# YuePanEdward/GH-ICP

Hardware: AMD Instinct MI355X
Metric: registered_pairs_per_sec (higher is better)
Workload: dtype f64

## Files before the change

### gh-icp_amd/csrc/ctx.h

```cpp
#pragma once
#include <hip/hip_runtime.h>

#include <atomic>
#include <cstdarg>
#include <cstdio>
#include <cstring>
#include <string>
#include <vector>

#include "../../include/ghicp_c.h"

#define GH_HIP(call)                                                                                          \
  do {                                                                                                        \
    hipError_t e_ = (call);                                                                                   \
    if (e_ != hipSuccess) return ctx->fail(GHICP_ERR_HIP, "%s:%d %s -> %s", __FILE__, __LINE__, #call, hipGetErrorString(e_)); \
  } while (0)
#define GH_TRY(call)               \
  do {                             \
    int r_ = (call);               \
    if (r_ != GHICP_OK) return r_; \
  } while (0)
#define GH_ARG(cond)                                                                \
  do {                                                                              \
    if (!(cond)) return ctx->fail(GHICP_ERR_ARG, "%s: bad argument (%s)", __func__, #cond); \
  } while (0)

#define GH_ENTER(ctx)                                                                                             \
  do {                                                                                                            \
    if (!(ctx)) return GHICP_ERR_ARG;                                                                             \
    if (hipSetDevice((ctx)->device) != hipSuccess) return (ctx)->fail(GHICP_ERR_HIP, "hipSetDevice(%d) failed", (ctx)->device); \
  } while (0)

struct DevBuf {
  void* p = nullptr;
  size_t cap = 0;
  hipError_t reserve(size_t bytes) {
    if (bytes <= cap) return hipSuccess;
    if (p) {
      hipError_t e = hipFree(p);
      if (e != hipSuccess) return e;
      p = nullptr; cap = 0;
    }
    size_t want = bytes + bytes / 4 + 256;
    hipError_t e = hipMalloc(&p, want);
    if (e != hipSuccess) return e;
    cap = want;
    return hipSuccess;
  }
  template <typename T> T* as() const { return reinterpret_cast<T*>(p); }
  void release() { if (p) (void)hipFree(p); p = nullptr; cap = 0; }
};

enum BufSlot {
  B_STAGE0 = 0, B_STAGE1, B_STAGE2, B_STAGE3, B_STAGE4, B_STAGE5, B_STAGE6, B_STAGE7,
  B_LOOP_STATE, B_LOOP_KPS, B_LOOP_PARTMIN, B_LOOP_PARTIDX, B_LOOP_PARTSUM, B_LOOP_PARTMIN2, B_LOOP_PARTIDX2, B_LOOP_FDT,
  B_LOOP_SP, B_LOOP_TP, B_LOOP_TRACE, B_LOOP_WFD, B_LOOP_KMW, B_LOOP_KMMATCH, B_LOOP_KMSCR, B_LOOP_ACC,
  B_GRID_KEYS, B_GRID_KEYS2, B_GRID_VALS, B_GRID_VALS2, B_GRID_TMP, B_GRID_START, B_GRID_PTS, B_GRID_MISC,
  B_GRID2_KEYS, B_GRID2_KEYS2, B_GRID2_VALS, B_GRID2_VALS2, B_GRID2_START, B_GRID2_PTS,
  B_FE_LAMBDA, B_FE_CURV, B_FE_COUNT, B_FE_CAND, B_FE_STATE, B_FE_KP, B_FE_SORTK, B_FE_SORTK2, B_FE_SORTV, B_FE_SORTV2, B_FE_CPTS,
  B_FE_FLAGS, B_FE_SCAN, B_FE_SCATTER,
  B_P_KEEP_S, B_P_KEEP_T, B_P_DS_S, B_P_DS_T, B_P_KP_S, B_P_KP_T, B_P_KPXYZ_S, B_P_KPXYZ_T, B_P_FEAT_S, B_P_FEAT_T, B_P_LCS,
  B_P_FD, B_P_MISC, B_P_PATTERN, B_FD_JOBS, B_TRANSFORM_JOBS,
  B_KM_LX, B_KM_MISC, B_KM_SLACK, B_KM_LSTAT, B_KM_ORDER,
  B_FB_DESC, B_FB_HEADPOS, B_FB_DS, B_FB_ORD,
  B_PRIM_TMP, B_NMSR_KEY, B_NMSR_CELL, B_NMSR_TABLE, B_NMSR_HEAD, B_NMSR_PTS, B_NMSR_SKEY, B_NMSR_STATE, B_NMSR_NEXT, B_NMSR_SEL, B_NMSR_MISC, B_NMSR_LIST, B_NMSR_PTS0, B_NMSR_SKEY0,
  B_ICP_TC_KEYS, B_ICP_TC_KEYS2, B_ICP_TC_VALS, B_ICP_TC_VALS2, B_ICP_TC_START, B_ICP_TC_PTS,
  B_ICP_SC_KEYS, B_ICP_SC_KEYS2, B_ICP_SC_VALS, B_ICP_SC_VALS2, B_ICP_SC_START, B_ICP_SC_PTS,
  B_ICP_CUR, B_ICP_Q, B_ICP_NN, B_ICP_ND, B_ICP_NN2, B_ICP_ND2, B_ICP_KEYS, B_ICP_KEYS2, B_ICP_SORTTMP, B_ICP_PART, B_ICP_STATE,
  B_ICP_PEND, B_ICP_TNRM, B_ICP_OUT,
  B_GICP_COVS, B_GICP_COVT, B_GICP_MAHAL, B_GICP_SRC4,
  B_NUM
};

enum KtSlot { KT_PCA = 0, KT_BSC, KT_KM_SOLVE, KT_CD_ROWMIN, KT_KM_WEIGHTS, KT_FD_BSC, KT_NMS_ROUND, KT_VOXEL_SORT,
              KT_FB_VOXEL, KT_FB_GRID, KT_FB_PRUNE, KT_FB_RANK, KT_FB_OUT,
              KT_PAIR_LOOP,
              KT_TRANSFORM,
              KT_PAIR_LOOP_DISPATCH,
              KT_NUM };
static const char* const kKtNames[KT_NUM] = {"pca_cells", "bsc", "km_solve", "cd_rowmin", "km_weights", "fd_bsc", "nms_round", "voxel_sort",
                                             "fb_voxel", "fb_grid", "fb_prune", "fb_rank", "fb_out", "pair_loop", "transform", "pair_loop_dispatch"};

struct ghicp_ctx {
  bool kt_on = false;
  double kt_ms[KT_NUM] = {0};
  long long kt_count[KT_NUM] = {0};
  struct KtPending { int slot; hipEvent_t a, b; };
  std::vector<KtPending> kt_pending;
  std::vector<hipEvent_t> kt_pool;
  hipEvent_t kt_event() {
    if (!kt_pool.empty()) { hipEvent_t e = kt_pool.back(); kt_pool.pop_back(); return e; }
    hipEvent_t e = nullptr;
    (void)hipEventCreate(&e);
    return e;
  }
  hipEvent_t kt_begin(int slot) { return kt_begin_on(slot, stream); }
  void kt_end(int slot, hipEvent_t a) { kt_end_on(slot, a, stream); }
  hipEvent_t kt_begin_on(int slot, hipStream_t st) {
    if (!kt_on) return nullptr;
    hipEvent_t a = kt_event();
    (void)hipEventRecord(a, st);
    (void)slot;
    return a;
  }
  void kt_end_on(int slot, hipEvent_t a, hipStream_t st) {
    if (!kt_on || !a) return;
    hipEvent_t b = kt_event();
    (void)hipEventRecord(b, st);
    kt_pending.push_back({slot, a, b});
  }
  void kt_collect() {
    for (auto& p : kt_pending) {
      float ms = 0;
      if (hipEventElapsedTime(&ms, p.a, p.b) == hipSuccess) { kt_ms[p.slot] += ms; kt_count[p.slot]++; }
      kt_pool.push_back(p.a);
      kt_pool.push_back(p.b);
    }
    kt_pending.clear();
  }
  static constexpr int KM_LSTAT_MAX = 8192;
  static constexpr int KM_LSTAT_W = 8;
  long long km_launches = 0;
  std::vector<int> km_slots;
  long long loop_hazards = 0;
  std::vector<float> loop_cost_hints;
  std::vector<long long> loop_timeline;
  std::atomic<long long> loop_active{0}, loop_total{0};
  bool bbox_valid = false;
  const float* bbox_ptr = nullptr;
  long long bbox_n = 0;
  int bbox_stride = 0;
  float bbox_mm[6] = {0, 0, 0, 0, 0, 0};
  int device = 0;
  hipStream_t stream = nullptr;
  hipStream_t own_stream = nullptr;
  bool km_stats = false, km_force_hazard = false;
  int loop_slots_cap = 0;
  bool loop_confine = true;
  double loop_confine_margin = 1.15;
  hipStream_t confine_stream = nullptr, rest_stream = nullptr;
  int confine_cus = 0;
  struct ConfinePair { int cus; hipStream_t confined, rest; };
  std::vector<ConfinePair> confine_cache;
  int loop_min_lds = 0;
  std::vector<uint32_t> cu_mask;
  std::vector<hipStream_t> aux_streams;
  std::vector<hipEvent_t> aux_events;
  int* progress_host = nullptr;
  std::atomic<bool> progress_live{false};
  bool host_ptrs = false;
  struct Staged { const void* host; size_t bytes; uint64_t fp; void* dev; uint64_t tick; };
  std::vector<Staged> staged;
  size_t staged_bytes = 0;
  uint64_t stage_tick = 0;
  long long staged_hits = 0, staged_misses = 0;
  void stage_clear() {
    if (staged.empty()) return;
    (void)hipStreamSynchronize(stream);
    for (auto& e : staged) (void)hipFree(e.dev);
    staged.clear();
    staged_bytes = 0;
  }
  static constexpr size_t STAGED_MIN = 256 * 1024, STAGED_CAP = (size_t)1 << 30;
  std::string err;
  DevBuf buf[B_NUM];
  std::vector<DevBuf> pairbuf;
  void* pinned = nullptr;
  void* job_pinned = nullptr;
  size_t job_pinned_cap = 0;
  hipEvent_t job_event = nullptr;
  bool job_pending = false;
  int upload_table(const void* src, size_t bytes, void* dst) {
    if (job_pending) {
      if (hipEventSynchronize(job_event) != hipSuccess) return fail(GHICP_ERR_HIP, "job table: event wait failed");
      job_pending = false;
    }
    if (bytes > job_pinned_cap) {
      if (job_pinned) (void)hipHostFree(job_pinned);
      job_pinned = nullptr;
      job_pinned_cap = 0;
      const size_t cap = ((bytes * 3 / 2) + 4095) & ~(size_t)4095;
      if (hipHostMalloc(&job_pinned, cap, hipHostMallocDefault) != hipSuccess) return fail(GHICP_ERR_HIP, "job table: pinned allocation of %zu bytes failed", cap);
      job_pinned_cap = cap;
    }
    if (!job_event && hipEventCreateWithFlags(&job_event, hipEventDisableTiming) != hipSuccess) return fail(GHICP_ERR_HIP, "job table: event creation failed");
    memcpy(job_pinned, src, bytes);
    if (hipMemcpyAsync(dst, job_pinned, bytes, hipMemcpyHostToDevice, stream) != hipSuccess) return fail(GHICP_ERR_HIP, "job table: upload failed");
    if (hipEventRecord(job_event, stream) != hipSuccess) return fail(GHICP_ERR_HIP, "job table: event record failed");
    job_pending = true;
    return GHICP_OK;
  }
  void* fb_pinned = nullptr;
  std::vector<struct ghicp_cloud*> pair_clouds;
  size_t pinned_cap = 0;
  int num_cu = 256;

  int fail(int code, const char* fmt, ...) {
    char tmp[1024];
    va_list ap;
    va_start(ap, fmt);
    vsnprintf(tmp, sizeof(tmp), fmt, ap);
    va_end(ap);
    err = tmp;
    return code;
  }
  template <typename T> int reserve(BufSlot s, size_t count, T** out) {
    hipError_t e = buf[s].reserve(count * sizeof(T) + 16);
    if (e != hipSuccess) return fail(GHICP_ERR_HIP, "hipMalloc(%zu bytes, slot %d): %s", count * sizeof(T), (int)s, hipGetErrorString(e));
    *out = buf[s].as<T>();
    return GHICP_OK;
  }
};

struct Stager {
  ghicp_ctx* ctx;
  struct Out { void* host; void* dev; size_t bytes; };
  std::vector<Out> outs;
  std::vector<void*> temps;
  bool uploaded = false;
  explicit Stager(ghicp_ctx* c) : ctx(c) { ctx->stage_tick++; }
  ~Stager() {
    if (uploaded && temps.empty()) (void)hipStreamSynchronize(ctx->stream);
    for (void* p : temps) (void)hipFree(p);
  }
  static uint64_t fingerprint(const void* p, size_t bytes) {
    const unsigned char* b = reinterpret_cast<const unsigned char*>(p);
    const size_t nw = bytes / 8;
    uint64_t h0 = 0x9E3779B97F4A7C15ull, h1 = 0xC2B2AE3D27D4EB4Full, h2 = 0x165667B19E3779F9ull, h3 = 0x27D4EB2F165667C5ull;
    size_t i = 0;
    for (; i + 4 <= nw; i += 4) {
      uint64_t w[4];
      memcpy(w, b + i * 8, 32);
      h0 = (h0 ^ w[0]) * 0x100000001B3ull; h1 = (h1 ^ w[1]) * 0x100000001B3ull;
      h2 = (h2 ^ w[2]) * 0x100000001B3ull; h3 = (h3 ^ w[3]) * 0x100000001B3ull;
      h0 ^= h0 >> 29; h1 ^= h1 >> 31; h2 ^= h2 >> 27; h3 ^= h3 >> 33;
    }
    for (; i < nw; i++) { uint64_t w; memcpy(&w, b + i * 8, 8); h0 = (h0 ^ w) * 0x100000001B3ull; }
    for (size_t k = nw * 8; k < bytes; k++) h1 = (h1 ^ b[k]) * 0x100000001B3ull;
    return (h0 ^ (h1 << 1) ^ (h2 << 2) ^ (h3 << 3)) + bytes;
  }
  template <typename T> int in_cloud(const T* p, size_t count, const T** out) { return stage_in(p, count, out, true); }
  template <typename T> int in(const T* p, size_t count, const T** out) { return stage_in(p, count, out, false); }
  template <typename T> int stage_in(const T* p, size_t count, const T** out, bool cacheable) {
    if (!ctx->host_ptrs || p == nullptr) { *out = p; return GHICP_OK; }
    const size_t bytes = count * sizeof(T);
    if (cacheable && bytes >= ghicp_ctx::STAGED_MIN && bytes <= ghicp_ctx::STAGED_CAP / 4) {
      const uint64_t fp = fingerprint(p, bytes);
      for (auto& e : ctx->staged)
        if (e.host == p && e.bytes == bytes && e.fp == fp) {
          e.tick = ctx->stage_tick;
          ctx->staged_hits++;
          *out = reinterpret_cast<const T*>(e.dev);
          return GHICP_OK;
        }
      while (!ctx->staged.empty() && (ctx->staged_bytes + bytes > ghicp_ctx::STAGED_CAP || ctx->staged.size() >= 16)) {
        size_t lru = ctx->staged.size();
        for (size_t i = 0; i < ctx->staged.size(); i++)
          if (ctx->staged[i].tick != ctx->stage_tick && (lru == ctx->staged.size() || ctx->staged[i].tick < ctx->staged[lru].tick)) lru = i;
        if (lru == ctx->staged.size()) break;
        (void)hipStreamSynchronize(ctx->stream);
        (void)hipFree(ctx->staged[lru].dev);
        ctx->staged_bytes -= ctx->staged[lru].bytes;
        ctx->staged.erase(ctx->staged.begin() + (long)lru);
      }
      void* d = nullptr;
      if (hipMalloc(&d, bytes + 16) != hipSuccess) return ctx->fail(GHICP_ERR_HIP, "stage-in hipMalloc failed");
      if (hipMemcpyAsync(d, p, bytes, hipMemcpyHostToDevice, ctx->stream) != hipSuccess) { (void)hipFree(d); return ctx->fail(GHICP_ERR_HIP, "stage-in copy failed"); }
      ctx->staged.push_back({p, bytes, fp, d, ctx->stage_tick});
      ctx->staged_bytes += bytes;
      ctx->staged_misses++;
      uploaded = true;
      *out = reinterpret_cast<const T*>(d);
      return GHICP_OK;
    }
    void* d = nullptr;
    if (hipMalloc(&d, count * sizeof(T) + 16) != hipSuccess) return ctx->fail(GHICP_ERR_HIP, "stage-in hipMalloc failed");
    temps.push_back(d);
    if (hipMemcpyAsync(d, p, count * sizeof(T), hipMemcpyHostToDevice, ctx->stream) != hipSuccess)
      return ctx->fail(GHICP_ERR_HIP, "stage-in copy failed");
    *out = reinterpret_cast<const T*>(d);
    return GHICP_OK;
  }
  template <typename T> int out(T* p, size_t count, T** outp) {
    if (!ctx->host_ptrs || p == nullptr) { *outp = p; return GHICP_OK; }
    void* d = nullptr;
    if (hipMalloc(&d, count * sizeof(T) + 16) != hipSuccess) return ctx->fail(GHICP_ERR_HIP, "stage-out hipMalloc failed");
    temps.push_back(d);
    outs.push_back({p, d, count * sizeof(T)});
    *outp = reinterpret_cast<T*>(d);
    return GHICP_OK;
  }
  int finish() {
    for (auto& o : outs)
      if (hipMemcpyAsync(o.host, o.dev, o.bytes, hipMemcpyDeviceToHost, ctx->stream) != hipSuccess)
        return ctx->fail(GHICP_ERR_HIP, "stage-out copy failed");
    if (!outs.empty() && hipStreamSynchronize(ctx->stream) != hipSuccess) return ctx->fail(GHICP_ERR_HIP, "stage-out sync failed");
    outs.clear();
    return GHICP_OK;
  }
};

static inline int cdiv(long long a, long long b) { return (int)((a + b - 1) / b); }
__host__ __device__ inline int cdiv_dev(int a, int b) { return (a + b - 1) / b; }

struct gh_loop_job {
  const ghicp_params* p;
  const double* kpS;
  int ks;
  const double* kpT;
  int kt;
  const void* FD;
  const void* FDt;
  double* Rt16;
  ghicp_iter* trace;
  int32_t* n_iter;
  int32_t* converged;
  int32_t* matchlist;
  double* rmse_after;
  const void* resume_in;
  void* resume_out;
  double* kpS_out;
  ghicp_iter* trace_last;
  int ml_row0;
};
int gh_register_batch_dev(ghicp_ctx* ctx, int nb, const gh_loop_job* jobs);
static inline int gh_registered_ok(int converged, double rmse_after, float radius_nonmax) {
  return (converged && rmse_after < 1.5 * (double)radius_nonmax) ? 1 : 0;
}

int gh_fd_bsc_dev(ghicp_ctx* ctx, const uint8_t* featS, int ks, int V, const uint8_t* featT, int kt, uint16_t* FD);
struct gh_fd_bsc_job { const uint8_t* featS; const uint8_t* featT; uint16_t* FD; uint16_t* FDt; int ks, kt, V; };
int gh_fd_bsc_batch_dev(ghicp_ctx* ctx, int nb, const gh_fd_bsc_job* jobs);
int gh_register_dev(ghicp_ctx* ctx, const ghicp_params* p, const double* kpS, int ks, const double* kpT, int kt, const void* FD,
                    double* Rt16, ghicp_iter* trace, int32_t* n_iter, int32_t* matchlist);
int gh_knn_normals_dev(ghicp_ctx* ctx, const float* xyz, long long m, int stride, int k, float* normals);
int gh_gicp_cov_dev(ghicp_ctx* ctx, const float* xyz, long long m, int stride, int k, double eps, double* cov6);
int gh_km_solve_dev(ghicp_ctx* ctx, const double* w, int n, double eps, int32_t* match, const int* done_flag);
```

### gh-icp_amd/csrc/ctx.hip

```cpp
#include "ctx.h"
#include "devmath.h"

extern "C" const char* ghicp_version(void) { return "ghicp-hip 0.1 (gfx950)"; }

extern "C" void ghicp_params_default(ghicp_params* p) {
  if (!p) return;
  memset(p, 0, sizeof(*p));
  p->feature = GHICP_FEATURE_BSC;
  p->corr = GHICP_CORR_KM;
  p->dof = 6;
  p->max_iter = 200;
  p->radius_nonmax = 1.5f;
  p->adjust_ratio = 1.1f;
  p->adjust_step = 0.1f;
  p->est_iou = 0.6f;
  p->converge_t = 0.02f;
  p->converge_r = 0.02f;
  p->bbx_magnitude = 0.f;
  p->penalty_initial = 2.0;
  p->para1 = 1.0;
  p->para2 = 1.0;
  p->km_eps = 0.01;
  p->min_cor = 10;
  p->weight_changing_rate = 6;
}

extern "C" int ghicp_ctx_create(int device, ghicp_ctx** out) {
  if (!out) return GHICP_ERR_ARG;
  *out = nullptr;
  int count = 0;
  if (hipGetDeviceCount(&count) != hipSuccess || count <= 0 || device < 0 || device >= count) return GHICP_ERR_NO_GPU;
  if (hipSetDevice(device) != hipSuccess) return GHICP_ERR_NO_GPU;
  hipDeviceProp_t prop;
  if (hipGetDeviceProperties(&prop, device) != hipSuccess) return GHICP_ERR_NO_GPU;
  ghicp_ctx* c = new ghicp_ctx();
  c->device = device;
  c->num_cu = prop.multiProcessorCount > 0 ? prop.multiProcessorCount : 256;
  c->km_stats = getenv("GHICP_KM_STATS") != nullptr;
  c->km_force_hazard = getenv("GHICP_KM_FORCE_HAZARD") != nullptr;
  if (const char* e = getenv("GHICP_LOOP_SLOTS")) c->loop_slots_cap = atoi(e) > 0 ? atoi(e) : 0;
  if (const char* e = getenv("GHICP_LOOP_CONFINE")) c->loop_confine = atoi(e) != 0;
  if (const char* e = getenv("GHICP_LOOP_MIN_LDS")) c->loop_min_lds = atoi(e) > 0 ? atoi(e) : 0;
  if (const char* e = getenv("GHICP_LOOP_CONFINE_MARGIN")) { const double m = atof(e); if (m >= 0.25 && m <= 4.0) c->loop_confine_margin = m; }
  if (hipHostMalloc(&c->pinned, 4096, hipHostMallocDefault) != hipSuccess) { delete c; return GHICP_ERR_HIP; }
  c->pinned_cap = 4096;
  *out = c;
  return GHICP_OK;
}

extern "C" int ghicp_ctx_destroy(ghicp_ctx* ctx) {
  if (!ctx) return GHICP_OK;
  (void)hipSetDevice(ctx->device);
  (void)hipDeviceSynchronize();
  ctx->kt_collect();
  for (hipEvent_t e : ctx->kt_pool) (void)hipEventDestroy(e);
  for (ghicp_cloud* c : ctx->pair_clouds) (void)ghicp_cloud_destroy(c);
  ctx->pair_clouds.clear();
  for (int i = 0; i < B_NUM; i++) ctx->buf[i].release();
  for (auto& b : ctx->pairbuf) b.release();
  ctx->stage_clear();
  if (ctx->pinned) (void)hipHostFree(ctx->pinned);
  if (ctx->job_pinned) (void)hipHostFree(ctx->job_pinned);
  if (ctx->job_event) (void)hipEventDestroy(ctx->job_event);
  if (ctx->fb_pinned) (void)hipHostFree(ctx->fb_pinned);
  if (ctx->own_stream) (void)hipStreamDestroy(ctx->own_stream);
  for (auto& e : ctx->confine_cache) { (void)hipStreamDestroy(e.confined); (void)hipStreamDestroy(e.rest); }
  for (hipStream_t a : ctx->aux_streams) (void)hipStreamDestroy(a);
  for (hipEvent_t e : ctx->aux_events) (void)hipEventDestroy(e);
  if (ctx->progress_host) (void)hipHostFree(ctx->progress_host);
  delete ctx;
  return GHICP_OK;
}

extern "C" int ghicp_ctx_stage_stats(const ghicp_ctx* ctx, int64_t* hits, int64_t* misses, int64_t* bytes_kept) {
  if (!ctx) return GHICP_ERR_ARG;
  if (hits) *hits = ctx->staged_hits;
  if (misses) *misses = ctx->staged_misses;
  if (bytes_kept) *bytes_kept = (int64_t)ctx->staged_bytes;
  return GHICP_OK;
}

extern "C" int ghicp_ctx_set_stream(ghicp_ctx* ctx, void* s) {
  GH_ENTER(ctx);
  ctx->stream = reinterpret_cast<hipStream_t>(s);
  return GHICP_OK;
}
extern "C" int ghicp_ctx_set_cu_mask(ghicp_ctx* ctx, const uint32_t* mask, int32_t n_words) {
  GH_ENTER(ctx);
  GH_ARG(mask != nullptr && n_words >= 1 && n_words <= 64);
  bool any = false;
  for (int i = 0; i < n_words; i++) any = any || mask[i] != 0u;
  GH_ARG(any);
  hipStream_t s = nullptr;
  GH_HIP(hipExtStreamCreateWithCUMask(&s, (uint32_t)n_words, mask));
  if (ctx->own_stream) { (void)hipStreamSynchronize(ctx->own_stream); (void)hipStreamDestroy(ctx->own_stream); }
  ctx->own_stream = s;
  ctx->stream = s;
  ctx->cu_mask.assign(mask, mask + n_words);
  for (hipStream_t a : ctx->aux_streams) { (void)hipStreamSynchronize(a); (void)hipStreamDestroy(a); }
  ctx->aux_streams.clear();
  return GHICP_OK;
}

extern "C" int ghicp_ctx_set_host_pointers(ghicp_ctx* ctx, int on) {
  GH_ENTER(ctx);
  ctx->host_ptrs = on != 0;
  if (!ctx->host_ptrs) ctx->stage_clear();
  return GHICP_OK;
}
extern "C" int ghicp_ctx_stage_clear(ghicp_ctx* ctx) {
  GH_ENTER(ctx);
  ctx->stage_clear();
  return GHICP_OK;
}
extern "C" int ghicp_ctx_synchronize(ghicp_ctx* ctx) {
  GH_ENTER(ctx);
  GH_HIP(hipStreamSynchronize(ctx->stream));
  return GHICP_OK;
}
extern "C" int ghicp_ctx_kernel_timing(ghicp_ctx* ctx, int on) {
  GH_ENTER(ctx);
  GH_HIP(hipStreamSynchronize(ctx->stream));
  ctx->kt_collect();
  ctx->kt_on = on != 0;
  for (int i = 0; i < KT_NUM; i++) { ctx->kt_ms[i] = 0; ctx->kt_count[i] = 0; }
  if (on) {
    unsigned long long* lstat;
    GH_TRY(ctx->reserve(B_KM_LSTAT, (size_t)ghicp_ctx::KM_LSTAT_MAX * ghicp_ctx::KM_LSTAT_W, &lstat));
    GH_HIP(hipMemsetAsync(lstat, 0, (size_t)ghicp_ctx::KM_LSTAT_MAX * ghicp_ctx::KM_LSTAT_W * sizeof(unsigned long long), ctx->stream));
    ctx->km_launches = 0;
    ctx->km_slots.clear();
  }
  return GHICP_OK;
}
extern "C" int ghicp_ctx_loop_progress(const ghicp_ctx* ctx, int64_t* active, int64_t* total) {
  if (!ctx || !active || !total) return GHICP_ERR_ARG;
  *total = ctx->loop_total.load(std::memory_order_relaxed);
  if (ctx->progress_live.load(std::memory_order_acquire) && ctx->progress_host) {
    const long long done = *(volatile int*)ctx->progress_host;
    *active = *total > done ? *total - done : 0;
  } else {
    *active = ctx->loop_active.load(std::memory_order_relaxed);
  }
  return GHICP_OK;
}
extern "C" int ghicp_ctx_loop_progress_reset(ghicp_ctx* ctx, int64_t total) {
  if (!ctx || total < 0) return GHICP_ERR_ARG;
  ctx->progress_live.store(false, std::memory_order_release);
  ctx->loop_total.store(total, std::memory_order_relaxed);
  ctx->loop_active.store(total, std::memory_order_relaxed);
  return GHICP_OK;
}
extern "C" int ghicp_ctx_kernel_time(ghicp_ctx* ctx, const char* name, double* total_ms, int64_t* launches) {
  GH_ENTER(ctx);
  GH_ARG(name != nullptr);
  GH_HIP(hipStreamSynchronize(ctx->stream));
  ctx->kt_collect();
  for (int i = 0; i < KT_NUM; i++)
    if (strcmp(name, kKtNames[i]) == 0) {
      if (total_ms) *total_ms = ctx->kt_ms[i];
      if (launches) *launches = ctx->kt_count[i];
      return GHICP_OK;
    }
  return ctx->fail(GHICP_ERR_ARG, "unknown kernel name '%s'", name);
}
extern "C" int ghicp_ctx_set_loop_cost_hints(ghicp_ctx* ctx, int32_t n_pairs, const float* cost) {
  GH_ENTER(ctx);
  GH_ARG(n_pairs >= 0 && (n_pairs == 0 || cost != nullptr));
  ctx->loop_cost_hints.assign(cost, cost + n_pairs);
  for (float& c : ctx->loop_cost_hints)
    if (!(c == c)) c = 0.f;
  return GHICP_OK;
}
extern "C" int ghicp_ctx_loop_timeline(ghicp_ctx* ctx, int64_t* out3, int64_t cap_pairs, int64_t* n_pairs) {
  GH_ENTER(ctx);
  GH_ARG(n_pairs != nullptr && cap_pairs >= 0);
  const int64_t n = (int64_t)(ctx->loop_timeline.size() / 3);
  *n_pairs = n;
  if (out3)
    for (int64_t i = 0; i < std::min(n, cap_pairs) * 3; i++) out3[i] = ctx->loop_timeline[(size_t)i];
  return GHICP_OK;
}
extern "C" const char* ghicp_last_error(const ghicp_ctx* ctx) { return ctx ? ctx->err.c_str() : "null context"; }

namespace {

__global__ __launch_bounds__(1024) void k_rigid_svd(const double* __restrict__ src, const double* __restrict__ tgt, int c,
                                                    double* __restrict__ out16) {
  __shared__ double red[16];
  const int tid = threadIdx.x, nt = blockDim.x;
  double m[6] = {0, 0, 0, 0, 0, 0};
  for (int i = tid; i < c; i += nt)
    for (int d = 0; d < 3; d++) { m[d] += (double)(float)src[(size_t)i * 3 + d]; m[3 + d] += (double)(float)tgt[(size_t)i * 3 + d]; }
  for (int d = 0; d < 6; d++) m[d] = gh_block_sum(m[d], red);
  float msf[3], mtf[3];
  for (int d = 0; d < 3; d++) { msf[d] = (float)(m[d] / (double)c); mtf[d] = (float)(m[3 + d] / (double)c); }
  double H[9] = {0, 0, 0, 0, 0, 0, 0, 0, 0};
  for (int i = tid; i < c; i += nt) {
    double a[3], b[3];
    for (int d = 0; d < 3; d++) {
      a[d] = (double)(float)tgt[(size_t)i * 3 + d] - (double)mtf[d];
      b[d] = (double)(float)src[(size_t)i * 3 + d] - (double)msf[d];
    }
    for (int r = 0; r < 3; r++)
      for (int q = 0; q < 3; q++) H[r * 3 + q] += a[r] * b[q];
  }
  for (int d = 0; d < 9; d++) H[d] = gh_block_sum(H[d], red);
  if (tid == 0) {
    double A[9], R[9];
    for (int d = 0; d < 9; d++) A[d] = H[d] / (double)c;
    gh_quant_grid(A, 9);
    gh_kabsch(A, R);
    float Rf[9];
    for (int d = 0; d < 9; d++) Rf[d] = (float)R[d];
    for (int d = 0; d < 16; d++) out16[d] = 0;
    for (int r = 0; r < 3; r++) {
      const float t = (float)((double)mtf[r] - (((double)Rf[r * 3] * (double)msf[0] + (double)Rf[r * 3 + 1] * (double)msf[1]) +
                                                 (double)Rf[r * 3 + 2] * (double)msf[2]));
      for (int q = 0; q < 3; q++) out16[r * 4 + q] = (double)Rf[r * 3 + q];
      out16[r * 4 + 3] = (double)t;
    }
    out16[15] = 1;
  }
}

struct M34 { float m[12]; };
__global__ __launch_bounds__(256) void k_transform(const float* __restrict__ xyz, long long n, int stride, M34 M, float* __restrict__ out) {
  for (long long i = blockIdx.x * 256ll + threadIdx.x; i < n; i += (long long)gridDim.x * 256) {
    const float x = xyz[i * stride], y = xyz[i * stride + 1], z = xyz[i * stride + 2];
    out[i * 3 + 0] = ((M.m[0] * x + M.m[1] * y) + M.m[2] * z) + M.m[3];
    out[i * 3 + 1] = ((M.m[4] * x + M.m[5] * y) + M.m[6] * z) + M.m[7];
    out[i * 3 + 2] = ((M.m[8] * x + M.m[9] * y) + M.m[10] * z) + M.m[11];
  }
}

struct TransformJob { const float* xyz; float* out; long long n; M34 M; };
__device__ __forceinline__ void transform_point(const M34& M, float x, float y, float z, float& ox, float& oy, float& oz) {
  ox = ((M.m[0] * x + M.m[1] * y) + M.m[2] * z) + M.m[3];
  oy = ((M.m[4] * x + M.m[5] * y) + M.m[6] * z) + M.m[7];
  oz = ((M.m[8] * x + M.m[9] * y) + M.m[10] * z) + M.m[11];
}
__global__ __launch_bounds__(256) void k_transform_batch(const TransformJob* __restrict__ jobs, int job0, int stride) {
  const TransformJob J = jobs[job0 + blockIdx.y];
  const long long n = J.n;
  if (stride == 3 && ((reinterpret_cast<uintptr_t>(J.xyz) | reinterpret_cast<uintptr_t>(J.out)) & 15) == 0) {
    const long long n4 = n >> 2;
    const float4* __restrict__ in4 = reinterpret_cast<const float4*>(J.xyz);
    float4* __restrict__ out4 = reinterpret_cast<float4*>(J.out);
    for (long long g = blockIdx.x * 256ll + threadIdx.x; g < n4; g += (long long)gridDim.x * 256) {
      const float4 a = in4[g * 3], b = in4[g * 3 + 1], c = in4[g * 3 + 2];
      float4 oa, ob, oc;
      transform_point(J.M, a.x, a.y, a.z, oa.x, oa.y, oa.z);
      transform_point(J.M, a.w, b.x, b.y, oa.w, ob.x, ob.y);
      transform_point(J.M, b.z, b.w, c.x, ob.z, ob.w, oc.x);
      transform_point(J.M, c.y, c.z, c.w, oc.y, oc.z, oc.w);
      out4[g * 3] = oa; out4[g * 3 + 1] = ob; out4[g * 3 + 2] = oc;
    }
    if (blockIdx.x == 0 && threadIdx.x < (n & 3)) {
      const long long i = (n4 << 2) + threadIdx.x;
      transform_point(J.M, J.xyz[i * 3], J.xyz[i * 3 + 1], J.xyz[i * 3 + 2], J.out[i * 3], J.out[i * 3 + 1], J.out[i * 3 + 2]);
    }
    return;
  }
  for (long long i = blockIdx.x * 256ll + threadIdx.x; i < n; i += (long long)gridDim.x * 256)
    transform_point(J.M, J.xyz[i * stride], J.xyz[i * stride + 1], J.xyz[i * stride + 2], J.out[i * 3], J.out[i * 3 + 1], J.out[i * 3 + 2]);
}

__global__ __launch_bounds__(256) void k_gather4(const float* __restrict__ xyz, int stride, const int* __restrict__ idx, long long m,
                                                 float4* __restrict__ out) {
  const long long i = blockIdx.x * 256ll + threadIdx.x;
  if (i >= m) return;
  const long long s = idx[i];
  out[i] = make_float4(xyz[s * stride], xyz[s * stride + 1], xyz[s * stride + 2], 0.f);
}

__global__ __launch_bounds__(256) void k_bbox(const float* __restrict__ xyz, long long n, int stride, float* __restrict__ mm ) {
  __shared__ float smin[3][4], smax[3][4];
  float mn[3] = {3.0e38f, 3.0e38f, 3.0e38f}, mx[3] = {-3.0e38f, -3.0e38f, -3.0e38f};
  for (long long i = blockIdx.x * 256ll + threadIdx.x; i < n; i += (long long)gridDim.x * 256)
    for (int d = 0; d < 3; d++) { const float v = xyz[i * stride + d]; mn[d] = fminf(mn[d], v); mx[d] = fmaxf(mx[d], v); }
  for (int d = 0; d < 3; d++) {
    for (int o = 32; o > 0; o >>= 1) { mn[d] = fminf(mn[d], __shfl_xor(mn[d], o, 64)); mx[d] = fmaxf(mx[d], __shfl_xor(mx[d], o, 64)); }
    if ((threadIdx.x & 63) == 0) { smin[d][threadIdx.x >> 6] = mn[d]; smax[d][threadIdx.x >> 6] = mx[d]; }
  }
  __syncthreads();
  if (threadIdx.x < 3) {
    const int d = threadIdx.x;
    float a = smin[d][0], b = smax[d][0];
    for (int w = 1; w < 4; w++) { a = fminf(a, smin[d][w]); b = fmaxf(b, smax[d][w]); }
    auto enc = [](float f) { int i = __float_as_int(f); return i >= 0 ? i : i ^ 0x7fffffff; };
    atomicMin(reinterpret_cast<int*>(mm) + d, enc(a));
    atomicMax(reinterpret_cast<int*>(mm) + 3 + d, enc(b));
  }
}

}

__global__ void k_bbox_init(int* mm) {
  if (threadIdx.x < 6) mm[threadIdx.x] = threadIdx.x < 3 ? 0x7f7fffff : (int)0x80800000;
}

int gh_bbox_dev(ghicp_ctx* ctx, const float* xyz, long long n, int stride, float* mm_host6) {
  if (ctx->bbox_valid && ctx->bbox_ptr == xyz && ctx->bbox_n == n && ctx->bbox_stride == stride) {
    memcpy(mm_host6, ctx->bbox_mm, 6 * sizeof(float));
    return GHICP_OK;
  }
  int* d;
  GH_TRY(ctx->reserve(B_GRID_MISC, 64, &d));
  hipLaunchKernelGGL(k_bbox_init, dim3(1), dim3(64), 0, ctx->stream, d);
  if (n > 0) hipLaunchKernelGGL(k_bbox, dim3(min(cdiv(n, 256), 2048)), dim3(256), 0, ctx->stream, xyz, n, stride, reinterpret_cast<float*>(d));
  int* h = reinterpret_cast<int*>(reinterpret_cast<char*>(ctx->pinned) + 256);
  GH_HIP(hipMemcpyAsync(h, d, 6 * sizeof(int), hipMemcpyDeviceToHost, ctx->stream));
  GH_HIP(hipStreamSynchronize(ctx->stream));
  for (int k = 0; k < 6; k++) {
    int i = h[k] >= 0 ? h[k] : h[k] ^ 0x7fffffff;
    memcpy(&mm_host6[k], &i, 4);
  }
  return GHICP_OK;
}

extern "C" int ghicp_cloud_bounds(ghicp_ctx* ctx, const float* xyz, int64_t n, int stride, double* out6) {
  GH_ENTER(ctx);
  GH_ARG(out6 != nullptr && n > 0 && stride >= 3);
  Stager sg(ctx);
  const float* d;
  GH_TRY(sg.in_cloud(xyz, (size_t)n * stride, &d));
  float mm[6];
  GH_TRY(gh_bbox_dev(ctx, d, n, stride, mm));
  for (int k = 0; k < 6; k++) out6[k] = (double)mm[k];
  return GHICP_OK;
}

extern "C" int ghicp_bbx_magnitude(ghicp_ctx* ctx, const float* xyz, int64_t n, int stride, float* bbx) {
  GH_ENTER(ctx);
  GH_ARG(bbx != nullptr && n >= 0 && stride >= 3);
  Stager sg(ctx);
  const float* d;
  GH_TRY(sg.in_cloud(xyz, (size_t)n * stride, &d));
  if (n == 0) { *bbx = 0.f; return GHICP_OK; }
  float mm[6];
  GH_TRY(gh_bbox_dev(ctx, d, n, stride, mm));
  *bbx = (float)((double)mm[3] - (double)mm[0] + (double)mm[4] - (double)mm[1] + (double)mm[5] - (double)mm[2]);
  return GHICP_OK;
}

extern "C" int ghicp_rigid_svd(ghicp_ctx* ctx, const double* src, const double* tgt, int64_t c, double* Rt16) {
  GH_ENTER(ctx);
  GH_ARG(c > 0 && src && tgt && Rt16);
  Stager sg(ctx);
  const double *ds, *dt;
  GH_TRY(sg.in(src, (size_t)c * 3, &ds));
  GH_TRY(sg.in(tgt, (size_t)c * 3, &dt));
  double* out;
  GH_TRY(ctx->reserve(B_P_MISC, 16, &out));
  hipLaunchKernelGGL(k_rigid_svd, dim3(1), dim3(1024), 0, ctx->stream, ds, dt, (int)c, out);
  GH_HIP(hipGetLastError());
  GH_HIP(hipMemcpyAsync(Rt16, out, 16 * sizeof(double), hipMemcpyDeviceToHost, ctx->stream));
  GH_HIP(hipStreamSynchronize(ctx->stream));
  return GHICP_OK;
}

extern "C" int ghicp_rigid_svd_host(const double* src, const double* tgt, int64_t c, double* out16) {
  if (!src || !tgt || !out16 || c < 1) return GHICP_ERR_ARG;
  double m[6] = {0, 0, 0, 0, 0, 0};
  for (int64_t i = 0; i < c; i++)
    for (int d = 0; d < 3; d++) { m[d] += (double)(float)src[(size_t)i * 3 + d]; m[3 + d] += (double)(float)tgt[(size_t)i * 3 + d]; }
  float msf[3], mtf[3];
  for (int d = 0; d < 3; d++) { msf[d] = (float)(m[d] / (double)c); mtf[d] = (float)(m[3 + d] / (double)c); }
  double H[9] = {0, 0, 0, 0, 0, 0, 0, 0, 0};
  for (int64_t i = 0; i < c; i++) {
    double a[3], b[3];
    for (int d = 0; d < 3; d++) {
      a[d] = (double)(float)tgt[(size_t)i * 3 + d] - (double)mtf[d];
      b[d] = (double)(float)src[(size_t)i * 3 + d] - (double)msf[d];
    }
    for (int r = 0; r < 3; r++)
      for (int q = 0; q < 3; q++) H[r * 3 + q] += a[r] * b[q];
  }
  double A[9], R[9];
  for (int d = 0; d < 9; d++) A[d] = H[d] / (double)c;
  gh_quant_grid(A, 9);
  gh_kabsch(A, R);
  float Rf[9];
  for (int d = 0; d < 9; d++) Rf[d] = (float)R[d];
  for (int d = 0; d < 16; d++) out16[d] = 0;
  for (int r = 0; r < 3; r++) {
    const float t = (float)((double)mtf[r] - (((double)Rf[r * 3] * (double)msf[0] + (double)Rf[r * 3 + 1] * (double)msf[1]) +
                                               (double)Rf[r * 3 + 2] * (double)msf[2]));
    for (int q = 0; q < 3; q++) out16[r * 4 + q] = (double)Rf[r * 3 + q];
    out16[r * 4 + 3] = (double)t;
  }
  out16[15] = 1;
  return GHICP_OK;
}

extern "C" int ghicp_transform_cloud(ghicp_ctx* ctx, const float* xyz, int64_t n, int stride, const double* Rt, float* out) {
  GH_ENTER(ctx);
  GH_ARG(n >= 0 && stride >= 3 && Rt != nullptr);
  Stager sg(ctx);
  const float* d;
  float* o;
  GH_TRY(sg.in_cloud(xyz, (size_t)n * stride, &d));
  GH_TRY(sg.out(out, (size_t)n * 3, &o));
  M34 M;
  for (int r = 0; r < 3; r++)
    for (int c = 0; c < 4; c++) M.m[r * 4 + c] = (float)Rt[r * 4 + c];
  if (n > 0) {
    hipLaunchKernelGGL(k_transform, dim3(min(cdiv(n, 256), 4096)), dim3(256), 0, ctx->stream, d, (long long)n, stride, M, o);
    GH_HIP(hipGetLastError());
  }
  return sg.finish();
}

extern "C" int ghicp_transform_clouds(ghicp_ctx* ctx, int32_t n_clouds, const float* const* xyz, const int64_t* n, int stride, const double* Rt16,
                                      float* const* out) {
  GH_ENTER(ctx);
  GH_ARG(n_clouds >= 0 && stride >= 3 && (n_clouds == 0 || (xyz && n && Rt16 && out)));
  if (ctx->host_ptrs) return ctx->fail(GHICP_ERR_ARG, "ghicp_transform_clouds: device-pointer mode only (use ghicp_transform_cloud per cloud)");
  if (n_clouds == 0) return GHICP_OK;
  std::vector<TransformJob> h((size_t)n_clouds);
  int64_t nmax = 0;
  for (int i = 0; i < n_clouds; i++) {
    GH_ARG(n[i] >= 0 && (n[i] == 0 || (xyz[i] && out[i])));
    h[i].xyz = xyz[i]; h[i].out = out[i]; h[i].n = n[i];
    for (int r = 0; r < 3; r++)
      for (int c = 0; c < 4; c++) h[i].M.m[r * 4 + c] = (float)Rt16[(size_t)i * 16 + r * 4 + c];
    nmax = std::max<int64_t>(nmax, n[i]);
  }
  TransformJob* d;
  GH_TRY(ctx->reserve(B_TRANSFORM_JOBS, h.size(), &d));
  GH_TRY(ctx->upload_table(h.data(), h.size() * sizeof(TransformJob), d));
  if (nmax > 0) {
    const int bx = (int)std::max<int64_t>(1, std::min<int64_t>(cdiv(nmax, 256 * 8), 2048));
    hipEvent_t kev = ctx->kt_begin(KT_TRANSFORM);
    for (int j0 = 0; j0 < n_clouds; j0 += 65535)
      hipLaunchKernelGGL(k_transform_batch, dim3(bx, std::min(65535, n_clouds - j0)), dim3(256), 0, ctx->stream, (const TransformJob*)d, j0, stride);
    ctx->kt_end(KT_TRANSFORM, kev);
    GH_HIP(hipGetLastError());
  }
  return GHICP_OK;
}

extern "C" int ghicp_gather_points(ghicp_ctx* ctx, const float* xyz, int stride, const int32_t* idx, int64_t m, float* out) {
  GH_ENTER(ctx);
  GH_ARG(m >= 0 && stride >= 3);
  if (ctx->host_ptrs) return ctx->fail(GHICP_ERR_ARG, "ghicp_gather_points: device-pointer mode only");
  if (m > 0) {
    hipLaunchKernelGGL(k_gather4, dim3(cdiv(m, 256)), dim3(256), 0, ctx->stream, xyz, stride, idx, (long long)m, reinterpret_cast<float4*>(out));
    GH_HIP(hipGetLastError());
  }
  return GHICP_OK;
}
```

### gh-icp_amd/csrc/km4.hip

```cpp
#include "km4_dev.h"

#include <algorithm>
#include <vector>
#include <cstdlib>

namespace {

template <bool PROF>
__global__ __launch_bounds__(K4_T) void k_km4(const Km2Problem* __restrict__ probs, int flags, int lds_bytes, unsigned long long* __restrict__ lstat,
                                            const int* __restrict__ order) {
  const Km2Problem P = probs[order ? order[blockIdx.x] : (int)blockIdx.x];
  if (P.n <= 0 || (P.done && *P.done)) return;
  extern __shared__ __attribute__((aligned(16))) char smem[];
  k4_solve_block<PROF>(P, flags, smem, lds_bytes, lstat);
}

}

size_t gh_km4_lds_bytes(int n) {
  const size_t nw = (size_t)(n + 31) / 32;
  return (size_t)n * 3 * 8 + 16 * 8 + 8 * nw * 4 + SH_NUM * 4 + ((size_t)n * (1 + 2 * K4_CAP) + 2 * ((size_t)n + 2)) * 2 + (size_t)n + 64;
}

bool gh_km4_fits(int n) { return n <= 65534 && gh_km4_lds_bytes(n) <= 160 * 1024 - 256; }

static int k4_launch(ghicp_ctx* ctx, const Km2Problem* d_probs, int nprob, size_t lds, const int* d_order) {
  const size_t want = 160 * 1024;
  GH_HIP(hipFuncSetAttribute(reinterpret_cast<const void*>(&k_km4<false>), hipFuncAttributeMaxDynamicSharedMemorySize, (int)want));
  GH_HIP(hipFuncSetAttribute(reinterpret_cast<const void*>(&k_km4<true>), hipFuncAttributeMaxDynamicSharedMemorySize, (int)want));
  const int kflags = ctx->km_force_hazard ? 4 : 0;
  unsigned long long* lstat = nullptr;
  if (ctx->kt_on && ctx->km_launches < ghicp_ctx::KM_LSTAT_MAX) {
    GH_TRY(ctx->reserve(B_KM_LSTAT, (size_t)ghicp_ctx::KM_LSTAT_MAX * ghicp_ctx::KM_LSTAT_W, &lstat));
    lstat += ctx->km_launches * ghicp_ctx::KM_LSTAT_W;
    int per_cu = 0;
    GH_HIP(hipOccupancyMaxActiveBlocksPerMultiprocessor(&per_cu, reinterpret_cast<const void*>(&k_km4<false>), K4_T, lds));
    ctx->km_slots.push_back(per_cu * ctx->num_cu);
    ctx->km_launches++;
  }
  hipEvent_t kt = ctx->kt_begin(KT_KM_SOLVE);
  if (ctx->km_stats) hipLaunchKernelGGL((k_km4<true>), dim3(nprob), dim3(K4_T), lds, ctx->stream, d_probs, kflags, (int)lds, lstat, d_order);
  else hipLaunchKernelGGL((k_km4<false>), dim3(nprob), dim3(K4_T), lds, ctx->stream, d_probs, kflags, (int)lds, lstat, d_order);
  ctx->kt_end(KT_KM_SOLVE, kt);
  GH_HIP(hipGetLastError());
  return GHICP_OK;
}

int gh_km4_launch(ghicp_ctx* ctx, const Km2Problem* d_probs, int nprob, int n_max) {
  return k4_launch(ctx, d_probs, nprob, gh_km4_lds_bytes(n_max), nullptr);
}

int gh_km4_plan(ghicp_ctx* ctx, const int* h_n, int nprob, Km4Plan* plan, const float* cost) {
  *plan = Km4Plan();
  std::vector<std::pair<int, int>> key((size_t)nprob);
  for (int i = 0; i < nprob; i++) {
    const int n = std::max(1, h_n[i]);
    if (!gh_km4_fits(n)) return ctx->fail(GHICP_ERR_INTERNAL, "gh_km4_plan: n = %d does not fit", n);
    key[i] = {(int)std::min<size_t>(4, (160 * 1024) / gh_km4_lds_bytes(n)), n};
  }
  std::vector<int> order((size_t)nprob);
  for (int i = 0; i < nprob; i++) order[i] = i;
  std::stable_sort(order.begin(), order.end(), [&](int a, int b) {
    if (key[a].first != key[b].first) return key[a].first < key[b].first;
    if (cost && cost[a] != cost[b]) return cost[a] > cost[b];
    return key[a].second > key[b].second;
  });
  int nc = 0;
  for (int i = 0; i < nprob;) {
    int j = i;
    while (j < nprob && key[order[j]].first == key[order[i]].first) j++;
    if (nc == 8) { plan->count[7] += nprob - i; break; }
    plan->begin[nc] = i; plan->count[nc] = j - i;
    int nmax = 1;
    for (int t = i; t < j; t++) nmax = std::max(nmax, key[order[t]].second);
    plan->lds[nc] = gh_km4_lds_bytes(nmax);
    plan->per_cu[nc] = key[order[i]].first;
    for (int t = i; t < j; t++) plan->weight[nc] += (cost && cost[order[t]] > 0.f) ? (double)cost[order[t]] : (double)key[order[t]].second * (double)key[order[t]].second;
    nc++;
    i = j;
  }
  plan->nclass = nc;
  GH_TRY(ctx->reserve(B_KM_ORDER, (size_t)nprob + 1, &plan->d_order));
  GH_HIP(hipMemcpyAsync(plan->d_order, order.data(), (size_t)nprob * sizeof(int), hipMemcpyHostToDevice, ctx->stream));
  GH_HIP(hipStreamSynchronize(ctx->stream));
  return GHICP_OK;
}

int gh_km4_launch_plan(ghicp_ctx* ctx, const Km2Problem* d_probs, const Km4Plan& plan) {
  for (int c = 0; c < plan.nclass; c++)
    if (plan.count[c] > 0) GH_TRY(k4_launch(ctx, d_probs, plan.count[c], plan.lds[c], plan.d_order + plan.begin[c]));
  return GHICP_OK;
}

extern "C" int ghicp_ctx_km_launch_stats(ghicp_ctx* ctx, double* out8) {
  GH_ENTER(ctx);
  GH_ARG(out8 != nullptr);
  for (int i = 0; i < 8; i++) out8[i] = 0.0;
  const long long nl = ctx->km_launches;
  if (nl <= 0 || !ctx->buf[B_KM_LSTAT].p) return GHICP_OK;
  GH_HIP(hipStreamSynchronize(ctx->stream));
  constexpr int W = ghicp_ctx::KM_LSTAT_W;
  std::vector<unsigned long long> h((size_t)nl * W);
  GH_HIP(hipMemcpy(h.data(), ctx->buf[B_KM_LSTAT].p, h.size() * sizeof(unsigned long long), hipMemcpyDeviceToHost));
  const double tick_ms = 1e3 / 100e6;
  double solves = 0, sum_dt = 0, sum_max = 0, sum_span = 0, cap = 0, worst = 0, slots = 0;
  long long used = 0;
  for (long long l = 0; l < nl; l++) {
    const unsigned long long* r = &h[(size_t)l * W];
    if (r[4] == 0 || r[6] != 0) continue;
    const double start = (double)((1ull << 62) - r[0]), span = (double)r[1] - start;
    used++;
    solves += (double)r[4]; sum_dt += (double)r[2]; sum_max += (double)r[3]; sum_span += span;
    slots = (double)ctx->km_slots[(size_t)l];
    cap += std::min(slots, (double)r[4]) * span;
    worst = std::max(worst, (double)r[3] / ((double)r[2] / (double)r[4]));
  }
  if (used == 0) return GHICP_OK;
  out8[0] = (double)used; out8[1] = solves; out8[2] = sum_dt / solves * tick_ms; out8[3] = sum_max / (double)used * tick_ms;
  out8[4] = sum_span / (double)used * tick_ms; out8[5] = slots; out8[6] = cap > 0 ? 1.0 - sum_dt / cap : 0.0; out8[7] = worst;
  return GHICP_OK;
}

extern "C" int ghicp_ctx_loop_hazards(ghicp_ctx* ctx, int64_t* solves) {
  GH_ENTER(ctx);
  GH_ARG(solves != nullptr);
  *solves = (int64_t)ctx->loop_hazards;
  return GHICP_OK;
}

extern "C" int ghicp_ctx_pair_loop_stats(ghicp_ctx* ctx, double* out8) {
  GH_ENTER(ctx);
  GH_ARG(out8 != nullptr);
  for (int i = 0; i < 8; i++) out8[i] = 0.0;
  const long long nl = ctx->km_launches;
  if (nl <= 0 || !ctx->buf[B_KM_LSTAT].p) return GHICP_OK;
  for (hipStream_t a : ctx->aux_streams) GH_HIP(hipStreamSynchronize(a));
  GH_HIP(hipStreamSynchronize(ctx->stream));
  constexpr int W = ghicp_ctx::KM_LSTAT_W;
  std::vector<unsigned long long> h((size_t)nl * W);
  GH_HIP(hipMemcpy(h.data(), ctx->buf[B_KM_LSTAT].p, h.size() * sizeof(unsigned long long), hipMemcpyDeviceToHost));
  const double tick_ms = 1e3 / 100e6;
  double launches = 0, slots = 0, solves = 0, sum_dt = 0, mx = 0, sum_span = 0, life = 0, cap = 0;
  for (long long l = 0; l < nl; l++) {
    const unsigned long long* r = &h[(size_t)l * W];
    if (r[6] == 0) continue;
    const double start = (double)((1ull << 62) - r[0]), span = (double)r[1] - start;
    launches++; slots += (double)r[6]; solves += (double)r[4]; sum_dt += (double)r[2]; mx = std::max(mx, (double)r[3]);
    sum_span += span; life += (double)r[5]; cap += std::min((double)ctx->km_slots[(size_t)l], (double)r[6]) * span;
  }
  if (launches == 0) return GHICP_OK;
  out8[0] = launches; out8[1] = slots; out8[2] = solves; out8[3] = solves > 0 ? sum_dt / solves * tick_ms : 0.0; out8[4] = mx * tick_ms;
  out8[5] = sum_span / launches * tick_ms; out8[6] = cap > 0 ? 1.0 - life / cap : 0.0; out8[7] = life > 0 ? sum_dt / life : 0.0;
  return GHICP_OK;
}
```

### gh-icp_amd/csrc/km4_dev.h

```cpp
#pragma once
#include "ctx.h"
#include "devmath.h"
#include "km_prob.h"

#include <climits>

namespace {


constexpr int K4_CAP = 3;
constexpr int K4_OVER = 255;
constexpr int K4_HINT = 2 * K4_CAP;
constexpr int K4_T = 256;
constexpr int K4_NONE = 0xFFFF;
constexpr double K4_INF = 1000.0;

typedef __attribute__((address_space(1))) const int* k4_gint;
typedef __attribute__((address_space(1))) const double* k4_gf64;
typedef __attribute__((address_space(1))) const unsigned* k4_gu32;

enum { SH_QT = 0, SH_FREE, SH_RES, SH_QTF, SH_HAZ, SH_CH0, SH_CH1, SH_BAD, SH_NF, SH_UNCERT, SH_LROW, SH_CH2, SH_DFS, SH_NUM = 16 };

struct K4 {
  double *lx, *ly, *slack, *red;
  unsigned *visx, *visy, *prevy, *pushed, *good, *goody, *freey, *ovf;
  int* sh;
  unsigned short *match, *stx, *sty, *tlc, *tlo;
  unsigned char* tln;
  int n, nw;
  double bg, eps;
  k4_gu32 rptr;
  k4_gint cols;
  k4_gf64 vals;
};

__device__ inline bool k4_bit(const unsigned* b, int i) { return (b[i >> 5] >> (i & 31)) & 1u; }
__device__ inline bool k4_flagged(int tn) { return tn > K4_CAP; }
__device__ inline int k4_cnt(int tn) { return tn > K4_CAP ? 0 : tn; }

template <bool REBUILD, bool PUSH, bool ONLY_UNPUSHED, bool SEED = false>
__device__ inline void k4_bulk(const K4& s, const unsigned short* list, int count, int wave, int lane) {
  const int grp = lane >> 4, lig = lane & 15;
  unsigned long long* sl = reinterpret_cast<unsigned long long*>(s.slack);
  for (int base = 0; base < count; base += 16) {
    const int i = base + wave * 4 + grp;
    int x = -1;
    if (i < count) {
      x = list[i];
      if (ONLY_UNPUSHED && k4_bit(s.pushed, x)) x = -1;
    }
    unsigned cb = 0, ce = 0;
    double lxr = 0.0;
    if (x >= 0) { cb = s.rptr[x]; ce = s.rptr[x + 1]; lxr = s.lx[x]; }
    int cnt = 0;
    for (unsigned off = 0; __ballot(cb + off < ce); off += 64) {
      int col[4];
      double val[4];
      unsigned c[4];
#pragma unroll
      for (int j = 0; j < 4; j++) {
        c[j] = cb + off + 16u * j + lig;
        col[j] = 0; val[j] = 0.0;
        if (ce > cb) { const unsigned cc = min(c[j], ce - 1u); col[j] = s.cols[cc]; val[j] = s.vals[cc]; }
      }
      double lyv[4];
#pragma unroll
      for (int j = 0; j < 4; j++) lyv[j] = s.ly[col[j]];
#pragma unroll
      for (int j = 0; j < 4; j++) {
        const bool in = c[j] < ce;
        const double d = (lxr + lyv[j]) - val[j];
        const bool td = d < s.eps;
        if (PUSH && in && !td) atomicMin(&sl[col[j]], (unsigned long long)__double_as_longlong(d));
        if (SEED && in && td) {
          const unsigned bit = 1u << (col[j] & 31);
          if (s.prevy[col[j] >> 5] & bit) {
            if (s.sty[col[j]] == x) atomicOr(&s.goody[col[j] >> 5], bit);
          } else if (!(atomicOr(&s.visy[col[j] >> 5], bit) & bit)) {
            s.sty[col[j]] = (unsigned short)x;
            const int m = s.match[col[j]];
            if (m == K4_NONE) s.sh[SH_FREE] = 1;
            else { s.stx[atomicAdd(&s.sh[SH_QT], 1)] = (unsigned short)m; atomicOr(&s.visx[m >> 5], 1u << (m & 31)); }
          }
        }
        if (REBUILD) {
          const unsigned gb = (unsigned)(__ballot(in && td) >> (grp * 16)) & 0xffffu;
          if (in && td) {
            const int rk = cnt + __popc(gb & ((1u << lig) - 1u));
            if (rk < K4_CAP) { s.tlc[x * K4_CAP + rk] = (unsigned short)col[j]; s.tlo[x * K4_CAP + rk] = (unsigned short)(c[j] - cb); }
          }
          __builtin_amdgcn_wave_barrier();
          if (in && td) {
            const int rk = cnt + __popc(gb & ((1u << lig) - 1u));
            if (rk >= K4_CAP && rk < K4_HINT) s.tlo[x * K4_CAP + rk - K4_CAP] = (unsigned short)col[j];
          }
          cnt += __popc(gb);
        }
      }
    }
    if (REBUILD && lig == 0 && x >= 0) {
      const int tn = cnt > K4_HINT ? K4_OVER : cnt;
      const bool over = tn == K4_OVER, was = s.tln[x] == K4_OVER;
      s.tln[x] = (unsigned char)tn;
      if (over != was) {
        if (over) atomicOr(&s.ovf[x >> 5], 1u << (x & 31));
        else atomicAnd(&s.ovf[x >> 5], ~(1u << (x & 31)));
      }
    }
  }
}

__device__ inline void k4_revalidate(const K4& s, int tid) {
  for (int base = tid; base < s.n; base += 4 * K4_T) {
    int tn[4], lc[4][K4_CAP];
    unsigned px[4], pv[4][K4_CAP];
#pragma unroll
    for (int k = 0; k < 4; k++) {
      const int ic = min(base + k * K4_T, s.n - 1);
      tn[k] = s.tln[ic];
      px[k] = s.pushed[ic >> 5];
#pragma unroll
      for (int e = 0; e < K4_CAP; e++) lc[k][e] = s.tlc[ic * K4_CAP + e];
    }
#pragma unroll
    for (int k = 0; k < 4; k++)
#pragma unroll
      for (int e = 0; e < K4_CAP; e++) pv[k][e] = s.prevy[lc[k][e] >> 5];
#pragma unroll
    for (int k = 0; k < 4; k++) {
      const int i = base + k * K4_T;
      if (i >= s.n || tn[k] == 0 || k4_flagged(tn[k]) || ((px[k] >> (i & 31)) & 1u)) continue;
      bool hit = false;
#pragma unroll
      for (int e = 0; e < K4_CAP; e++) hit |= (int)(e < tn[k]) & (int)((pv[k][e] >> (lc[k][e] & 31)) & 1u);
      if (!hit) continue;
      const double lxv = s.lx[i];
      const unsigned rb = s.rptr[i];
      int keep = 0;
      for (int e = 0; e < tn[k]; e++) {
        const int col = s.tlc[i * K4_CAP + e];
        const unsigned short o = s.tlo[i * K4_CAP + e];
        const double w = s.vals[rb + o];
        if (((lxv + s.ly[col]) - w) < s.eps) { s.tlc[i * K4_CAP + keep] = (unsigned short)col; s.tlo[i * K4_CAP + keep] = o; keep++; }
      }
      s.tln[i] = (unsigned char)keep;
    }
  }
}

__device__ inline void k4_pool_build(const K4& s, const unsigned short* __restrict__ flist, unsigned short* __restrict__ pool, int nf, int region, int wave, int lane) {
  const int grp = lane >> 4, lig = lane & 15, capf = region - 1;
  for (int base = 0; base < nf; base += 16) {
    const int i = base + wave * 4 + grp;
    int x = -1;
    if (i < nf) x = flist[i];
    unsigned cb = 0, ce = 0;
    double lxr = 0.0;
    if (x >= 0) { cb = s.rptr[x]; ce = s.rptr[x + 1]; lxr = s.lx[x]; }
    int cnt = 0;
    for (unsigned off = 0; __ballot(cb + off < ce); off += 64) {
      int col[4];
      double val[4];
      unsigned c[4];
#pragma unroll
      for (int j = 0; j < 4; j++) {
        c[j] = cb + off + 16u * j + lig;
        col[j] = 0; val[j] = 0.0;
        if (ce > cb) { const unsigned cc = min(c[j], ce - 1u); col[j] = s.cols[cc]; val[j] = s.vals[cc]; }
      }
      double lyv[4];
#pragma unroll
      for (int j = 0; j < 4; j++) lyv[j] = s.ly[col[j]];
#pragma unroll
      for (int j = 0; j < 4; j++) {
        const bool td = (int)(c[j] < ce) & (int)(((lxr + lyv[j]) - val[j]) < s.eps);
        const unsigned gb = (unsigned)(__ballot(td) >> (grp * 16)) & 0xffffu;
        if (td) {
          const int rk = cnt + __popc(gb & ((1u << lig) - 1u));
          if (rk < capf) pool[i * region + 1 + rk] = (unsigned short)col[j];
        }
        cnt += __popc(gb);
      }
    }
    if (lig == 0 && x >= 0) {
      if (cnt > capf) { atomicOr(&s.good[x >> 5], 1u << (x & 31)); cnt = 0; }
      pool[i * region] = (unsigned short)cnt;
    }
  }
}

#define K4_DPP_MIN(V, CTRL)                                                                                   \
  V = fmin(V, __hiloint2double(__builtin_amdgcn_update_dpp(0, __double2hiint(V), CTRL, 0xf, 0xf, false),     \
                               __builtin_amdgcn_update_dpp(0, __double2loint(V), CTRL, 0xf, 0xf, false)))
__device__ inline double k4_wave_min(double v) {
  K4_DPP_MIN(v, 0xb1);
  K4_DPP_MIN(v, 0x4e);
  K4_DPP_MIN(v, 0x124);
  K4_DPP_MIN(v, 0x128);
  const int hi = __double2hiint(v), lo = __double2loint(v);
  const double r0 = __hiloint2double(__builtin_amdgcn_readlane(hi, 0), __builtin_amdgcn_readlane(lo, 0));
  const double r1 = __hiloint2double(__builtin_amdgcn_readlane(hi, 16), __builtin_amdgcn_readlane(lo, 16));
  const double r2 = __hiloint2double(__builtin_amdgcn_readlane(hi, 32), __builtin_amdgcn_readlane(lo, 32));
  const double r3 = __hiloint2double(__builtin_amdgcn_readlane(hi, 48), __builtin_amdgcn_readlane(lo, 48));
  return fmin(fmin(r0, r1), fmin(r2, r3));
}
#undef K4_DPP_MIN

#define K4_CLAIM(WANT, COL, OWNER, PARENT)                                                  \
  do {                                                                                      \
    unsigned old_ = 0u;                                                                     \
    const unsigned bit_ = 1u << ((COL) & 31);                                               \
    if (WANT) old_ = atomicOr(&s.visy[(COL) >> 5], bit_);                                   \
    const bool fresh_ = (WANT) && !(old_ & bit_);                                           \
    if (fresh_) s.sty[COL] = (unsigned short)(PARENT);                                      \
    free_l |= fresh_ && (OWNER) == K4_NONE;                                                 \
    const bool enq_ = fresh_ && (OWNER) != K4_NONE;                                         \
    const unsigned long long eb_ = __ballot(enq_);                                          \
    if (enq_) {                                                                             \
      s.stx[qt + __popcll(eb_ & ((1ull << lane) - 1ull))] = (unsigned short)(OWNER);        \
      atomicOr(&s.visx[(OWNER) >> 5], 1u << ((OWNER) & 31));                                \
    }                                                                                       \
    qt += __popcll(eb_);                                                                    \
  } while (0)

template <bool PROF>
__device__ inline bool k4_flood(const K4& s, int qh0, int qt0, double lflood0, int lane, int* qt_out, long long* pc) {
  const int n = s.n;
  int qh = qh0, qt = qt0;
  bool free_l = false;
  double lflood = lflood0;
  while (qh < qt) {
    const int qe = qt;
    double lcand = INFINITY;
    int xcand = 0;
    const long long tl0 = PROF ? (long long)__builtin_readcyclecounter() : 0;
    if (PROF) pc[0]++;
    for (int base = qh; base < qe; base += 64) {
      const int i = base + lane;
      const bool act = i < qe;
      const int xr = s.stx[min(i, qe - 1)];
      const double lxr = s.lx[xr];
      const int tn = s.tln[xr];
      int lc[K4_CAP], mc[K4_CAP];
      unsigned vw[K4_CAP];
#pragma unroll
      for (int k = 0; k < K4_CAP; k++) lc[k] = s.tlc[xr * K4_CAP + k];
#pragma unroll
      for (int k = 0; k < K4_CAP; k++) { vw[k] = s.visy[lc[k] >> 5]; mc[k] = s.match[lc[k]]; }
      const int t = act ? k4_cnt(tn) : 0;
#pragma unroll
      for (int k = 0; k < K4_CAP; k++) {
        const bool want = (int)(k < t) & (int)(((vw[k] >> (lc[k] & 31)) & 1u) == 0u);
        K4_CLAIM(want, lc[k], mc[k], xr);
      }
      if (act && (lxr - s.bg) < s.eps && lxr < lflood && lxr < lcand) { lcand = lxr; xcand = xr; }
      unsigned long long ob = __ballot(act && k4_flagged(tn));
      if (PROF) pc[1] += __popcll(ob);
      while (ob) {
        const int l = (int)__ffsll((long long)ob) - 1;
        ob &= ob - 1ull;
        const int xo = __builtin_amdgcn_readlane(xr, l);
        const double lxo = s.lx[xo];
        const unsigned cb = s.rptr[xo], ce = s.rptr[xo + 1];
        for (unsigned c0 = cb; c0 < ce; c0 += 64) {
          const unsigned c = c0 + lane, cc = min(c, ce - 1u);
          const int col = s.cols[cc];
          const double val = s.vals[cc];
          const int m = s.match[col];
          const bool want = (int)(c < ce) & (int)(((lxo + s.ly[col]) - val) < s.eps) & (int)!k4_bit(s.visy, col);
          K4_CLAIM(want, col, m, xo);
        }
      }
    }
    const long long tl1 = PROF ? (long long)__builtin_readcyclecounter() : 0;
    if (PROF) pc[2] += tl1 - tl0;
    if (__ballot(lcand < lflood)) {
      const double lmin = k4_wave_min(lcand);
      const int xpar = __builtin_amdgcn_readlane(xcand, (int)__ffsll((long long)__ballot(lcand == lmin)) - 1);
      lcand = lmin;
      lflood = lcand;
      if (PROF) pc[3]++;
      for (int y0 = 0; y0 < n; y0 += 256) {
        bool c[4];
        int m[4];
#pragma unroll
        for (int k = 0; k < 4; k++) {
          const int y = y0 + k * 64 + lane, yc = min(y, n - 1);
          const unsigned vw = s.visy[yc >> 5];
          const double lv = s.ly[yc];
          m[k] = s.match[yc];
          c[k] = (int)(y < n) & (int)(((vw >> (yc & 31)) & 1u) == 0u) & (int)(((lcand + lv) - s.bg) < s.eps);
        }
#pragma unroll
        for (int k = 0; k < 4; k++) {
          if (y0 + k * 64 >= n) break;
          const int y = min(y0 + k * 64 + lane, n - 1);
          K4_CLAIM(c[k], y, m[k], xpar);
        }
      }
    }
    __builtin_amdgcn_wave_barrier();
    if (PROF) pc[4] += (long long)__builtin_readcyclecounter() - tl1;
    qh = qe;
    if (__ballot(free_l)) { *qt_out = qt; return true; }
  }
  *qt_out = qt;
  return false;
}
#undef K4_CLAIM

struct K4Dfs {
  int sp, x, ystart, cp, cnext;
  double ck;
};
template <bool PROF>
__device__ inline int k4_dfs(const K4& s, K4Dfs& D, const bool lazy, int lane, long long* q_iter, long long* q_act, long long* pd) {
  const int n = s.n;
  const double bg = s.bg, eps = s.eps;
  int sp = D.sp, x = D.x, ystart = D.ystart;
  double ck = D.ck;
  int cp = D.cp, cnext = D.cnext;
  const int lk = min(lane, K4_CAP - 1);
  for (;;) {
    if (PROF) { ++*q_iter; ++*q_act; }
    const long long t_it0 = PROF ? (long long)__builtin_readcyclecounter() : 0;
    int it_type = 0;
    const double lxv = s.lx[x];
    const int tn = s.tln[x];
    const int lc = s.tlc[x * K4_CAP + lk];
    const int ncnt = k4_cnt(tn);
    const bool bgt = (lxv - bg) < eps;
    if (PROF) it_type = k4_flagged(tn) ? 0 : (!bgt ? 1 : (tn != 0 ? 2 : 3));
    int slot = 0, p = n;
    if (bgt) {
      const unsigned long long hit = __ballot(ck == lxv);
      p = ystart;
      if (hit) {
        slot = (int)__ffsll((long long)hit) - 1;
        p = max(p, __builtin_amdgcn_readlane(cp, slot));
      } else {
        slot = cnext;
        cnext = (cnext + 1) & 63;
        if (lane == slot) ck = lxv;
      }
    }
    const unsigned vwL = s.visy[lc >> 5], gwL = s.goody[lc >> 5];
    const int mL = s.match[lc];
    int yw = p + lane, ywc = min(yw, n - 1);
    unsigned vwW = s.visy[ywc >> 5], gwW = s.goody[ywc >> 5];
    double lyW = s.ly[ywc];
    int mW = s.match[ywc];
    int best = INT_MAX, mbest = K4_NONE;
    if (k4_flagged(tn)) {
      const unsigned cb = s.rptr[x], ce = s.rptr[x + 1];
      for (unsigned c0 = cb; c0 < ce; c0 += 64) {
        const unsigned c = c0 + lane, cc = min(c, ce - 1u);
        const int col = s.cols[cc];
        const double val = s.vals[cc];
        const bool t = (int)(c < ce) & (int)(((lxv + s.ly[col]) - val) < eps) & (int)(col >= ystart) & (int)!k4_bit(s.visy, col) & (int)k4_bit(s.goody, col);
        const unsigned long long b = __ballot(t);
        if (b) { best = __builtin_amdgcn_readlane(col, (int)__ffsll((long long)b) - 1); mbest = s.match[best]; break; }
      }
    } else {
      const bool t = (int)(lane < ncnt) & (int)(lc >= ystart) & (int)((((~vwL & gwL) >> (lc & 31)) & 1u) != 0u);
      const unsigned long long b = __ballot(t);
      if (b) {
        const int l = (int)__ffsll((long long)b) - 1;
        best = __builtin_amdgcn_readlane(lc, l);
        mbest = __builtin_amdgcn_readlane(mL, l);
      }
    }
    bool augment = false;
    if (bgt) {
      const int lim = min(n, best);
      bool cand = (int)(yw < lim) & (int)((((~vwW & gwW) >> (ywc & 31)) & 1u) != 0u) & (int)(((lxv + lyW) - bg) < eps);
      unsigned long long bw = __ballot(cand);
      while (!bw && p + 64 < lim) {
        p += 64;
        yw = p + lane; ywc = min(yw, n - 1);
        vwW = s.visy[ywc >> 5]; gwW = s.goody[ywc >> 5]; lyW = s.ly[ywc]; mW = s.match[ywc];
        cand = (int)(yw < lim) & (int)((((~vwW & gwW) >> (ywc & 31)) & 1u) != 0u) & (int)(((lxv + lyW) - bg) < eps);
        bw = __ballot(cand);
      }
      if (tn != 0) {
        if (bw) {
          const int l = (int)__ffsll((long long)bw) - 1;
          best = p + l;
          mbest = __builtin_amdgcn_readlane(mW, l);
          if (lane == slot) cp = best;
        } else if (lane == slot) cp = max(p, lim);
      } else {
        int outcome = bw ? 3 : 0;
        if (!bw) p = n;
        while (outcome == 3) {
          bool cont = false;
          if (cand && mW != K4_NONE) cont = (int)(s.tln[mW] == 0) & (int)(s.lx[mW] == lxv);
          const unsigned long long stop = __ballot(cand && !cont);
          const int jstar = stop ? (int)__ffsll((long long)stop) - 1 : 63;
          const unsigned long long R = bw & (~0ull >> (63 - jstar));
          const unsigned long long below = R & ((1ull << lane) - 1ull);
          const int rank = __popcll(below);
          const int pm = __shfl(mW, below ? 63 - __clzll((long long)below) : 0, 64);
          if ((R >> lane) & 1ull) {
            atomicOr(&s.visy[yw >> 5], 1u << (yw & 31));
            s.sty[sp + rank] = (unsigned short)yw;
            if (rank > 0) s.stx[sp + rank] = (unsigned short)pm;
          }
          const int k = __popcll(R), lastlane = 63 - __clzll((long long)R);
          const int mlast = __builtin_amdgcn_readlane(mW, lastlane);
          if (PROF) *q_act += k - 1;
          sp += k - 1;
          p += lastlane + 1;
          if (mlast == K4_NONE) { outcome = 1; break; }
          sp++;
          if (lane == 0) { s.stx[sp] = (unsigned short)mlast; s.sty[sp] = (unsigned short)K4_NONE; }
          x = mlast; ystart = 0;
          if (stop) { outcome = 2; break; }
          if (PROF) ++*q_act;
          bw = 0;
          while (!bw && p < n) {
            yw = p + lane; ywc = min(yw, n - 1);
            vwW = s.visy[ywc >> 5]; gwW = s.goody[ywc >> 5]; lyW = s.ly[ywc]; mW = s.match[ywc];
            cand = (int)(yw < n) & (int)((((~vwW & gwW) >> (ywc & 31)) & 1u) != 0u) & (int)(((lxv + lyW) - bg) < eps);
            bw = __ballot(cand);
            if (!bw) p += 64;
          }
          if (!bw) outcome = 0;
        }
        if (lane == slot) cp = min(p, n);
        __builtin_amdgcn_wave_barrier();
        if (outcome == 1) { augment = true; }
        else if (outcome == 2) { if (PROF) { pd[it_type]++; pd[5 + it_type] += (long long)__builtin_readcyclecounter() - t_it0; } continue; }
      }
    }
    if (PROF && (augment || best != INT_MAX)) { pd[it_type]++; pd[5 + it_type] += (long long)__builtin_readcyclecounter() - t_it0; }
    if (augment) break;
    if (best != INT_MAX) {
      if (lane == 0) { atomicOr(&s.visy[best >> 5], 1u << (best & 31)); s.sty[sp] = (unsigned short)best; }
      if (mbest == K4_NONE) break;
      sp++;
      if (lane == 0) { s.stx[sp] = (unsigned short)mbest; s.sty[sp] = (unsigned short)K4_NONE; }
      x = mbest; ystart = 0;
    } else {
      if (lazy) {
        D.sp = sp; D.x = x; D.ystart = ystart; D.ck = ck; D.cp = cp; D.cnext = cnext;
        __builtin_amdgcn_wave_barrier();
        return 2;
      }
      sp--;
      if (sp < 0) return 0;
      x = s.stx[sp]; ystart = (int)s.sty[sp] + 1;
      if (PROF) { pd[4]++; pd[9] += (long long)__builtin_readcyclecounter() - t_it0; }
    }
    __builtin_amdgcn_wave_barrier();
  }
  __builtin_amdgcn_wave_barrier();
  const int ylast = s.sty[sp];
  for (int f = lane; f <= sp; f += 64) s.match[s.sty[f]] = s.stx[f];
  if (lane == 0) atomicAnd(&s.freey[ylast >> 5], ~(1u << (ylast & 31)));
  return 1;
}

__device__ inline bool k4_dfs_unwind(const K4& s, K4Dfs& D, int lane) {
  int keep = D.sp + 1;
  for (int base = 0; base <= D.sp; base += 64) {
    const int f = base + lane;
    const bool out = f <= D.sp && !k4_bit(s.good, s.stx[min(f, D.sp)]);
    const unsigned long long b = __ballot(out);
    if (b) { keep = base + (int)__ffsll((long long)b) - 1; break; }
  }
  if (keep == 0) return false;
  if (keep <= D.sp) {
    D.sp = keep - 1;
    D.x = s.stx[D.sp];
    D.ystart = (int)s.sty[D.sp] + 1;
  }
  return true;
}

__device__ inline int k4_literal(const K4& s, const Km2Problem& P) {
  const int n = s.n;
  const double bg = s.bg, eps = s.eps;
  unsigned short* curs = s.tlc;
  for (int i = 0; i < n; i++) { s.lx[i] = P.lx_init[i]; s.ly[i] = 0.0; s.match[i] = (unsigned short)K4_NONE; }
  long long budget = 2ll * n * n * n + 4096;
  for (int root = 0; root < n; root++) {
    for (int j = 0; j < n; j++) s.slack[j] = K4_INF;
    for (;;) {
      for (int w = 0; w < s.nw; w++) { s.visx[w] = 0u; s.visy[w] = 0u; }
      int sp = 0;
      s.stx[0] = (unsigned short)root; s.sty[0] = 0; curs[0] = 0;
      s.visx[root >> 5] |= 1u << (root & 31);
      bool ok = false;
      while (sp >= 0) {
        const int x = s.stx[sp];
        const double lxv = s.lx[x];
        const unsigned rb = s.rptr[x], re = s.rptr[x + 1];
        unsigned c = rb + curs[sp];
        int y = s.sty[sp];
        bool descended = false;
        for (; y < n; ++y) {
          double wv = bg;
          if (c < re && s.cols[c] == y) { wv = s.vals[c]; ++c; }
          if (k4_bit(s.visy, y)) continue;
          const double t = lxv + s.ly[y] - wv;
          if (t < eps) {
            s.visy[y >> 5] |= 1u << (y & 31);
            const int m = s.match[y];
            s.sty[sp] = (unsigned short)y;
            curs[sp] = (unsigned short)(c - rb);
            if (m == K4_NONE) { ok = true; break; }
            if (--budget < 0) return 5;
            sp++;
            s.stx[sp] = (unsigned short)m; s.sty[sp] = 0; curs[sp] = 0;
            s.visx[m >> 5] |= 1u << (m & 31);
            descended = true;
            break;
          } else
            s.slack[y] = fmin(t, s.slack[y]);
        }
        if (ok) break;
        if (descended) continue;
        sp--;
        if (sp >= 0) s.sty[sp] = (unsigned short)(s.sty[sp] + 1);
      }
      if (ok) {
        for (int f = 0; f <= sp; f++) s.match[s.sty[f]] = s.stx[f];
        break;
      }
      double delta = K4_INF;
      for (int j = 0; j < n; j++)
        if (!k4_bit(s.visy, j)) delta = fmin(delta, s.slack[j]);
      for (int i = 0; i < n; i++)
        if (k4_bit(s.visx, i)) s.lx[i] -= delta;
      for (int i = 0; i < n; i++) {
        if (k4_bit(s.visy, i)) s.ly[i] += delta;
        else s.slack[i] -= delta;
      }
      if (--budget < 0) return 5;
    }
  }
  return 0;
}

template <bool PROF>
__device__ inline void k4_solve_block(const Km2Problem& P, int flags, char* smem, int lds_bytes, unsigned long long* __restrict__ lstat) {
  const unsigned long long t_wall0 = lstat ? __builtin_amdgcn_s_memrealtime() : 0ull;
  const int n = P.n, nw = (n + 31) / 32, tid = threadIdx.x, lane = tid & 63, wave = tid >> 6;
  K4 s;
  s.n = n; s.nw = nw; s.bg = P.bg; s.eps = P.eps;
  s.rptr = (k4_gu32)P.row_ptr; s.cols = (k4_gint)P.cols; s.vals = (k4_gf64)P.vals;
  s.lx = (double*)smem;
  s.ly = s.lx + n;
  s.slack = s.ly + n;
  s.red = s.slack + n;
  s.visx = (unsigned*)(s.red + 16);
  s.visy = s.visx + nw; s.prevy = s.visy + nw; s.pushed = s.prevy + nw; s.good = s.pushed + nw; s.goody = s.good + nw;
  s.freey = s.goody + nw; s.ovf = s.freey + nw;
  s.sh = (int*)(s.ovf + nw);
  s.match = (unsigned short*)(s.sh + SH_NUM);
  s.stx = s.match + n;
  s.sty = s.stx + n + 2;
  s.tlc = s.sty + n + 2;
  s.tlo = s.tlc + (size_t)n * K4_CAP;
  s.tln = (unsigned char*)(s.tlo + (size_t)n * K4_CAP);
  if ((long long)(reinterpret_cast<char*>(s.tln + n) - smem) > (long long)lds_bytes) {
    if (tid == 0 && P.status) *P.status = 6;
    for (int i = tid; i < n; i += K4_T) P.match_out[i] = -1;
    return;
  }
  const double bg = s.bg, eps = s.eps;
  constexpr int sw = 0;

  long long c_flood = 0, c_fail = 0, c_pull = 0, c_dfs = 0, q_phase = 0, q_fail = 0, q_rounds = 0, q_iter = 0, q_act = 0, q_frows = 0, q_prows = 0;
  long long pcf[5] = {0, 0, 0, 0, 0};
  long long pd[10] = {0, 0, 0, 0, 0, 0, 0, 0, 0, 0};
  const long long t_begin = PROF ? (long long)__builtin_readcyclecounter() : 0;

  for (int i = tid; i < n; i += K4_T) { s.lx[i] = P.lx_init[i]; s.ly[i] = 0.0; s.match[i] = (unsigned short)K4_NONE; s.tln[i] = 0; }
  for (int i = tid; i < n * K4_CAP; i += K4_T) { s.tlc[i] = 0; s.tlo[i] = 0; }
  for (int w = tid; w < nw; w += K4_T) {
    unsigned all = ~0u;
    if (w == nw - 1 && (n & 31)) all = (1u << (n & 31)) - 1u;
    s.freey[w] = all; s.ovf[w] = 0u;
  }
  if (tid < SH_NUM) s.sh[tid] = 0;
  __syncthreads();
  for (int i = tid; i < n; i += K4_T) s.stx[i] = (unsigned short)i;
  __syncthreads();
  k4_bulk<true, false, false>(s, s.stx, n, wave, lane);
  __syncthreads();

  int bad = 0;
  bool hazard = false;
  for (int root = 0; root < n && !bad && !hazard; ++root) {
    for (int i = tid; i < n; i += K4_T) s.slack[i] = K4_INF;
    for (int w = tid; w < nw; w += K4_T) s.pushed[w] = 0u;
    bool have_prev = false;
    for (int w = tid; w < nw; w += K4_T) { s.visx[w] = 0u; s.visy[w] = 0u; }
    __syncthreads();
    if (wave == sw) {
      if (lane == 0) { s.stx[0] = (unsigned short)root; s.visx[root >> 5] = 1u << (root & 31); }
      __builtin_amdgcn_wave_barrier();
      int fq = 0;
      const long long tf0 = PROF ? (long long)__builtin_readcyclecounter() : 0;
      const bool fr = k4_flood<PROF>(s, 0, 1, INFINITY, lane, &fq, pcf);
      if (PROF) c_flood += (long long)__builtin_readcyclecounter() - tf0;
      if (lane == 0) { s.sh[SH_RES] = fr ? 1 : 0; s.sh[SH_QTF] = fq; }
    }
    for (int phase = 0;; ++phase) {
      if (PROF) q_phase++;
      __syncthreads();
      const bool free_found = s.sh[SH_RES] != 0;
      const int qt = s.sh[SH_QTF];
      const long long t1 = PROF ? (long long)__builtin_readcyclecounter() : 0;
      if (!free_found) {
        if (PROF) { q_fail++; q_frows += qt; }
        k4_bulk<false, true, true>(s, s.stx, qt, wave, lane);
        double lm = INFINITY;
        for (int i = tid; i < qt; i += K4_T) lm = fmin(lm, s.lx[s.stx[i]]);
        lm = k4_wave_min(lm);
        if (lane == 0) s.red[wave] = lm;
        __syncthreads();
        const double lxmin = fmin(fmin(s.red[0], s.red[1]), fmin(s.red[2], s.red[3]));
        double dl = K4_INF;
        for (int y = tid; y < n; y += K4_T)
          if (!k4_bit(s.visy, y)) {
            const double s2 = fmin(s.slack[y], (lxmin + s.ly[y]) - bg);
            s.slack[y] = s2;
            dl = fmin(dl, s2);
          }
        dl = k4_wave_min(dl);
        if (lane == 0) s.red[4 + wave] = dl;
        for (int w = tid; w < nw; w += K4_T) {
          if (have_prev && (s.prevy[w] & ~s.visy[w])) s.sh[SH_HAZ] = 1;
          s.prevy[w] = s.visy[w];
        }
        __syncthreads();
        dl = fmin(fmin(s.red[4], s.red[5]), fmin(s.red[6], s.red[7]));
        if (s.sh[SH_HAZ] || ((flags & 4) && phase == 0 && root == n / 2)) { hazard = true; break; }
        for (int i = tid; i < n; i += K4_T) {
          if (k4_bit(s.visx, i)) s.lx[i] -= dl;
          if (k4_bit(s.visy, i)) s.ly[i] += dl;
          else s.slack[i] -= dl;
        }
        for (int w = tid; w < nw; w += K4_T) { s.pushed[w] = s.visx[w]; s.goody[w] = 0u; }
        if (tid == 0) { s.sh[SH_QT] = qt; s.sh[SH_FREE] = 0; s.sh[SH_UNCERT] = 0; s.sh[SH_LROW] = 0; }
        __syncthreads();
        k4_revalidate(s, tid);
        k4_bulk<true, true, false, true>(s, s.stx, qt, wave, lane);
        double lb = INFINITY;
        for (int i = tid; i < qt; i += K4_T) {
          const double l = s.lx[s.stx[i]];
          if ((l - bg) < eps) lb = fmin(lb, l);
        }
        lb = k4_wave_min(lb);
        if (lane == 0) s.red[8 + wave] = lb;
        __syncthreads();
        const double lnew = fmin(fmin(s.red[8], s.red[9]), fmin(s.red[10], s.red[11]));
        for (int i = tid; i < qt; i += K4_T)
          if (s.lx[s.stx[i]] == lnew) s.sh[SH_LROW] = s.stx[i];
        __syncthreads();
        const int lrow = s.sh[SH_LROW];
        for (int y = tid; y < n; y += K4_T) {
          const unsigned bit = 1u << (y & 31);
          if (s.prevy[y >> 5] & bit) {
            if (!(s.goody[y >> 5] & bit) && !(((s.lx[s.sty[y]] + s.ly[y]) - bg) < eps)) s.sh[SH_UNCERT] = 1;
          } else if (!(s.visy[y >> 5] & bit) && ((lnew + s.ly[y]) - bg) < eps) {
            if (!(atomicOr(&s.visy[y >> 5], bit) & bit)) {
              s.sty[y] = (unsigned short)lrow;
              const int m = s.match[y];
              if (m == K4_NONE) s.sh[SH_FREE] = 1;
              else { s.stx[atomicAdd(&s.sh[SH_QT], 1)] = (unsigned short)m; atomicOr(&s.visx[m >> 5], 1u << (m & 31)); }
            }
          }
        }
        __syncthreads();
        const bool certified = s.sh[SH_UNCERT] == 0;
        if (!certified) {
          __syncthreads();
          for (int w = tid; w < nw; w += K4_T) { s.visx[w] = 0u; s.visy[w] = 0u; }
          __syncthreads();
        }
        long long c_fl_in = 0;
        if (wave == sw) {
          int fq = s.sh[SH_QT];
          bool fr = s.sh[SH_FREE] != 0;
          const long long tf0 = PROF ? (long long)__builtin_readcyclecounter() : 0;
          if (!certified) {
            if (lane == 0) { s.stx[0] = (unsigned short)root; s.visx[root >> 5] = 1u << (root & 31); }
            __builtin_amdgcn_wave_barrier();
            fr = k4_flood<PROF>(s, 0, 1, INFINITY, lane, &fq, pcf);
          } else if (!fr) {
            fr = k4_flood<PROF>(s, qt, fq, lnew, lane, &fq, pcf);
          }
          __builtin_amdgcn_wave_barrier();
          if (PROF) { c_fl_in = (long long)__builtin_readcyclecounter() - tf0; c_flood += c_fl_in; }
          if (lane == 0) { s.sh[SH_RES] = fr ? 1 : 0; s.sh[SH_QTF] = fq; }
        }
        have_prev = true;
        if (PROF) { q_prows += qt; c_fail += (long long)__builtin_readcyclecounter() - t1 - c_fl_in; }
        if (phase > 4 * n + 16) { bad = 2; break; }
        continue;
      }
      for (int w = tid; w < nw; w += K4_T) { s.visx[w] = 0u; s.visy[w] = 0u; s.goody[w] = ~0u; }
      __syncthreads();
      K4Dfs dfs;
      dfs.sp = 0; dfs.x = root; dfs.ystart = 0; dfs.cp = 0; dfs.cnext = 0;
      dfs.ck = __longlong_as_double(0x7ff8000000000000ll);
      if (wave == sw) {
        if (lane == 0) { s.stx[0] = (unsigned short)root; s.sty[0] = (unsigned short)K4_NONE; }
        __builtin_amdgcn_wave_barrier();
        const int r = k4_dfs<PROF>(s, dfs, true, lane, &q_iter, &q_act, pd);
        if (lane == 0) s.sh[SH_DFS] = r;
      }
      __syncthreads();
      const long long t1b = PROF ? (long long)__builtin_readcyclecounter() : 0;
      if (PROF) c_dfs += t1b - t1;
      long long t2 = t1b;
      if (s.sh[SH_DFS] == 2) {
      for (int w = tid; w < nw; w += K4_T) { s.good[w] = 0u; s.goody[w] = s.freey[w]; }
      if (tid == 0) { s.sh[SH_CH0] = 0; s.sh[SH_CH1] = 0; s.sh[SH_CH2] = 0; s.sh[SH_NF] = 0; }
      unsigned short* mx = reinterpret_cast<unsigned short*>(s.slack);
      unsigned short* flist = mx + n;
      unsigned short* pool = mx + 2 * (size_t)n;
      if (wave == 0) {
        int cnt = 0;
        for (int base = 0; base < n; base += 64) {
          const int x = base + lane;
          const bool f = x < n && k4_bit(s.ovf, x);
          const unsigned long long b = __ballot(f);
          if (f) flist[cnt + __popcll(b & ((1ull << lane) - 1ull))] = (unsigned short)x;
          cnt += __popcll(b);
        }
        if (lane == 0) s.sh[SH_NF] = cnt;
      }
      for (int i = tid; i < n; i += K4_T) mx[i] = (unsigned short)K4_NONE;
      __syncthreads();
      for (int y = tid; y < n; y += K4_T) {
        const int m = s.match[y];
        if (m != K4_NONE) mx[m] = (unsigned short)y;
      }
      __syncthreads();
      const int nf = s.sh[SH_NF];
      const int region = nf > 0 ? min(64, (n + 2) / nf) : 0;
      if (nf > 0) {
        k4_pool_build(s, flist, pool, nf, region, wave, lane);
        __syncthreads();
      }
      for (int round = 0;; round++) {
        if (PROF) q_rounds++;
        const int chslot[3] = {SH_CH0, SH_CH1, SH_CH2};
        if (tid == 0) s.sh[chslot[(round + 1) % 3]] = 0;
        bool ch = false;
        for (int base = tid; base < n; base += 2 * K4_T) {
          int xx[2], tn[2], lc[2][K4_HINT];
          unsigned gdw[2];
          double lxv[2];
#pragma unroll
          for (int k = 0; k < 2; k++) {
            xx[k] = base + k * K4_T;
            const int xc = min(xx[k], n - 1);
            gdw[k] = s.good[xc >> 5]; lxv[k] = s.lx[xc]; tn[k] = s.tln[xc];
#pragma unroll
            for (int e = 0; e < K4_CAP; e++) { lc[k][e] = s.tlc[xc * K4_CAP + e]; lc[k][K4_CAP + e] = s.tlo[xc * K4_CAP + e]; }
          }
          unsigned gyw[2][K4_HINT];
#pragma unroll
          for (int k = 0; k < 2; k++)
#pragma unroll
            for (int e = 0; e < K4_HINT; e++) gyw[k][e] = s.goody[lc[k][e] >> 5];
#pragma unroll
          for (int k = 0; k < 2; k++) {
            if (xx[k] >= n) continue;
            if ((gdw[k] >> (xx[k] & 31)) & 1u) {
              const int yo = mx[xx[k]];
              if (yo != K4_NONE && !k4_bit(s.goody, yo)) { atomicOr(&s.goody[yo >> 5], 1u << (yo & 31)); ch = true; }
              continue;
            }
            bool g = (lxv[k] - bg) < eps;
            const int t = tn[k] <= K4_HINT ? tn[k] : 0;
#pragma unroll
            for (int e = 0; e < K4_HINT; e++) g |= (int)(e < t) & (int)((gyw[k][e] >> (lc[k][e] & 31)) & 1u);
            if (g) {
              atomicOr(&s.good[xx[k] >> 5], 1u << (xx[k] & 31));
              const int yo = mx[xx[k]];
              if (yo != K4_NONE) atomicOr(&s.goody[yo >> 5], 1u << (yo & 31));
              ch = true;
            }
          }
        }
        for (int fb = 0; fb < nf; fb += 16) {
          const int i = fb + wave * 4 + (lane >> 4), lig = lane & 15;
          int x = -1, cnt = 0;
          if (i < nf) { x = flist[i]; cnt = pool[i * region]; }
          bool hit = false;
          if (x >= 0 && !k4_bit(s.good, x))
            for (int e = lig; e < cnt; e += 16) hit |= k4_bit(s.goody, pool[i * region + 1 + e]);
          const unsigned gb = (unsigned)(__ballot(hit) >> (lane & 48)) & 0xffffu;
          if (gb && lig == 0) {
            atomicOr(&s.good[x >> 5], 1u << (x & 31));
            const int yo = mx[x];
            if (yo != K4_NONE) atomicOr(&s.goody[yo >> 5], 1u << (yo & 31));
            ch = true;
          }
        }
        if (ch) s.sh[chslot[round % 3]] = 1;
        __syncthreads();
        if (!s.sh[chslot[round % 3]]) break;
        if (round >= 40) {
          for (int w = tid; w < nw; w += K4_T) { s.goody[w] = ~0u; s.good[w] = ~0u; }
          break;
        }
      }
      __syncthreads();
      t2 = PROF ? (long long)__builtin_readcyclecounter() : 0;
      if (PROF) c_pull += t2 - t1b;
      if (wave == sw) {
        int r = 0;
        if (k4_dfs_unwind(s, dfs, lane)) r = k4_dfs<PROF>(s, dfs, false, lane, &q_iter, &q_act, pd);
        if (lane == 0) s.sh[SH_DFS] = r;
      }
      __syncthreads();
      if (PROF) c_dfs += (long long)__builtin_readcyclecounter() - t2;
      }
      if (s.sh[SH_DFS] != 1 && tid == 0) s.sh[SH_BAD] = 3;
      __syncthreads();
      if (s.sh[SH_BAD]) bad = s.sh[SH_BAD];
      break;
    }
  }
  __syncthreads();
  if (hazard) {
    if (tid == 0) s.sh[SH_BAD] = k4_literal(s, P);
    __syncthreads();
    bad = s.sh[SH_BAD];
  }
  for (int i = tid; i < n; i += K4_T) P.match_out[i] = s.match[i] == K4_NONE ? -1 : (int)s.match[i];
  if (tid == 0 && lstat) {
    const unsigned long long t1 = __builtin_amdgcn_s_memrealtime(), dt = t1 - t_wall0;
    atomicMax(&lstat[0], (1ull << 62) - t_wall0);
    atomicMax(&lstat[1], t1);
    atomicAdd(&lstat[2], dt);
    atomicMax(&lstat[3], dt);
    atomicAdd(&lstat[4], 1ull);
  }
  if (tid == 0) {
    if (bad && P.status) *P.status = bad;
    if (hazard && P.status) atomicAdd(P.status, 0x10000);
    if (P.steps) {
      P.steps[0] = q_act;
      if (PROF) {
        P.steps[1] = q_phase; P.steps[2] = q_fail; P.steps[3] = q_rounds; P.steps[4] = q_iter; P.steps[5] = q_frows; P.steps[6] = q_prows;
        P.steps[7] = c_flood; P.steps[8] = c_fail; P.steps[9] = c_pull; P.steps[10] = c_dfs;
        P.steps[11] = (long long)__builtin_readcyclecounter() - t_begin; P.steps[12] = hazard ? 1 : 0;
        for (int k = 0; k < 5; k++) P.steps[13 + k] = pcf[k];
        for (int k = 0; k < 10; k++) P.steps[18 + k] = pd[k];
      }
    }
  }
}


}
```

### gh-icp_amd/csrc/km_prob.h

```cpp
#pragma once
struct Km2Problem {
  int n, pad_;
  double bg, eps;
  const unsigned* row_ptr;
  const int* cols;
  const double* vals;
  const double* lx_init;
  int* match_out;
  int* status;
  const int* done;
  long long* steps;
};
struct ghicp_ctx;
int gh_km4_launch(ghicp_ctx* ctx, const Km2Problem* d_probs, int nprob, int n_max);
bool gh_km4_fits(int n);
size_t gh_km4_lds_bytes(int n);

struct Km4Plan {
  int nclass = 0;
  int begin[8] = {0}, count[8] = {0};
  size_t lds[8] = {0};
  int per_cu[8] = {0};
  double weight[8] = {0};
  int* d_order = nullptr;
};
int gh_km4_plan(ghicp_ctx* ctx, const int* h_n, int nprob, Km4Plan* plan, const float* cost = nullptr);
int gh_km4_launch_plan(ghicp_ctx* ctx, const Km2Problem* d_probs, const Km4Plan& plan);
```

### gh-icp_amd/csrc/loop.hip

```cpp
#include "ctx.h"
#include "devmath.h"

#include <cmath>

#include "km_prob.h"
#include "km4_dev.h"
int gh_km_solve_dev(ghicp_ctx* ctx, const double* w, int n, double eps, int32_t* match, const int* done_flag);

namespace {

struct LoopState {
  int it, done, cor, converged_flag;
  double RMS, FDM, FDstd, IoU, para1, para2, penalty, CDmean, CDstd, energy;
  double Rt_till[16];
  double rmse_after;
  unsigned long long t_begin, t_end;
  unsigned long long t_solve_max;
  int it_solve_max;
  unsigned hw_id;
};

struct LoopConst {
  int ks, kt, n, feature, corr, max_iter, min_cor, nchunk_a, nchunk_b, chunk_a, chunk_b, nparts;
  float scale, est_iou, adjust_ratio, adjust_step;
  double converge_t, converge_r, penalty_initial, km_eps;
};

struct LoopProb {
  LoopConst C;
  LoopState* st;
  double* kpS;
  const double* kpS_src;
  const double* kpT;
  const void* FD;
  const void* FDt;
  int fdt_given;
  const double* wfd;
  double *pminA, *pminB, *psum;
  int *pidxA, *pidxB, *SP, *TP, *SVs, *TVs;
  ghicp_iter* trace;
  int* matchlist;
  int ml_row0;
  unsigned *km_cnt, *km_rptr;
  int *km_cols, *kmmatch, *km_status;
  double *km_vals, *km_lx, *kmw;
  Km2Problem* km_desc;
};

constexpr int ROWS = 256;
constexpr int CHUNK_MAX = 512;

template <int FT>
__device__ inline double combined_distance(double ed, const void* fd, size_t idx, double wed, double wfd, double inv_k) {
  if (FT == GHICP_FEATURE_BSC) return wed * ed + wfd * (double)reinterpret_cast<const uint16_t*>(fd)[idx];
  if (FT == GHICP_FEATURE_FPFH) return 1.0 * ed / pow((double)reinterpret_cast<const float*>(fd)[idx], inv_k);
  return ed;
}

template <int FT>
__device__ inline double cd_pivot(const LoopProb& P, double wed, double wfd, double inv_k) {
  const double dx = P.kpS[0] - P.kpT[0], dy = P.kpS[1] - P.kpT[1], dz = P.kpS[2] - P.kpT[2];
  return combined_distance<FT>((double)P.C.scale * sqrt(dx * dx + dy * dy + dz * dz), P.FD, 0, wed, wfd, inv_k);
}

template <int FT, bool COLS>
__device__ inline void dev_cd_rowmin(const LoopProb& P, const int bx, const int by, double* sB, double* red) {
  const int ka = COLS ? P.C.kt : P.C.ks, kb = COLS ? P.C.ks : P.C.kt;
  const int chunk = COLS ? P.C.chunk_a : P.C.chunk_b, nchunk = COLS ? P.C.nchunk_a : P.C.nchunk_b;
  if (by >= nchunk || bx * ROWS >= ka) return;
  const double* A = COLS ? P.kpT : P.kpS;
  const double* B = COLS ? P.kpS : P.kpT;
  const void* F = COLS ? P.FD : P.FDt;
  const int it = P.st->it;
  const int jb = by * chunk;
  const int je = min(kb, jb + chunk);
  for (int t = threadIdx.x; t < (je - jb) * 3; t += ROWS) sB[t] = B[(size_t)jb * 3 + t];
  __syncthreads();
  const int a = bx * ROWS + threadIdx.x;
  const bool live = a < ka;
  double ax = 0, ay = 0, az = 0;
  if (live) { ax = A[(size_t)a * 3]; ay = A[(size_t)a * 3 + 1]; az = A[(size_t)a * 3 + 2]; }
  double wfd = 0, wed = 1;
  if (FT == GHICP_FEATURE_BSC) { wfd = P.wfd[it]; wed = 1.0 - wfd; }
  const double inv_k = 1.0 / (double)(it + 1);
  const double dscale = (double)P.C.scale;
  double best = 9e20, s = 0, s2 = 0;
  int bidx = 0;
  double piv = 0;
  if (!COLS) piv = cd_pivot<FT>(P, wed, wfd, inv_k);
  if (live) {
    for (int j = jb; j < je; j++) {
      const double dx = ax - sB[(j - jb) * 3], dy = ay - sB[(j - jb) * 3 + 1], dz = az - sB[(j - jb) * 3 + 2];
      const double ed = dscale * sqrt(dx * dx + dy * dy + dz * dz);
      const double cd = combined_distance<FT>(ed, F, (size_t)j * ka + a, wed, wfd, inv_k);
      if (cd < best) { best = cd; bidx = j; }
      if (!COLS) { const double c0 = cd - piv; s += c0; s2 += c0 * c0; }
    }
    (COLS ? P.pminB : P.pminA)[(size_t)by * ka + a] = best;
    (COLS ? P.pidxB : P.pidxA)[(size_t)by * ka + a] = bidx;
  }
  if (!COLS) {
    const double bs = gh_block_sum(s, red);
    const double bs2 = gh_block_sum(s2, red);
    if (threadIdx.x == 0) {
      const size_t b = (size_t)by * cdiv_dev(ka, ROWS) + bx;
      P.psum[b * 2] = bs;
      P.psum[b * 2 + 1] = bs2;
    }
  }
}

template <int FT, bool COLS>
__global__ __launch_bounds__(ROWS) void k_cd_rowmin(const LoopProb* __restrict__ probs) {
  const LoopProb& P = probs[blockIdx.z];
  if (P.st->done) return;
  __shared__ double sB[CHUNK_MAX * 3];
  __shared__ double red[16];
  dev_cd_rowmin<FT, COLS>(P, (int)blockIdx.x, (int)blockIdx.y, sB, red);
}

__device__ inline void dev_penalty(const LoopProb& P, double* red) {
  LoopState* st = P.st;
  const LoopConst& C = P.C;
  double s = 0, s2 = 0;
  for (int i = threadIdx.x; i < C.nparts; i += blockDim.x) { s += P.psum[i * 2]; s2 += P.psum[i * 2 + 1]; }
  s = gh_block_sum(s, red);
  s2 = gh_block_sum(s2, red);
  if (threadIdx.x == 0) {
    const int it = st->it;
    const double cnt = (double)C.ks * (double)C.kt;
    double piv, wfd0 = 0, wed0 = 1;
    if (C.feature == GHICP_FEATURE_BSC) { wfd0 = P.wfd[it]; wed0 = 1.0 - wfd0; }
    const double inv_k0 = 1.0 / (double)(it + 1);
    if (C.feature == GHICP_FEATURE_BSC) piv = cd_pivot<GHICP_FEATURE_BSC>(P, wed0, wfd0, inv_k0);
    else if (C.feature == GHICP_FEATURE_FPFH) piv = cd_pivot<GHICP_FEATURE_FPFH>(P, wed0, wfd0, inv_k0);
    else piv = cd_pivot<GHICP_FEATURE_NONE>(P, wed0, wfd0, inv_k0);
    const double dm = s / (double)C.kt / (double)C.ks;
    const double mean = piv + dm;
    double var = s2 / cnt - dm * dm;
    if (var < 0) var = 0;
    const double sd = sqrt(var);
    double pen;
    if (C.feature == GHICP_FEATURE_NONE) {
      pen = fmax(mean, 1.0);
      st->CDstd = 0;
    } else if (C.feature == GHICP_FEATURE_BSC) {
      const double wfd = P.wfd[it], wed = 1.0 - wfd;
      if (it > 1) pen = st->RMS * st->para1 * (double)C.scale * wed + (st->FDM + st->para2 * st->FDstd) * wfd;
      else pen = mean - C.penalty_initial * sd;
      pen = fmax(pen, 5.0);
      st->CDstd = sd;
    } else {
      if (it > 1) pen = st->RMS * st->para1 * (double)C.scale * st->para2;
      else pen = mean / C.penalty_initial;
      st->CDstd = 0;
    }
    st->CDmean = mean;
    st->penalty = pen;
  }
}

__global__ __launch_bounds__(256) void k_penalty(const LoopProb* __restrict__ probs) {
  const LoopProb& P = probs[blockIdx.x];
  if (P.st->done) return;
  __shared__ double red[16];
  dev_penalty(P, red);
}

template <int FT>
__global__ __launch_bounds__(256) void k_km_weights(const LoopProb* __restrict__ probs) {
  const LoopProb& P = probs[blockIdx.z];
  if (P.st->done || P.kmw == nullptr) return;
  const LoopConst& C = P.C;
  const int j = blockIdx.x * 256 + threadIdx.x;
  const int i = blockIdx.y;
  if (j >= C.n || i >= C.n) return;
  const double pen = P.st->penalty;
  double out = -pen;
  if (i < C.ks && j < C.kt) {
    const int it = P.st->it;
    const double dx = P.kpS[(size_t)i * 3] - P.kpT[(size_t)j * 3], dy = P.kpS[(size_t)i * 3 + 1] - P.kpT[(size_t)j * 3 + 1],
                 dz = P.kpS[(size_t)i * 3 + 2] - P.kpT[(size_t)j * 3 + 2];
    const double ed = (double)C.scale * sqrt(dx * dx + dy * dy + dz * dz);
    double wfd = 0, wed = 1;
    if (FT == GHICP_FEATURE_BSC) { wfd = P.wfd[it]; wed = 1.0 - wfd; }
    const double cd = combined_distance<FT>(ed, P.FD, (size_t)i * C.kt + j, wed, wfd, 1.0 / (double)(it + 1));
    if (cd < pen) out = -cd;
  }
  P.kmw[(size_t)i * C.n + j] = out;
}

template <int FT, int FILL>
__device__ inline void dev_km_csr(const LoopProb& P, const int bx) {
  const LoopConst& C = P.C;
  const int wave = threadIdx.x >> 6, lane = threadIdx.x & 63;
  const int i = bx * 4 + wave;
  if (i >= C.n) return;
  const double pen = P.st->penalty;
  if (i >= C.ks) {
    if (!FILL && lane == 0) { P.km_cnt[i] = 0u; P.km_lx[i] = -pen; }
    return;
  }
  const int it = P.st->it;
  double wfd = 0, wed = 1;
  if (FT == GHICP_FEATURE_BSC) { wfd = P.wfd[it]; wed = 1.0 - wfd; }
  const double inv_k = 1.0 / (double)(it + 1);
  const double sx = P.kpS[(size_t)i * 3], sy = P.kpS[(size_t)i * 3 + 1], sz = P.kpS[(size_t)i * 3 + 2];
  const unsigned base = FILL ? P.km_rptr[i] : 0u;
  unsigned c = 0;
  double mx = -pen;
  for (int j0 = 0; j0 < C.kt; j0 += 64) {
    const int j = j0 + lane;
    bool e = false;
    double wv = 0;
    if (j < C.kt) {
      const double dx = sx - P.kpT[(size_t)j * 3], dy = sy - P.kpT[(size_t)j * 3 + 1], dz = sz - P.kpT[(size_t)j * 3 + 2];
      const double ed = (double)C.scale * sqrt(dx * dx + dy * dy + dz * dz);
      const double cd = combined_distance<FT>(ed, P.FD, (size_t)i * C.kt + j, wed, wfd, inv_k);
      e = cd < pen;
      wv = -cd;
    }
    const unsigned long long b = __ballot(e);
    if (FILL && e) {
      const unsigned off = c + __popcll(b & ((1ull << lane) - 1ull));
      P.km_cols[base + off] = j;
      P.km_vals[base + off] = wv;
    }
    if (!FILL && e) mx = fmax(mx, wv);
    c += __popcll(b);
  }
  if (!FILL) {
    for (int o = 32; o > 0; o >>= 1) mx = fmax(mx, __shfl_xor(mx, o, 64));
    if (lane == 0) { P.km_cnt[i] = c; P.km_lx[i] = mx; }
  }
}

template <int FT, int FILL>
__global__ __launch_bounds__(256) void k_km_csr(const LoopProb* __restrict__ probs) {
  const LoopProb& P = probs[blockIdx.y];
  if (P.st->done || P.km_rptr == nullptr) return;
  dev_km_csr<FT, FILL>(P, (int)blockIdx.x);
}

__device__ inline void dev_km_scan_desc(const LoopProb& P, int* sc) {
  const int n = P.C.n;
  int carry = 0;
  for (int base = 0; base < n; base += (int)blockDim.x) {
    const int i = base + threadIdx.x;
    const int v = i < n ? (int)P.km_cnt[i] : 0;
    int tot;
    const int ex = gh_block_excl_scan(v, sc, &tot);
    if (i < n) P.km_rptr[i] = (unsigned)(carry + ex);
    carry += tot;
    __syncthreads();
  }
  if (threadIdx.x == 0) {
    P.km_rptr[n] = (unsigned)carry;
    Km2Problem p;
    p.n = n; p.pad_ = 0; p.bg = -P.st->penalty; p.eps = P.C.km_eps; p.row_ptr = P.km_rptr; p.cols = P.km_cols; p.vals = P.km_vals;
    p.lx_init = P.km_lx; p.match_out = P.kmmatch; p.status = P.km_status; p.done = &P.st->done; p.steps = nullptr;
    *P.km_desc = p;
  }
}

__global__ __launch_bounds__(1024) void k_km_scan_desc(const LoopProb* __restrict__ probs) {
  const LoopProb& P = probs[blockIdx.x];
  if (P.st->done || P.km_rptr == nullptr) return;
  __shared__ int sc[17];
  dev_km_scan_desc(P, sc);
}

template <int FT>
__device__ inline void dev_solve(const LoopProb& P, double* red, int* ired, double* sh) {
  LoopState* st = P.st;
  const LoopConst& C = P.C;
  double* kpS = P.kpS;
  const double* kpT = P.kpT;
  const void* FD = P.FD;
  int* SP = P.SP;
  int* TP = P.TP;
  const int tid = threadIdx.x, nt = blockDim.x;
  const int it = st->it;
  const double penalty = st->penalty;
  int* matchlist = P.matchlist;
  if (matchlist)
    for (int i = tid; i < C.ks; i += nt) matchlist[(size_t)(it - P.ml_row0) * C.ks + i] = -1;

  int cor = 0;
  if (C.corr == GHICP_CORR_KM) {
    double e = 0;
    for (int base = 0; base < C.n; base += nt) {
      const int y = base + tid;
      int flag = 0, x = -1;
      if (y < C.n) x = P.kmmatch[y];
      if (y < C.n && x >= 0) {
        double g = -penalty;
        if (P.km_rptr) {
          unsigned lo = P.km_rptr[x], hi = P.km_rptr[x + 1];
          const unsigned end = hi;
          while (lo < hi) { const unsigned mid = (lo + hi) >> 1; if (P.km_cols[mid] < y) lo = mid + 1; else hi = mid; }
          if (lo < end && P.km_cols[lo] == y) g = P.km_vals[lo];
        } else {
          g = P.kmw[(size_t)x * C.n + y];
        }
        flag = (g != -penalty) ? 1 : 0;
        if (g != -10000.0) e -= g;
      }
      int tot;
      const int pos = gh_block_excl_scan(flag, ired, &tot);
      if (flag) { SP[cor + pos] = x; TP[cor + pos] = y; }
      cor += tot;
      __syncthreads();
    }
    e = gh_block_sum(e, red);
    if (tid == 0) st->energy = e;
  } else {
    for (int i = tid; i < C.ks; i += nt) {
      double best = 9e20; int bi = 0;
      for (int c = 0; c < C.nchunk_b; c++) {
        const double v = P.pminA[(size_t)c * C.ks + i];
        if (v < best) { best = v; bi = P.pidxA[(size_t)c * C.ks + i]; }
      }
      P.SVs[i] = bi;
      P.TVs[C.kt + i] = (best < penalty) ? 1 : 0;
    }
    if (C.corr == GHICP_CORR_NNR) {
      for (int j = tid; j < C.kt; j += nt) {
        double best = 9e20; int bi = 0;
        for (int c = 0; c < C.nchunk_a; c++) {
          const double v = P.pminB[(size_t)c * C.kt + j];
          if (v < best) { best = v; bi = P.pidxB[(size_t)c * C.kt + j]; }
        }
        P.TVs[j] = bi;
      }
    }
    __syncthreads();
    for (int base = 0; base < C.ks; base += nt) {
      const int i = base + tid;
      int flag = 0, sv = 0;
      if (i < C.ks) {
        sv = P.SVs[i];
        if (C.corr == GHICP_CORR_NN) flag = P.TVs[C.kt + i];
        else flag = (C.kt > 0 && P.TVs[sv] == i) ? 1 : 0;
      }
      int tot;
      const int pos = gh_block_excl_scan(flag, ired, &tot);
      if (flag) { SP[cor + pos] = i; TP[cor + pos] = sv; }
      cor += tot;
      __syncthreads();
    }
  }
  __syncthreads();
  if (matchlist)
    for (int c = tid; c < cor; c += nt) matchlist[(size_t)(it - P.ml_row0) * C.ks + SP[c]] = TP[c];

  double rm = 0, fm = 0;
  for (int c = tid; c < cor; c += nt) {
    const int i = SP[c], j = TP[c];
    const double dx = kpS[(size_t)i * 3] - kpT[(size_t)j * 3], dy = kpS[(size_t)i * 3 + 1] - kpT[(size_t)j * 3 + 1],
                 dz = kpS[(size_t)i * 3 + 2] - kpT[(size_t)j * 3 + 2];
    rm += dx * dx + dy * dy + dz * dz;
    if (FT == GHICP_FEATURE_BSC) fm += (double)reinterpret_cast<const uint16_t*>(FD)[(size_t)i * C.kt + j];
    if (FT == GHICP_FEATURE_FPFH) fm += (double)reinterpret_cast<const float*>(FD)[(size_t)i * C.kt + j];
  }
  rm = gh_block_sum(rm, red);
  fm = gh_block_sum(fm, red);
  const double FDM = fm / (double)cor;
  double fc = 0;
  if (FT != GHICP_FEATURE_NONE)
    for (int c = tid; c < cor; c += nt) {
      const int i = SP[c], j = TP[c];
      double f = (FT == GHICP_FEATURE_BSC) ? (double)reinterpret_cast<const uint16_t*>(FD)[(size_t)i * C.kt + j]
                                           : (double)reinterpret_cast<const float*>(FD)[(size_t)i * C.kt + j];
      f -= FDM;
      fc += f * f;
    }
  fc = gh_block_sum(fc, red);
  const double FDstd = sqrt(fc / (double)cor);
  const double RMSE = sqrt(rm / (double)cor);

  double m[6] = {0, 0, 0, 0, 0, 0};
  for (int c = tid; c < cor; c += nt) {
    const int i = SP[c], j = TP[c];
    for (int d = 0; d < 3; d++) { m[d] += (double)(float)kpS[(size_t)i * 3 + d]; m[3 + d] += (double)(float)kpT[(size_t)j * 3 + d]; }
  }
  for (int d = 0; d < 6; d++) m[d] = gh_block_sum(m[d], red);
  float msf[3], mtf[3];
  for (int d = 0; d < 3; d++) { msf[d] = (float)(m[d] / (double)cor); mtf[d] = (float)(m[3 + d] / (double)cor); }
  double H[9] = {0, 0, 0, 0, 0, 0, 0, 0, 0};
  for (int c = tid; c < cor; c += nt) {
    const int i = SP[c], j = TP[c];
    double a[3], b[3];
    for (int d = 0; d < 3; d++) {
      a[d] = (double)(float)kpT[(size_t)j * 3 + d] - (double)mtf[d];
      b[d] = (double)(float)kpS[(size_t)i * 3 + d] - (double)msf[d];
    }
    for (int r = 0; r < 3; r++)
      for (int q = 0; q < 3; q++) H[r * 3 + q] += a[r] * b[q];
  }
  for (int d = 0; d < 9; d++) H[d] = gh_block_sum(H[d], red);
  if (tid == 0) {
    double A[9], R[9];
    for (int d = 0; d < 9; d++) A[d] = H[d] / (double)cor;
    gh_quant_grid(A, 9);
    gh_kabsch(A, R);
    float Rf[9], tf[3];
    for (int d = 0; d < 9; d++) Rf[d] = (float)R[d];
    for (int r = 0; r < 3; r++)
      tf[r] = (float)((double)mtf[r] -
                      (((double)Rf[r * 3] * (double)msf[0] + (double)Rf[r * 3 + 1] * (double)msf[1]) + (double)Rf[r * 3 + 2] * (double)msf[2]));
    for (int r = 0; r < 3; r++) {
      for (int q = 0; q < 3; q++) sh[r * 4 + q] = (double)Rf[r * 3 + q];
      sh[r * 4 + 3] = (double)tf[r];
    }
  }
  __syncthreads();
  double Rt[12];
  for (int d = 0; d < 12; d++) Rt[d] = sh[d];

  double ra = 0;
  for (int c = tid; c < cor; c += nt) {
    const int i = SP[c], j = TP[c];
    const double x = kpS[(size_t)i * 3], y = kpS[(size_t)i * 3 + 1], z = kpS[(size_t)i * 3 + 2];
    const double nx = ((Rt[0] * x + Rt[1] * y) + Rt[2] * z) + Rt[3];
    const double ny = ((Rt[4] * x + Rt[5] * y) + Rt[6] * z) + Rt[7];
    const double nz = ((Rt[8] * x + Rt[9] * y) + Rt[10] * z) + Rt[11];
    const double dx = nx - kpT[(size_t)j * 3], dy = ny - kpT[(size_t)j * 3 + 1], dz = nz - kpT[(size_t)j * 3 + 2];
    ra += dx * dx + dy * dy + dz * dz;
  }
  ra = gh_block_sum(ra, red);
  __syncthreads();
  for (int i = tid; i < C.ks; i += nt) {
    const double x = kpS[(size_t)i * 3], y = kpS[(size_t)i * 3 + 1], z = kpS[(size_t)i * 3 + 2];
    kpS[(size_t)i * 3] = ((Rt[0] * x + Rt[1] * y) + Rt[2] * z) + Rt[3];
    kpS[(size_t)i * 3 + 1] = ((Rt[4] * x + Rt[5] * y) + Rt[6] * z) + Rt[7];
    kpS[(size_t)i * 3 + 2] = ((Rt[8] * x + Rt[9] * y) + Rt[10] * z) + Rt[11];
  }

  if (tid == 0) {
    const double RMSEafter = sqrt(ra / (double)cor);
    bool conv = false;
    if (cor < C.min_cor) conv = true;
    const double IoU = 1.0 * (double)cor / (double)(C.ks + C.kt - cor);
    const double dx = Rt[3], dy = Rt[7], dz = Rt[11];
    double ax = atan2(Rt[9], Rt[10]);
    double ay = atan2(-Rt[8], sqrt(Rt[9] * Rt[9] + Rt[10] * Rt[10]));
    double az = atan2(Rt[1], Rt[0]);
    const double pi = 3.1415926;
    ax = ax / pi * 180; ay = ay / pi * 180; az = az / pi * 180;
    if (fabs(dx) < C.converge_t && fabs(dy) < C.converge_t && fabs(dz) < C.converge_t && fabs(ax) < C.converge_r &&
        fabs(ay) < C.converge_r && fabs(az) < C.converge_r)
      conv = true;
    double p1 = st->para1, p2 = st->para2;
    if ((double)C.est_iou / IoU > (double)C.adjust_ratio) { p1 += (double)C.adjust_step; p2 += (double)C.adjust_step; }
    else if (IoU / (double)C.est_iou > (double)C.adjust_ratio) { p1 -= (double)C.adjust_step; p2 -= (double)C.adjust_step; }
    double nt16[16];
    const double Rt16[16] = {Rt[0], Rt[1], Rt[2], Rt[3], Rt[4], Rt[5], Rt[6], Rt[7], Rt[8], Rt[9], Rt[10], Rt[11], 0, 0, 0, 1};
    for (int r = 0; r < 4; r++)
      for (int c = 0; c < 4; c++) {
        double s = 0;
        for (int k = 0; k < 4; k++) s += Rt16[r * 4 + k] * st->Rt_till[k * 4 + c];
        nt16[r * 4 + c] = s;
      }
    for (int d = 0; d < 16; d++) st->Rt_till[d] = nt16[d];
    ghicp_iter rec;
    rec.cor = cor; rec.converged = conv ? 1 : 0;
    rec.penalty = penalty; rec.cdmean = st->CDmean; rec.cdstd = st->CDstd; rec.rmse = RMSE; rec.rmse_after = RMSEafter;
    rec.fdm = FDM; rec.fdstd = FDstd; rec.iou = IoU; rec.para1 = p1; rec.para2 = p2;
    rec.energy = (C.corr == GHICP_CORR_KM) ? st->energy : 0.0;
    for (int d = 0; d < 16; d++) rec.Rt[d] = Rt16[d];
    P.trace[it] = rec;
    st->RMS = RMSE; st->FDM = FDM; st->FDstd = FDstd; st->IoU = IoU; st->para1 = p1; st->para2 = p2; st->cor = cor;
    st->rmse_after = RMSEafter;
    st->it = it + 1;
    if (conv || it + 1 >= C.max_iter) { st->done = 1; st->converged_flag = conv ? 1 : 0; }
  }
}

template <int FT>
__global__ __launch_bounds__(1024) void k_solve(const LoopProb* __restrict__ probs) {
  const LoopProb& P = probs[blockIdx.x];
  if (P.st->done) return;
  __shared__ double red[16];
  __shared__ int ired[17];
  __shared__ double sh[32];
  dev_solve<FT>(P, red, ired, sh);
}

__global__ __launch_bounds__(256) void k_pairs_copy_kps(const LoopProb* __restrict__ probs, int pair0) {
  const LoopProb& P = probs[pair0 + blockIdx.y];
  const int n = P.C.ks * 3;
  for (int i = blockIdx.x * 256 + threadIdx.x; i < n; i += gridDim.x * 256) P.kpS[i] = P.kpS_src[i];
}
template <typename T> __global__ void k_pairs_transpose(const LoopProb* __restrict__ probs, int pair0) {
  const LoopProb& P = probs[pair0 + blockIdx.z];
  const int rows = P.C.ks, cols = P.C.kt;
  if (rows <= 0 || cols <= 0 || (int)blockIdx.x * 32 >= cols || (int)blockIdx.y * 32 >= rows || P.fdt_given) return;
  const T* __restrict__ in = reinterpret_cast<const T*>(P.FD);
  T* __restrict__ out = const_cast<T*>(reinterpret_cast<const T*>(P.FDt));
  __shared__ T tile[32][33];
  const int x = blockIdx.x * 32 + threadIdx.x, y0 = blockIdx.y * 32;
  for (int r = threadIdx.y; r < 32; r += blockDim.y)
    if (x < cols && y0 + r < rows) tile[r][threadIdx.x] = in[(size_t)(y0 + r) * cols + x];
  __syncthreads();
  const int ox = blockIdx.y * 32 + threadIdx.x, oy0 = blockIdx.x * 32;
  for (int r = threadIdx.y; r < 32; r += blockDim.y)
    if (ox < rows && oy0 + r < cols) out[(size_t)(oy0 + r) * rows + ox] = tile[threadIdx.x][r];
}


__global__ void k_collect_done(const LoopProb* __restrict__ probs, int n, int* __restrict__ out) {
  const int i = blockIdx.x * blockDim.x + threadIdx.x;
  if (i < n) { out[i * 2] = probs[i].st->it; out[i * 2 + 1] = probs[i].st->done; }
}

constexpr int PL_SCRATCH = (CHUNK_MAX * 3 + 16 + 32) * 8 + 20 * 4;

template <int FT>
__device__ __noinline__ void pl_sweep(const LoopProb& P, double* sB, double* red) {
  const int rbA = cdiv_dev(P.C.ks > 0 ? P.C.ks : 1, ROWS);
  for (int by = 0; by < P.C.nchunk_b; by++)
    for (int bx = 0; bx < rbA; bx++) {
      __syncthreads();
      dev_cd_rowmin<FT, false>(P, bx, by, sB, red);
    }
  __syncthreads();
  dev_penalty(P, red);
  __syncthreads();
}
template <int FT>
__device__ __noinline__ void pl_graph(const LoopProb& P, int* ired) {
  const int rb4 = cdiv_dev(P.C.n, 4);
  for (int bx = 0; bx < rb4; bx++) dev_km_csr<FT, 0>(P, bx);
  __syncthreads();
  dev_km_scan_desc(P, ired);
  __syncthreads();
  for (int bx = 0; bx < rb4; bx++) dev_km_csr<FT, 1>(P, bx);
  __syncthreads();
}
template <bool PROF>
__device__ __noinline__ void pl_km(const Km2Problem* desc, int km_flags, char* smem, int lds_bytes) {
  const Km2Problem KP = *desc;
  k4_solve_block<PROF>(KP, km_flags, smem, lds_bytes, nullptr);
  __syncthreads();
}
template <int FT>
__device__ __noinline__ void pl_solve(const LoopProb& P, double* red, int* ired, double* sh) {
  dev_solve<FT>(P, red, ired, sh);
  __syncthreads();
}

template <int FT, bool PROF>
__global__ __launch_bounds__(K4_T, 4) void k_pair_loop(const LoopProb* __restrict__ probs, const int* __restrict__ order, const int npairs, int* qhead,
                                                  const int km_flags, const int lds_bytes, unsigned long long* lstat, int* progress,
                                                  const int* __restrict__ order2, const int npairs2, int* qhead2) {
  extern __shared__ __attribute__((aligned(16))) char smem[];
  double* sB = reinterpret_cast<double*>(smem);
  double* red = sB + CHUNK_MAX * 3;
  double* sh = red + 16;
  int* ired = reinterpret_cast<int*>(sh + 32);
  volatile int* s_idx = ired + 18;
  const unsigned long long t_slot0 = lstat ? __builtin_amdgcn_s_memrealtime() : 0ull;
  unsigned long long t_solve = 0ull, t_solve_max = 0ull, n_solve = 0ull;
  __builtin_amdgcn_s_setprio(3);
  for (int qsel = 0; qsel < 2; qsel++) {
  const int* const ord = qsel == 0 ? order : order2;
  const int np = qsel == 0 ? npairs : npairs2;
  int* const qh = qsel == 0 ? qhead : qhead2;
  if (ord == nullptr) break;
  for (;;) {
    __syncthreads();
    if (threadIdx.x == 0) *s_idx = atomicAdd(qh, 1);
    __syncthreads();
    const int q = *s_idx;
    if (q >= np) break;
    const LoopProb& P = probs[ord[q]];
    if (threadIdx.x == 0 && lstat) P.st->t_begin = __builtin_amdgcn_s_memrealtime();
    unsigned long long t_pair_max = 0ull;
    int it_pair_max = 0;
    while (*(volatile int*)&P.st->done == 0) {
      pl_sweep<FT>(P, sB, red);
      pl_graph<FT>(P, ired);
      const unsigned long long t0 = lstat ? __builtin_amdgcn_s_memrealtime() : 0ull;
      pl_km<PROF>(P.km_desc, km_flags, smem, lds_bytes);
      if (lstat) {
        const unsigned long long dt = __builtin_amdgcn_s_memrealtime() - t0;
        t_solve += dt; t_solve_max = dt > t_solve_max ? dt : t_solve_max; n_solve++;
        if (dt > t_pair_max) { t_pair_max = dt; it_pair_max = *(volatile int*)&P.st->it; }
      }
      pl_solve<FT>(P, red, ired, sh);
    }
    if (threadIdx.x == 0 && lstat) {
      P.st->t_end = __builtin_amdgcn_s_memrealtime();
      P.st->t_solve_max = t_pair_max;
      P.st->it_solve_max = it_pair_max;
      P.st->hw_id = ((unsigned)__builtin_amdgcn_s_getreg((4) | (0 << 6) | (31 << 11)) & 0xFFFFu) | (((unsigned)__builtin_amdgcn_s_getreg((20) | (0 << 6) | (3 << 11)) & 0xFu) << 16);
    }
    if (threadIdx.x == 0 && progress) __hip_atomic_fetch_add(progress, 1, __ATOMIC_RELAXED, __HIP_MEMORY_SCOPE_SYSTEM);
  }
  }
  if (threadIdx.x == 0 && lstat) {
    const unsigned long long t1 = __builtin_amdgcn_s_memrealtime();
    atomicMax(&lstat[0], (1ull << 62) - t_slot0);
    atomicMax(&lstat[1], t1);
    atomicAdd(&lstat[2], t_solve);
    atomicMax(&lstat[3], t_solve_max);
    atomicAdd(&lstat[4], n_solve);
    atomicAdd(&lstat[5], t1 - t_slot0);
    atomicAdd(&lstat[6], 1ull);
  }
}

static void pick_chunks(int ka, int kb, int batch, int* chunk, int* nchunk) {
  const int rowblocks = cdiv(ka > 0 ? ka : 1, ROWS) * (batch > 0 ? batch : 1);
  int want = cdiv(2048, rowblocks);
  int ch = cdiv(kb > 0 ? kb : 1, want);
  if (ch < 32) ch = 32;
  if (ch > CHUNK_MAX) ch = CHUNK_MAX;
  *chunk = ch;
  *nchunk = kb > 0 ? cdiv(kb, ch) : 1;
}

struct Carver {
  char* base;
  size_t off = 0;
  explicit Carver(char* b) : base(b) {}
  template <typename T> T* take(size_t count) {
    off = (off + 255) & ~(size_t)255;
    T* p = base ? reinterpret_cast<T*>(base + off) : nullptr;
    off += count * sizeof(T);
    return p;
  }
};

static void gh_join_aux(ghicp_ctx* ctx) {
  (void)hipStreamSynchronize(ctx->stream);
  if (ctx->confine_stream) (void)hipStreamSynchronize(ctx->confine_stream);
  if (ctx->rest_stream) (void)hipStreamSynchronize(ctx->rest_stream);
  for (hipStream_t a : ctx->aux_streams) (void)hipStreamSynchronize(a);
}
#define GH_HIP_JOIN(call)                                                                                     \
  do {                                                                                                        \
    const hipError_t e_ = (call);                                                                             \
    if (e_ != hipSuccess) { gh_join_aux(ctx); return ctx->fail(GHICP_ERR_HIP, "%s: %s", #call, hipGetErrorString(e_)); } \
  } while (0)
template <int FT>
int run_pair_loop(ghicp_ctx* ctx, const LoopProb* dprobs, int nb, const Km4Plan& plan, int* dqheads) {
  hipStream_t s = ctx->stream;
  const int nc = plan.nclass;
  if (nc <= 0) return GHICP_OK;
  while ((int)ctx->aux_streams.size() < nc - 1) {
    hipStream_t a = nullptr;
    if (ctx->cu_mask.empty()) GH_HIP(hipStreamCreateWithFlags(&a, hipStreamNonBlocking));
    else GH_HIP(hipExtStreamCreateWithCUMask(&a, (uint32_t)ctx->cu_mask.size(), ctx->cu_mask.data()));
    ctx->aux_streams.push_back(a);
  }
  while ((int)ctx->aux_events.size() < nc + 2) {
    hipEvent_t e = nullptr;
    GH_HIP(hipEventCreateWithFlags(&e, hipEventDisableTiming));
    ctx->aux_events.push_back(e);
  }
  if (!ctx->progress_host) {
    if (hipHostMalloc((void**)&ctx->progress_host, 64, hipHostMallocMapped) != hipSuccess)
      return ctx->fail(GHICP_ERR_HIP, "pair loop: mapped progress counter allocation failed");
  }
  *(volatile int*)ctx->progress_host = 0;
  ctx->progress_live.store(true, std::memory_order_release);
  const bool prof = ctx->km_stats;
  const void* fn = prof ? reinterpret_cast<const void*>(&k_pair_loop<FT, true>) : reinterpret_cast<const void*>(&k_pair_loop<FT, false>);
  GH_HIP(hipFuncSetAttribute(fn, hipFuncAttributeMaxDynamicSharedMemorySize, 160 * 1024));
  const int kflags = ctx->km_force_hazard ? 4 : 0;
  GH_HIP(hipMemsetAsync(dqheads, 0, 16 * sizeof(int), s));
  unsigned long long* lstat = nullptr;
  int batch_slots = 0, batch_grid = 0;
  if (ctx->kt_on && ctx->km_launches < ghicp_ctx::KM_LSTAT_MAX) {
    GH_TRY(ctx->reserve(B_KM_LSTAT, (size_t)ghicp_ctx::KM_LSTAT_MAX * ghicp_ctx::KM_LSTAT_W, &lstat));
    lstat += ctx->km_launches * ghicp_ctx::KM_LSTAT_W;
  }
  int confine_b = 0;
  if (ctx->loop_confine && nc == 2 && plan.per_cu[0] == 3 && plan.per_cu[1] == 4 && plan.count[0] > 0 && plan.count[1] > 0 && ctx->cu_mask.empty() &&
      ctx->num_cu >= 8 && ctx->num_cu <= 2048 && plan.weight[0] > 0 && plan.weight[1] > 0) {
    const double w = std::min(0.9, ctx->loop_confine_margin * plan.weight[0] / (plan.weight[0] + plan.weight[1]));
    int B = (int)std::ceil(w * 4.0 * ctx->num_cu / (3.0 + w));
    B = std::max(B, (plan.count[0] >= 3 ? 1 : 0));
    B = std::min(B, std::min(ctx->num_cu / 2, cdiv(plan.count[0], 3)));
    if (B >= 1) {
      if (ctx->confine_stream == nullptr || ctx->rest_stream == nullptr || ctx->confine_cus != B) {
        ctx->confine_stream = ctx->rest_stream = nullptr;
        ctx->confine_cus = 0;
        for (auto& e : ctx->confine_cache)
          if (e.cus == B) { ctx->confine_stream = e.confined; ctx->rest_stream = e.rest; ctx->confine_cus = B; }
        if (ctx->confine_cus != B) {
          if (ctx->confine_cache.size() >= 16) {
            for (auto& e : ctx->confine_cache) {
              (void)hipStreamSynchronize(e.confined); (void)hipStreamDestroy(e.confined);
              (void)hipStreamSynchronize(e.rest); (void)hipStreamDestroy(e.rest);
            }
            ctx->confine_cache.clear();
          }
          std::vector<uint32_t> mask((size_t)cdiv(ctx->num_cu, 32), 0u), rest((size_t)cdiv(ctx->num_cu, 32), 0u);
          for (int i = 0; i < ctx->num_cu; i++) {
            const bool in = (long long)(i + 1) * B / ctx->num_cu > (long long)i * B / ctx->num_cu;
            (in ? mask : rest)[(size_t)i >> 5] |= 1u << (i & 31);
          }
          hipStream_t sa = nullptr, sb = nullptr;
          if (hipExtStreamCreateWithCUMask(&sa, (uint32_t)mask.size(), mask.data()) == hipSuccess &&
              hipExtStreamCreateWithCUMask(&sb, (uint32_t)rest.size(), rest.data()) == hipSuccess) {
            ctx->confine_cache.push_back({B, sa, sb});
            ctx->confine_stream = sa; ctx->rest_stream = sb; ctx->confine_cus = B;
          } else {
            if (sa) (void)hipStreamDestroy(sa);
            if (sb) (void)hipStreamDestroy(sb);
            (void)hipGetLastError();
          }
        }
      }
      if (ctx->confine_cus == B) confine_b = B;
    }
  }
  hipEvent_t kt = ctx->kt_begin(KT_PAIR_LOOP);
  GH_HIP_JOIN(hipEventRecord(ctx->aux_events[0], s));
  bool stole = false;
  for (int c = 0; c < nc; c++) {
    if (plan.count[c] <= 0) continue;
    const bool confined = confine_b > 0;
    hipStream_t sc = confined ? (c == 0 ? ctx->confine_stream : ctx->rest_stream) : (c == 0 ? s : ctx->aux_streams[(size_t)c - 1]);
    if (c > 0 || confined) GH_HIP_JOIN(hipStreamWaitEvent(sc, ctx->aux_events[0], 0));
    const size_t lds = std::max(std::max(plan.lds[c], (size_t)PL_SCRATCH + 64), (size_t)ctx->loop_min_lds);
    int per_cu = 0;
    GH_HIP_JOIN(hipOccupancyMaxActiveBlocksPerMultiprocessor(&per_cu, fn, K4_T, lds));
    if (per_cu <= 0) gh_join_aux(ctx);
    if (per_cu <= 0) return ctx->fail(GHICP_ERR_INTERNAL, "pair loop: a workgroup with %zu bytes of LDS does not fit a CU", lds);
    const int slots = per_cu * (confined ? (c == 0 ? confine_b : ctx->num_cu - confine_b) : ctx->num_cu);
    int grid = std::min(plan.count[c], slots);
    if (ctx->loop_slots_cap > 0) grid = std::min(grid, ctx->loop_slots_cap);
    batch_slots = std::max(batch_slots, per_cu * ctx->num_cu);
    batch_grid += grid;
    hipEvent_t kd = ctx->kt_begin_on(KT_PAIR_LOOP_DISPATCH, sc);
    const bool steal = confined && c == 0 && plan.lds[1] <= lds;
    stole = stole || steal;
    const int* o2 = steal ? (const int*)(plan.d_order + plan.begin[1]) : (const int*)nullptr;
    const int n2 = steal ? plan.count[1] : 0;
    int* q2 = steal ? dqheads + 1 : (int*)nullptr;
    if (prof)
      hipLaunchKernelGGL((k_pair_loop<FT, true>), dim3(grid), dim3(K4_T), lds, sc, dprobs, (const int*)(plan.d_order + plan.begin[c]), plan.count[c],
                         dqheads + c, kflags, (int)lds, lstat, ctx->progress_host, o2, n2, q2);
    else
      hipLaunchKernelGGL((k_pair_loop<FT, false>), dim3(grid), dim3(K4_T), lds, sc, dprobs, (const int*)(plan.d_order + plan.begin[c]), plan.count[c],
                         dqheads + c, kflags, (int)lds, lstat, ctx->progress_host, o2, n2, q2);
    ctx->kt_end_on(KT_PAIR_LOOP_DISPATCH, kd, sc);
    GH_HIP_JOIN(hipGetLastError());
    if (c > 0 || confined) {
      GH_HIP_JOIN(hipEventRecord(ctx->aux_events[(size_t)c + 1], sc));
      GH_HIP_JOIN(hipStreamWaitEvent(s, ctx->aux_events[(size_t)c + 1], 0));
    }
    if (confined && c == 1 && !stole) {
      const int grid2 = std::min(plan.count[c], per_cu * confine_b);
      hipEvent_t kd2 = ctx->kt_begin_on(KT_PAIR_LOOP_DISPATCH, ctx->confine_stream);
      if (prof)
        hipLaunchKernelGGL((k_pair_loop<FT, true>), dim3(grid2), dim3(K4_T), lds, ctx->confine_stream, dprobs, (const int*)(plan.d_order + plan.begin[c]),
                           plan.count[c], dqheads + c, kflags, (int)lds, lstat, ctx->progress_host, (const int*)nullptr, 0, (int*)nullptr);
      else
        hipLaunchKernelGGL((k_pair_loop<FT, false>), dim3(grid2), dim3(K4_T), lds, ctx->confine_stream, dprobs, (const int*)(plan.d_order + plan.begin[c]),
                           plan.count[c], dqheads + c, kflags, (int)lds, lstat, ctx->progress_host, (const int*)nullptr, 0, (int*)nullptr);
      ctx->kt_end_on(KT_PAIR_LOOP_DISPATCH, kd2, ctx->confine_stream);
      GH_HIP_JOIN(hipGetLastError());
      batch_grid += grid2;
      GH_HIP_JOIN(hipEventRecord(ctx->aux_events[(size_t)nc + 1], ctx->confine_stream));
      GH_HIP_JOIN(hipStreamWaitEvent(s, ctx->aux_events[(size_t)nc + 1], 0));
    }
  }
  ctx->kt_end(KT_PAIR_LOOP, kt);
  if (lstat) {
    ctx->km_slots.push_back(std::min(batch_slots, batch_grid));
    ctx->km_launches++;
  }
  GH_HIP_JOIN(hipStreamSynchronize(s));
  return GHICP_OK;
}
#undef GH_HIP_JOIN

template <int FT>
int run_loops(ghicp_ctx* ctx, int nb, const gh_loop_job* jobs) {
  hipStream_t s = ctx->stream;
  std::vector<float> cost_hints;
  cost_hints.swap(ctx->loop_cost_hints);
  const ghicp_params* p0 = jobs[0].p;
  const int corr = p0->corr;
  int max_iter = 1;
  for (int b = 0; b < nb; b++) max_iter = jobs[b].p->max_iter > max_iter ? jobs[b].p->max_iter : max_iter;
  std::vector<double> wtab(max_iter + 1);
  for (int i = 0; i <= max_iter; i++) wtab[i] = std::exp(-1.0 * i / p0->weight_changing_rate);

  std::vector<LoopProb> hp(nb);
  std::vector<LoopState> hst(nb);
  size_t total = 0;
  int max_rowsA = 1, max_chunkB = 1, max_rowsB = 1, max_chunkA = 1, max_n = 1;
  bool persistent = corr == GHICP_CORR_KM;
  for (int b = 0; b < nb && persistent; b++) {
    const int n = std::max(jobs[b].ks, jobs[b].kt);
    persistent = (jobs[b].ks <= 0 || jobs[b].kt <= 0) || gh_km4_fits(n);
  }
  const int chunk_batch = persistent ? (1 << 20) : nb;
  for (int pass = 0; pass < 2; pass++) {
    char* arena = nullptr;
    if (pass == 1) GH_TRY(ctx->reserve(B_LOOP_STATE, total + 4096, &arena));
    Carver cv(arena);
    const double* wfd = cv.take<double>(wtab.size());
    LoopProb* dprobs = cv.take<LoopProb>(nb);
    int* dflags = cv.take<int>((size_t)nb * 2);
    int* dqheads = cv.take<int>(16);
    Km2Problem* d_descs = cv.take<Km2Problem>(nb);
    LoopState* dstates = cv.take<LoopState>(nb);
    int* dkmst = cv.take<int>((size_t)nb + 1);
    int max_ks = 1, max_kt = 1;
    bool need_transpose = false;
    for (int b = 0; b < nb; b++) {
      const gh_loop_job& J = jobs[b];
      const ghicp_params* p = J.p;
      LoopProb& L = hp[b];
      memset(&L, 0, sizeof(L));
      LoopConst& C = L.C;
      const int ks = J.ks, kt = J.kt;
      C.ks = ks; C.kt = kt; C.n = ks > kt ? ks : kt; C.feature = p->feature; C.corr = p->corr; C.max_iter = p->max_iter; C.min_cor = p->min_cor;
      C.scale = (float)(0.005 * p->bbx_magnitude);
      C.est_iou = p->est_iou; C.adjust_ratio = p->adjust_ratio; C.adjust_step = p->adjust_step;
      C.converge_t = (double)p->converge_t; C.converge_r = (double)p->converge_r; C.penalty_initial = p->penalty_initial; C.km_eps = p->km_eps;
      pick_chunks(ks, kt, chunk_batch, &C.chunk_b, &C.nchunk_b);
      pick_chunks(kt, ks, chunk_batch, &C.chunk_a, &C.nchunk_a);
      C.nparts = cdiv(ks > 0 ? ks : 1, ROWS) * C.nchunk_b;
      max_rowsA = std::max(max_rowsA, cdiv(ks > 0 ? ks : 1, ROWS)); max_chunkB = std::max(max_chunkB, C.nchunk_b);
      max_rowsB = std::max(max_rowsB, cdiv(kt > 0 ? kt : 1, ROWS)); max_chunkA = std::max(max_chunkA, C.nchunk_a);
      max_n = std::max(max_n, C.n);
      L.wfd = wfd;
      L.st = dstates + b;
      L.kpS_src = J.kpS;
      max_ks = std::max(max_ks, ks); max_kt = std::max(max_kt, kt);
      L.kpS = cv.take<double>((size_t)ks * 3 + 3);
      L.kpT = J.kpT; L.FD = J.FD;
      L.pminA = cv.take<double>((size_t)C.nchunk_b * ks + 1);
      L.pidxA = cv.take<int>((size_t)C.nchunk_b * ks + 1);
      L.psum = cv.take<double>((size_t)C.nparts * 2 + 2);
      if (corr == GHICP_CORR_NNR) {
        L.pminB = cv.take<double>((size_t)C.nchunk_a * kt + 1);
        L.pidxB = cv.take<int>((size_t)C.nchunk_a * kt + 1);
      }
      L.SP = cv.take<int>((size_t)C.n + 1);
      L.TP = cv.take<int>((size_t)C.n + 1);
      L.SVs = cv.take<int>((size_t)ks + 1);
      L.TVs = cv.take<int>((size_t)kt + ks + 2);
      L.trace = cv.take<ghicp_iter>((size_t)p->max_iter + 1);
      L.matchlist = J.matchlist;
      L.ml_row0 = J.ml_row0;
      if (FT != GHICP_FEATURE_NONE) {
        if (J.FDt) L.FDt = J.FDt;
        else { L.FDt = cv.take<char>((size_t)ks * kt * (FT == GHICP_FEATURE_BSC ? 2 : 4) + 16); need_transpose = true; }
        L.fdt_given = J.FDt != nullptr;
      }
      if (corr == GHICP_CORR_KM) {
        L.kmmatch = cv.take<int>((size_t)C.n + 1);
        L.km_status = dkmst + b;
        if (gh_km4_fits(C.n)) {
          L.km_cnt = cv.take<unsigned>((size_t)C.n + 1);
          L.km_rptr = cv.take<unsigned>((size_t)C.n + 2);
          L.km_lx = cv.take<double>((size_t)C.n + 1);
          L.km_cols = cv.take<int>((size_t)ks * kt + 1);
          L.km_vals = cv.take<double>((size_t)ks * kt + 1);
          L.km_desc = d_descs ? d_descs + b : nullptr;
        } else {
          L.kmw = cv.take<double>((size_t)C.n * C.n + 1);
        }
      }
    }
    total = cv.off;
    if (pass == 1) {
      GH_HIP(hipMemcpyAsync(const_cast<double*>(wfd), wtab.data(), wtab.size() * sizeof(double), hipMemcpyHostToDevice, s));
      GH_HIP(hipMemsetAsync(d_descs, 0, (size_t)nb * sizeof(Km2Problem), s));
      for (int b = 0; b < nb; b++) {
        LoopState& h = hst[b];
        memset(&h, 0, sizeof(h));
        h.RMS = 99999; h.para1 = jobs[b].p->para1; h.para2 = jobs[b].p->para2;
        for (int d = 0; d < 4; d++) h.Rt_till[d * 5] = 1.0;
        if (jobs[b].resume_in) {
          memcpy(&h, jobs[b].resume_in, sizeof(h));
          h.done = 0;
        }
        if (jobs[b].ks <= 0 || jobs[b].kt <= 0) h.done = 1;
      }
      GH_HIP(hipMemcpyAsync(dstates, hst.data(), (size_t)nb * sizeof(LoopState), hipMemcpyHostToDevice, s));
      GH_HIP(hipMemsetAsync(dkmst, 0, ((size_t)nb + 1) * sizeof(int), s));
      GH_HIP(hipMemcpyAsync(dprobs, hp.data(), (size_t)nb * sizeof(LoopProb), hipMemcpyHostToDevice, s));
      for (int b0 = 0; b0 < nb; b0 += 65535)
        hipLaunchKernelGGL(k_pairs_copy_kps, dim3(std::min(cdiv(max_ks * 3, 256), 8), std::min(65535, nb - b0)), dim3(256), 0, s, (const LoopProb*)dprobs, b0);
      if (FT != GHICP_FEATURE_NONE && need_transpose) {
        const int tx = cdiv(max_kt, 32), ty = cdiv(max_ks, 32);
        const int zmax = (int)std::max<long long>(1, std::min<long long>(65535, (1ll << 22) / ((long long)tx * ty)));
        for (int b0 = 0; b0 < nb; b0 += zmax) {
          const dim3 g(tx, ty, std::min(zmax, nb - b0));
          if (FT == GHICP_FEATURE_BSC) hipLaunchKernelGGL(k_pairs_transpose<uint16_t>, g, dim3(32, 8), 0, s, (const LoopProb*)dprobs, b0);
          else hipLaunchKernelGGL(k_pairs_transpose<float>, g, dim3(32, 8), 0, s, (const LoopProb*)dprobs, b0);
        }
      }
      GH_HIP(hipGetLastError());

      ctx->loop_total.store(nb, std::memory_order_relaxed);
      ctx->loop_active.store(nb, std::memory_order_relaxed);
      std::vector<int> hflags((size_t)nb * 2, 0);
      const int poll_every = 2;
      int launched = 0;
      bool all_done = false;
      bool any_dense = false;
      for (int b = 0; b < nb; b++) any_dense |= (hp[b].kmw != nullptr);
      bool any_sparse = false;
      int max_n_sparse = 1;
      for (int b = 0; b < nb; b++)
        if (hp[b].km_rptr) { any_sparse = true; max_n_sparse = std::max(max_n_sparse, hp[b].C.n); }
      Km4Plan km_plan;
      bool use_plan = false;
      if (any_sparse && !any_dense && gh_km4_fits(max_n_sparse)) {
        std::vector<int> hn((size_t)nb);
        bool all_sparse = true;
        for (int b = 0; b < nb; b++) { hn[b] = hp[b].C.n; all_sparse &= (hp[b].km_rptr != nullptr) || jobs[b].ks <= 0 || jobs[b].kt <= 0; }
        if (all_sparse) {
          const bool hinted = (int)cost_hints.size() == nb;
          GH_TRY(gh_km4_plan(ctx, hn.data(), nb, &km_plan, hinted ? cost_hints.data() : nullptr));
          use_plan = true;
        }
      }
      if (persistent && use_plan) {
        const int rc = run_pair_loop<FT>(ctx, dprobs, nb, km_plan, dqheads);
        if (rc != GHICP_OK) {
          ctx->progress_live.store(false, std::memory_order_release);
          return rc;
        }
        all_done = true;
      }
      while (!all_done && launched < max_iter) {
        for (int r = 0; r < poll_every && launched < max_iter; r++, launched++) {
          hipEvent_t kev = ctx->kt_begin(KT_CD_ROWMIN);
          hipLaunchKernelGGL((k_cd_rowmin<FT, false>), dim3(max_rowsA, max_chunkB, nb), dim3(ROWS), 0, s, dprobs);
          ctx->kt_end(KT_CD_ROWMIN, kev);
          if (corr == GHICP_CORR_NNR) hipLaunchKernelGGL((k_cd_rowmin<FT, true>), dim3(max_rowsB, max_chunkA, nb), dim3(ROWS), 0, s, dprobs);
          hipLaunchKernelGGL(k_penalty, dim3(nb), dim3(256), 0, s, dprobs);
          if (corr == GHICP_CORR_KM) {
            hipEvent_t kw = ctx->kt_begin(KT_KM_WEIGHTS);
            hipLaunchKernelGGL((k_km_csr<FT, 0>), dim3(cdiv(max_n, 4), nb), dim3(256), 0, s, dprobs);
            hipLaunchKernelGGL(k_km_scan_desc, dim3(nb), dim3(1024), 0, s, dprobs);
            hipLaunchKernelGGL((k_km_csr<FT, 1>), dim3(cdiv(max_n, 4), nb), dim3(256), 0, s, dprobs);
            ctx->kt_end(KT_KM_WEIGHTS, kw);
            if (any_sparse) GH_TRY(use_plan ? gh_km4_launch_plan(ctx, d_descs, km_plan) : gh_km4_launch(ctx, d_descs, nb, max_n_sparse));
            if (any_dense) {
              hipLaunchKernelGGL(k_km_weights<FT>, dim3(cdiv(max_n, 256), max_n, nb), dim3(256), 0, s, dprobs);
              for (int b = 0; b < nb; b++)
                if (hp[b].kmw) GH_TRY(gh_km_solve_dev(ctx, hp[b].kmw, hp[b].C.n, hp[b].C.km_eps, hp[b].kmmatch, &hp[b].st->done));
            }
          }
          hipLaunchKernelGGL(k_solve<FT>, dim3(nb), dim3(256), 0, s, dprobs);
        }
        GH_HIP(hipGetLastError());
        hipLaunchKernelGGL(k_collect_done, dim3(cdiv(nb, 256)), dim3(256), 0, s, dprobs, nb, dflags);
        GH_HIP(hipMemcpyAsync(hflags.data(), dflags, hflags.size() * sizeof(int), hipMemcpyDeviceToHost, s));
        GH_HIP(hipStreamSynchronize(s));
        all_done = true;
        long long still = 0;
        for (int b = 0; b < nb; b++) { all_done &= (hflags[(size_t)b * 2 + 1] != 0); still += hflags[(size_t)b * 2 + 1] == 0; }
        ctx->loop_active.store(still, std::memory_order_relaxed);
      }
      ctx->loop_active.store(0, std::memory_order_relaxed);
      ctx->progress_live.store(false, std::memory_order_release);
      std::vector<int> hkmst((size_t)nb + 1, 0);
      GH_HIP(hipMemcpyAsync(hst.data(), dstates, (size_t)nb * sizeof(LoopState), hipMemcpyDeviceToHost, s));
      GH_HIP(hipMemcpyAsync(hkmst.data(), dkmst, ((size_t)nb + 1) * sizeof(int), hipMemcpyDeviceToHost, s));
      GH_HIP(hipStreamSynchronize(s));
      if (ctx->kt_on && persistent) {
        ctx->loop_timeline.resize((size_t)nb * 3);
        for (int b = 0; b < nb; b++) {
          const unsigned hw = hst[b].hw_id;
          const unsigned long long where = (unsigned long long)((hw >> 8) & 0xFu) | ((unsigned long long)((hw >> 12) & 1u) << 4) | ((unsigned long long)((hw >> 13) & 7u) << 5) |
                                           ((unsigned long long)((hw >> 16) & 0xFu) << 8);
          ctx->loop_timeline[(size_t)b * 3] = (long long)((hst[b].t_begin & 0x000FFFFFFFFFFFFFull) | (where << 52));
          ctx->loop_timeline[(size_t)b * 3 + 1] = (long long)(hst[b].t_end & 0x000FFFFFFFFFFFFFull);
          ctx->loop_timeline[(size_t)b * 3 + 2] = (long long)(((unsigned long long)(hst[b].it & 0xFFFF)) | ((unsigned long long)(hst[b].it_solve_max & 0xFFFF) << 16) |
                                                              (std::min<unsigned long long>(hst[b].t_solve_max >> 4, 0xFFFFFFFFull) << 32));
        }
      }
      for (int b = 0; b < nb; b++) {
        const gh_loop_job& J = jobs[b];
        for (int d = 0; d < 16; d++) J.Rt16[d] = hst[b].Rt_till[d];
        if (J.n_iter) *J.n_iter = hst[b].it;
        if (J.converged) *J.converged = hst[b].converged_flag;
        if (J.rmse_after) *J.rmse_after = hst[b].rmse_after;
        if (J.trace && hst[b].it > 0) GH_HIP(hipMemcpyAsync(J.trace, hp[b].trace, (size_t)hst[b].it * sizeof(ghicp_iter), hipMemcpyDeviceToHost, s));
        if (J.trace_last && hst[b].it > 0) GH_HIP(hipMemcpyAsync(J.trace_last, hp[b].trace + (hst[b].it - 1), sizeof(ghicp_iter), hipMemcpyDeviceToHost, s));
        if (J.kpS_out && J.ks > 0) GH_HIP(hipMemcpyAsync(J.kpS_out, hp[b].kpS, (size_t)J.ks * 3 * sizeof(double), hipMemcpyDeviceToDevice, s));
        if (J.resume_out) memcpy(J.resume_out, &hst[b], sizeof(LoopState));
      }
      GH_HIP(hipStreamSynchronize(s));
      int kmst = 0;
      for (int b = 0; b < nb; b++)
        if (hp[b].km_status) {
          kmst |= hkmst[(size_t)b] & 0xFFFF;
          ctx->loop_hazards += (long long)((unsigned)hkmst[(size_t)b] >> 16);
        }
      if (any_dense && ctx->buf[B_KM_MISC].p) {
        int v = 0;
        GH_HIP(hipMemcpy(&v, ctx->buf[B_KM_MISC].p, sizeof(int), hipMemcpyDeviceToHost));
        kmst |= v;
      }
      if (kmst) return ctx->fail(GHICP_ERR_INTERNAL, "KM solver status %d (non-finite energy?)", kmst);
    }
  }
  return GHICP_OK;
}

}

int gh_register_batch_dev(ghicp_ctx* ctx, int nb, const gh_loop_job* jobs) {
  if (nb <= 0) return GHICP_OK;
  for (int b = 0; b < nb; b++) {
    const gh_loop_job& J = jobs[b];
    GH_ARG(J.p != nullptr && J.Rt16 != nullptr);
    GH_ARG(J.ks >= 0 && J.kt >= 0 && J.p->max_iter > 0 && J.p->max_iter <= 100000);
    GH_ARG(J.p->corr == GHICP_CORR_NN || J.p->corr == GHICP_CORR_NNR || J.p->corr == GHICP_CORR_KM);
    GH_ARG(J.p->feature == jobs[0].p->feature && J.p->corr == jobs[0].p->corr && J.p->weight_changing_rate == jobs[0].p->weight_changing_rate);
    if (J.p->feature == GHICP_FEATURE_BSC || J.p->feature == GHICP_FEATURE_FPFH) GH_ARG(J.FD != nullptr || J.ks == 0 || J.kt == 0);
  }
  switch (jobs[0].p->feature) {
    case GHICP_FEATURE_BSC: return run_loops<GHICP_FEATURE_BSC>(ctx, nb, jobs);
    case GHICP_FEATURE_FPFH: return run_loops<GHICP_FEATURE_FPFH>(ctx, nb, jobs);
    case GHICP_FEATURE_NONE:
    case GHICP_FEATURE_ROPS:
      return run_loops<GHICP_FEATURE_NONE>(ctx, nb, jobs);
    default: return ctx->fail(GHICP_ERR_ARG, "unknown feature type %d", jobs[0].p->feature);
  }
}

int gh_register_dev(ghicp_ctx* ctx, const ghicp_params* p, const double* kpS, int ks, const double* kpT, int kt, const void* FD,
                    double* Rt16, ghicp_iter* trace, int32_t* n_iter, int32_t* matchlist) {
  gh_loop_job J;
  memset(&J, 0, sizeof(J));
  J.p = p; J.kpS = kpS; J.ks = ks; J.kpT = kpT; J.kt = kt; J.FD = FD; J.Rt16 = Rt16; J.trace = trace; J.n_iter = n_iter; J.matchlist = matchlist;
  return gh_register_batch_dev(ctx, 1, &J);
}

extern "C" int ghicp_register(ghicp_ctx* ctx, const ghicp_params* p, const double* kpS, int64_t ks, const double* kpT, int64_t kt,
                              const void* FD, double* Rt16, ghicp_iter* trace, int32_t* n_iter, int32_t* matchlist) {
  GH_ENTER(ctx);
  GH_ARG(p != nullptr && ks >= 0 && kt >= 0 && ks < (1 << 24) && kt < (1 << 24));
  Stager sg(ctx);
  const double *dS, *dT;
  GH_TRY(sg.in(kpS, (size_t)ks * 3, &dS));
  GH_TRY(sg.in(kpT, (size_t)kt * 3, &dT));
  const size_t esz = p->feature == GHICP_FEATURE_BSC ? 2 : 4;
  const char* dFD = nullptr;
  if (p->feature == GHICP_FEATURE_BSC || p->feature == GHICP_FEATURE_FPFH) GH_TRY(sg.in((const char*)FD, (size_t)ks * kt * esz, &dFD));
  int32_t* dml;
  GH_TRY(sg.out(matchlist, (size_t)p->max_iter * ks, &dml));
  GH_TRY(gh_register_dev(ctx, p, dS, (int)ks, dT, (int)kt, dFD, Rt16, trace, n_iter, dml));
  return sg.finish();
}

struct ghicp_loop {
  ghicp_ctx* ctx;
  ghicp_params p;
  int ks, kt;
  DevBuf kpS, kpT, FD;
  LoopState st;
  bool started, finished;
};

extern "C" int ghicp_loop_create(ghicp_ctx* ctx, const ghicp_params* p, const double* kpS, int64_t ks, const double* kpT, int64_t kt, const void* FD,
                                 ghicp_loop** out) {
  GH_ENTER(ctx);
  GH_ARG(p != nullptr && out != nullptr && ks >= 0 && kt >= 0 && ks < (1 << 24) && kt < (1 << 24));
  GH_ARG(p->corr == GHICP_CORR_NN || p->corr == GHICP_CORR_NNR || p->corr == GHICP_CORR_KM);
  const bool has_fd = p->feature == GHICP_FEATURE_BSC || p->feature == GHICP_FEATURE_FPFH;
  if (has_fd) GH_ARG(FD != nullptr || ks == 0 || kt == 0);
  *out = nullptr;
  ghicp_loop* L = new ghicp_loop();
  L->ctx = ctx; L->p = *p; L->ks = (int)ks; L->kt = (int)kt; L->started = false; L->finished = false;
  memset(&L->st, 0, sizeof(L->st));
  const hipMemcpyKind kind = ctx->host_ptrs ? hipMemcpyHostToDevice : hipMemcpyDeviceToDevice;
  const size_t esz = p->feature == GHICP_FEATURE_BSC ? 2 : 4;
  hipError_t e = L->kpS.reserve((size_t)ks * 24 + 32);
  if (e == hipSuccess) e = L->kpT.reserve((size_t)kt * 24 + 32);
  if (e == hipSuccess && has_fd) e = L->FD.reserve((size_t)ks * kt * esz + 32);
  if (e == hipSuccess && ks > 0) e = hipMemcpyAsync(L->kpS.p, kpS, (size_t)ks * 24, kind, ctx->stream);
  if (e == hipSuccess && kt > 0) e = hipMemcpyAsync(L->kpT.p, kpT, (size_t)kt * 24, kind, ctx->stream);
  if (e == hipSuccess && has_fd && ks > 0 && kt > 0) e = hipMemcpyAsync(L->FD.p, FD, (size_t)ks * kt * esz, kind, ctx->stream);
  if (e == hipSuccess) e = hipStreamSynchronize(ctx->stream);
  if (e != hipSuccess) {
    L->kpS.release(); L->kpT.release(); L->FD.release();
    delete L;
    return ctx->fail(GHICP_ERR_HIP, "ghicp_loop_create: %s", hipGetErrorString(e));
  }
  *out = L;
  return GHICP_OK;
}

extern "C" int ghicp_iterate(ghicp_ctx* ctx, ghicp_loop* L, ghicp_iter* out, int32_t* match_row) {
  GH_ENTER(ctx);
  GH_ARG(L != nullptr && L->ctx == ctx && out != nullptr);
  if (L->finished) return ctx->fail(GHICP_ERR_ARG, "ghicp_iterate: the loop has converged (or has no keypoints); create a new one");
  ghicp_params p = L->p;
  p.max_iter = (L->started ? L->st.it : 0) + 1;
  Stager sg(ctx);
  int32_t* dml;
  GH_TRY(sg.out(match_row, (size_t)L->ks, &dml));
  double Rt16[16];
  int32_t n_iter = 0, conv = 0;
  gh_loop_job J;
  memset(&J, 0, sizeof(J));
  J.p = &p; J.kpS = L->kpS.as<double>(); J.ks = L->ks; J.kpT = L->kpT.as<double>(); J.kt = L->kt; J.FD = L->FD.p; J.Rt16 = Rt16;
  J.n_iter = &n_iter; J.converged = &conv; J.matchlist = dml; J.ml_row0 = p.max_iter - 1;
  J.resume_in = L->started ? &L->st : nullptr; J.resume_out = &L->st; J.kpS_out = L->kpS.as<double>(); J.trace_last = out;
  memset(out, 0, sizeof(*out));
  GH_TRY(gh_register_batch_dev(ctx, 1, &J));
  GH_HIP(hipStreamSynchronize(ctx->stream));
  L->started = true;
  if (L->ks <= 0 || L->kt <= 0 || conv) L->finished = true;
  if (L->ks <= 0 || L->kt <= 0) out->converged = 1;
  return sg.finish();
}

extern "C" int ghicp_loop_result(const ghicp_loop* L, double* Rt16, int32_t* n_iter, int32_t* converged, double* rmse_after) {
  if (!L || !Rt16) return GHICP_ERR_ARG;
  for (int d = 0; d < 16; d++) Rt16[d] = L->started ? L->st.Rt_till[d] : (d % 5 == 0 ? 1.0 : 0.0);
  if (n_iter) *n_iter = L->started ? L->st.it : 0;
  if (converged) *converged = L->started ? L->st.converged_flag : 0;
  if (rmse_after) *rmse_after = L->started ? L->st.rmse_after : 0.0;
  return GHICP_OK;
}

extern "C" void ghicp_loop_destroy(ghicp_loop* L) {
  if (!L) return;
  (void)hipSetDevice(L->ctx->device);
  L->kpS.release(); L->kpT.release(); L->FD.release();
  delete L;
}
```

Measured before the change: 387.5.

## Add compact KM solver variant spilling rarely-used arrays to global scratch

Adds a compact variant of the KM assignment solver that moves the DFS stack y-array and overflow candidate lists out of LDS into per-block global scratch. This shrinks per-problem LDS, so mid-size problems that previously fit only one or two workgroups per CU can fit four. The planner now classes problems by the compact slot size, and both the standalone KM kernel and the fused pair loop pick the compact path when a problem's full layout exceeds the LDS it was given. The cost is global-memory traffic and block fences on those arrays, an extra kernel launch in the standalone path, and a global scratch allocation.

```diff
diff --git a/gh-icp_amd/csrc/ctx.h b/gh-icp_amd/csrc/ctx.h
--- a/gh-icp_amd/csrc/ctx.h
+++ b/gh-icp_amd/csrc/ctx.h
@@ -142,6 +142,9 @@
   int confine_cus = 0;
   struct ConfinePair { int cus; hipStream_t confined, rest; };
   std::vector<ConfinePair> confine_cache;
+  bool km_compact = true;
+  int km_compact_from = 0;
+  int km_kflags() const { return (km_force_hazard ? 4 : 0) | (km_compact_from << 8); }
   int loop_min_lds = 0;
   std::vector<uint32_t> cu_mask;
   std::vector<hipStream_t> aux_streams;
diff --git a/gh-icp_amd/csrc/ctx.hip b/gh-icp_amd/csrc/ctx.hip
--- a/gh-icp_amd/csrc/ctx.hip
+++ b/gh-icp_amd/csrc/ctx.hip
@@ -40,6 +40,8 @@
   c->km_force_hazard = getenv("GHICP_KM_FORCE_HAZARD") != nullptr;
   if (const char* e = getenv("GHICP_LOOP_SLOTS")) c->loop_slots_cap = atoi(e) > 0 ? atoi(e) : 0;
   if (const char* e = getenv("GHICP_LOOP_CONFINE")) c->loop_confine = atoi(e) != 0;
+  if (const char* e = getenv("GHICP_KM_COMPACT")) c->km_compact = atoi(e) != 0;
+  if (const char* e = getenv("GHICP_KM_COMPACT_FROM")) c->km_compact_from = atoi(e) > 0 && atoi(e) < 65535 ? atoi(e) : 0;
   if (const char* e = getenv("GHICP_LOOP_MIN_LDS")) c->loop_min_lds = atoi(e) > 0 ? atoi(e) : 0;
   if (const char* e = getenv("GHICP_LOOP_CONFINE_MARGIN")) { const double m = atof(e); if (m >= 0.25 && m <= 4.0) c->loop_confine_margin = m; }
   if (hipHostMalloc(&c->pinned, 4096, hipHostMallocDefault) != hipSuccess) { delete c; return GHICP_ERR_HIP; }
diff --git a/gh-icp_amd/csrc/km4.hip b/gh-icp_amd/csrc/km4.hip
--- a/gh-icp_amd/csrc/km4.hip
+++ b/gh-icp_amd/csrc/km4.hip
@@ -6,15 +6,23 @@
 
 namespace {
 
-template <bool PROF>
-__global__ __launch_bounds__(K4_T) void k_km4(const Km2Problem* __restrict__ probs, int flags, int lds_bytes, unsigned long long* __restrict__ lstat,
-                                            const int* __restrict__ order) {
+template <bool PROF, bool CP>
+__global__ __launch_bounds__(K4_T, CP ? 4 : 1) void k_km4(const Km2Problem* __restrict__ probs, int flags, int lds_bytes, unsigned long long* __restrict__ lstat,
+                                                        const int* __restrict__ order, unsigned short* __restrict__ scr, long long scr_stride) {
   const Km2Problem P = probs[order ? order[blockIdx.x] : (int)blockIdx.x];
   if (P.n <= 0 || (P.done && *P.done)) return;
+  if (k4_takes_compact(P.n, flags, lds_bytes) != CP) return;
   extern __shared__ __attribute__((aligned(16))) char smem[];
-  k4_solve_block<PROF>(P, flags, smem, lds_bytes, lstat);
+  k4_solve_block<PROF, CP>(P, flags, smem, lds_bytes, lstat, CP && scr ? (k4_gu16)(scr + (size_t)blockIdx.x * (size_t)scr_stride) : (k4_gu16) nullptr);
 }
 
+}
+
+size_t gh_km4_lds_bytes_compact(int n) { return (size_t)k4_lds_need(n, true) + 16; }
+
+size_t gh_km4_slot_bytes(int n, bool compact_on) {
+  const size_t quarter = 160 * 1024 / 4, std_b = gh_km4_lds_bytes(n);
+  return (compact_on && std_b > quarter && gh_km4_lds_bytes_compact(n) <= quarter) ? gh_km4_lds_bytes_compact(n) : std_b;
 }
 
 size_t gh_km4_lds_bytes(int n) {
@@ -24,41 +32,50 @@
 
 bool gh_km4_fits(int n) { return n <= 65534 && gh_km4_lds_bytes(n) <= 160 * 1024 - 256; }
 
-static int k4_launch(ghicp_ctx* ctx, const Km2Problem* d_probs, int nprob, size_t lds, const int* d_order) {
+static int k4_launch(ghicp_ctx* ctx, const Km2Problem* d_probs, int nprob, size_t lds, const int* d_order, int n_max) {
+  unsigned short* scr = nullptr;
+  const long long scr_stride = k4_scratch_u16(n_max);
+  if (ctx->km_compact_from > 0 || k4_lds_need(n_max, false) > (long long)lds) GH_TRY(ctx->reserve(B_KM_SLACK, (size_t)nprob * (size_t)scr_stride, &scr));
   const size_t want = 160 * 1024;
-  GH_HIP(hipFuncSetAttribute(reinterpret_cast<const void*>(&k_km4<false>), hipFuncAttributeMaxDynamicSharedMemorySize, (int)want));
-  GH_HIP(hipFuncSetAttribute(reinterpret_cast<const void*>(&k_km4<true>), hipFuncAttributeMaxDynamicSharedMemorySize, (int)want));
-  const int kflags = ctx->km_force_hazard ? 4 : 0;
+  GH_HIP(hipFuncSetAttribute(reinterpret_cast<const void*>(&k_km4<false, false>), hipFuncAttributeMaxDynamicSharedMemorySize, (int)want));
+  GH_HIP(hipFuncSetAttribute(reinterpret_cast<const void*>(&k_km4<true, false>), hipFuncAttributeMaxDynamicSharedMemorySize, (int)want));
+  GH_HIP(hipFuncSetAttribute(reinterpret_cast<const void*>(&k_km4<false, true>), hipFuncAttributeMaxDynamicSharedMemorySize, (int)want));
+  GH_HIP(hipFuncSetAttribute(reinterpret_cast<const void*>(&k_km4<true, true>), hipFuncAttributeMaxDynamicSharedMemorySize, (int)want));
+  const int kflags = ctx->km_kflags();
   unsigned long long* lstat = nullptr;
   if (ctx->kt_on && ctx->km_launches < ghicp_ctx::KM_LSTAT_MAX) {
     GH_TRY(ctx->reserve(B_KM_LSTAT, (size_t)ghicp_ctx::KM_LSTAT_MAX * ghicp_ctx::KM_LSTAT_W, &lstat));
     lstat += ctx->km_launches * ghicp_ctx::KM_LSTAT_W;
     int per_cu = 0;
-    GH_HIP(hipOccupancyMaxActiveBlocksPerMultiprocessor(&per_cu, reinterpret_cast<const void*>(&k_km4<false>), K4_T, lds));
+    GH_HIP(hipOccupancyMaxActiveBlocksPerMultiprocessor(&per_cu, reinterpret_cast<const void*>(&k_km4<false, false>), K4_T, lds));
     ctx->km_slots.push_back(per_cu * ctx->num_cu);
     ctx->km_launches++;
   }
   hipEvent_t kt = ctx->kt_begin(KT_KM_SOLVE);
-  if (ctx->km_stats) hipLaunchKernelGGL((k_km4<true>), dim3(nprob), dim3(K4_T), lds, ctx->stream, d_probs, kflags, (int)lds, lstat, d_order);
-  else hipLaunchKernelGGL((k_km4<false>), dim3(nprob), dim3(K4_T), lds, ctx->stream, d_probs, kflags, (int)lds, lstat, d_order);
+  if (ctx->km_stats) hipLaunchKernelGGL((k_km4<true, false>), dim3(nprob), dim3(K4_T), lds, ctx->stream, d_probs, kflags, (int)lds, lstat, d_order, scr, scr_stride);
+  else hipLaunchKernelGGL((k_km4<false, false>), dim3(nprob), dim3(K4_T), lds, ctx->stream, d_probs, kflags, (int)lds, lstat, d_order, scr, scr_stride);
+  if (scr) {
+    if (ctx->km_stats) hipLaunchKernelGGL((k_km4<true, true>), dim3(nprob), dim3(K4_T), lds, ctx->stream, d_probs, kflags, (int)lds, lstat, d_order, scr, scr_stride);
+    else hipLaunchKernelGGL((k_km4<false, true>), dim3(nprob), dim3(K4_T), lds, ctx->stream, d_probs, kflags, (int)lds, lstat, d_order, scr, scr_stride);
+  }
   ctx->kt_end(KT_KM_SOLVE, kt);
   GH_HIP(hipGetLastError());
   return GHICP_OK;
 }
 
 int gh_km4_launch(ghicp_ctx* ctx, const Km2Problem* d_probs, int nprob, int n_max) {
-  return k4_launch(ctx, d_probs, nprob, gh_km4_lds_bytes(n_max), nullptr);
+  return k4_launch(ctx, d_probs, nprob, gh_km4_slot_bytes(n_max, ctx->km_compact), nullptr, n_max);
 }
 
-int gh_km4_plan(ghicp_ctx* ctx, const int* h_n, int nprob, Km4Plan* plan, const float* cost) {
+static int k4_plan_host(const int* h_n, int nprob, const float* cost, bool compact_on, Km4Plan* plan, std::vector<int>& order) {
   *plan = Km4Plan();
   std::vector<std::pair<int, int>> key((size_t)nprob);
   for (int i = 0; i < nprob; i++) {
     const int n = std::max(1, h_n[i]);
-    if (!gh_km4_fits(n)) return ctx->fail(GHICP_ERR_INTERNAL, "gh_km4_plan: n = %d does not fit", n);
-    key[i] = {(int)std::min<size_t>(4, (160 * 1024) / gh_km4_lds_bytes(n)), n};
+    if (!gh_km4_fits(n)) return n;
+    key[i] = {(int)std::min<size_t>(4, (160 * 1024) / gh_km4_slot_bytes(n, compact_on)), n};
   }
-  std::vector<int> order((size_t)nprob);
+  order.resize((size_t)nprob);
   for (int i = 0; i < nprob; i++) order[i] = i;
   std::stable_sort(order.begin(), order.end(), [&](int a, int b) {
     if (key[a].first != key[b].first) return key[a].first < key[b].first;
@@ -73,13 +90,35 @@
     plan->begin[nc] = i; plan->count[nc] = j - i;
     int nmax = 1;
     for (int t = i; t < j; t++) nmax = std::max(nmax, key[order[t]].second);
-    plan->lds[nc] = gh_km4_lds_bytes(nmax);
+    for (int t = i; t < j; t++) plan->lds[nc] = std::max(plan->lds[nc], gh_km4_slot_bytes(key[order[t]].second, compact_on));
+    plan->nmax[nc] = nmax;
     plan->per_cu[nc] = key[order[i]].first;
     for (int t = i; t < j; t++) plan->weight[nc] += (cost && cost[order[t]] > 0.f) ? (double)cost[order[t]] : (double)key[order[t]].second * (double)key[order[t]].second;
     nc++;
     i = j;
   }
   plan->nclass = nc;
+  return 0;
+}
+
+extern "C" int ghicp_km4_plan_probe(const int32_t* n, int32_t count, int32_t compact_on, int32_t* per_cu_of_problem, int64_t* lds_of_class, int32_t* nclass) {
+  if (!n || count <= 0 || !per_cu_of_problem || !lds_of_class || !nclass) return GHICP_ERR_ARG;
+  Km4Plan plan;
+  std::vector<int> order;
+  if (k4_plan_host(n, count, nullptr, compact_on != 0, &plan, order) != 0) return GHICP_ERR_ARG;
+  for (int c = 0; c < plan.nclass; c++) {
+    lds_of_class[c] = (int64_t)plan.lds[c];
+    for (int t = plan.begin[c]; t < plan.begin[c] + plan.count[c]; t++) per_cu_of_problem[order[(size_t)t]] = plan.per_cu[c];
+  }
+  *nclass = plan.nclass;
+  return GHICP_OK;
+}
+extern "C" int64_t ghicp_km4_lds_bytes(int32_t n, int32_t compact) { return (int64_t)(compact ? gh_km4_lds_bytes_compact(n) : gh_km4_lds_bytes(n)); }
+
+int gh_km4_plan(ghicp_ctx* ctx, const int* h_n, int nprob, Km4Plan* plan, const float* cost) {
+  std::vector<int> order;
+  const int bad_n = k4_plan_host(h_n, nprob, cost, ctx->km_compact, plan, order);
+  if (bad_n) return ctx->fail(GHICP_ERR_INTERNAL, "gh_km4_plan: n = %d does not fit", bad_n);
   GH_TRY(ctx->reserve(B_KM_ORDER, (size_t)nprob + 1, &plan->d_order));
   GH_HIP(hipMemcpyAsync(plan->d_order, order.data(), (size_t)nprob * sizeof(int), hipMemcpyHostToDevice, ctx->stream));
   GH_HIP(hipStreamSynchronize(ctx->stream));
@@ -88,7 +127,7 @@
 
 int gh_km4_launch_plan(ghicp_ctx* ctx, const Km2Problem* d_probs, const Km4Plan& plan) {
   for (int c = 0; c < plan.nclass; c++)
-    if (plan.count[c] > 0) GH_TRY(k4_launch(ctx, d_probs, plan.count[c], plan.lds[c], plan.d_order + plan.begin[c]));
+    if (plan.count[c] > 0) GH_TRY(k4_launch(ctx, d_probs, plan.count[c], plan.lds[c], plan.d_order + plan.begin[c], plan.nmax[c]));
   return GHICP_OK;
 }
 
diff --git a/gh-icp_amd/csrc/km4_dev.h b/gh-icp_amd/csrc/km4_dev.h
--- a/gh-icp_amd/csrc/km4_dev.h
+++ b/gh-icp_amd/csrc/km4_dev.h
@@ -21,11 +21,18 @@
 
 enum { SH_QT = 0, SH_FREE, SH_RES, SH_QTF, SH_HAZ, SH_CH0, SH_CH1, SH_BAD, SH_NF, SH_UNCERT, SH_LROW, SH_CH2, SH_DFS, SH_NUM = 16 };
 
+typedef __attribute__((address_space(1))) unsigned short* k4_gu16;
+template <bool CP> struct K4Mem { typedef unsigned short* u16p; };
+template <> struct K4Mem<true> { typedef k4_gu16 u16p; };
+
+template <bool CP>
 struct K4 {
   double *lx, *ly, *slack, *red;
   unsigned *visx, *visy, *prevy, *pushed, *good, *goody, *freey, *ovf;
   int* sh;
-  unsigned short *match, *stx, *sty, *tlc, *tlo;
+  unsigned short *match, *stx, *tlc;
+  typename K4Mem<CP>::u16p sty, tlo;
+  typename K4Mem<CP>::u16p tlh;
   unsigned char* tln;
   int n, nw;
   double bg, eps;
@@ -34,12 +41,14 @@
   k4_gf64 vals;
 };
 
+template <bool CP> __device__ inline void k4_gfence() { if (CP) __threadfence_block(); }
+
 __device__ inline bool k4_bit(const unsigned* b, int i) { return (b[i >> 5] >> (i & 31)) & 1u; }
 __device__ inline bool k4_flagged(int tn) { return tn > K4_CAP; }
 __device__ inline int k4_cnt(int tn) { return tn > K4_CAP ? 0 : tn; }
 
-template <bool REBUILD, bool PUSH, bool ONLY_UNPUSHED, bool SEED = false>
-__device__ inline void k4_bulk(const K4& s, const unsigned short* list, int count, int wave, int lane) {
+template <bool REBUILD, bool PUSH, bool ONLY_UNPUSHED, bool SEED = false, bool CP = false>
+__device__ inline void k4_bulk(const K4<CP>& s, const unsigned short* list, int count, int wave, int lane) {
   const int grp = lane >> 4, lig = lane & 15;
   unsigned long long* sl = reinterpret_cast<unsigned long long*>(s.slack);
   for (int base = 0; base < count; base += 16) {
@@ -92,7 +101,7 @@
           __builtin_amdgcn_wave_barrier();
           if (in && td) {
             const int rk = cnt + __popc(gb & ((1u << lig) - 1u));
-            if (rk >= K4_CAP && rk < K4_HINT) s.tlo[x * K4_CAP + rk - K4_CAP] = (unsigned short)col[j];
+            if (rk >= K4_CAP && rk < K4_HINT) s.tlh[x * K4_CAP + rk - K4_CAP] = (unsigned short)col[j];
           }
           cnt += __popc(gb);
         }
@@ -110,7 +119,8 @@
   }
 }
 
-__device__ inline void k4_revalidate(const K4& s, int tid) {
+template <bool CP>
+__device__ inline void k4_revalidate(const K4<CP>& s, int tid) {
   for (int base = tid; base < s.n; base += 4 * K4_T) {
     int tn[4], lc[4][K4_CAP];
     unsigned px[4], pv[4][K4_CAP];
@@ -148,7 +158,8 @@
   }
 }
 
-__device__ inline void k4_pool_build(const K4& s, const unsigned short* __restrict__ flist, unsigned short* __restrict__ pool, int nf, int region, int wave, int lane) {
+template <bool CP>
+__device__ inline void k4_pool_build(const K4<CP>& s, const unsigned short* __restrict__ flist, unsigned short* __restrict__ pool, int nf, int region, int wave, int lane) {
   const int grp = lane >> 4, lig = lane & 15, capf = region - 1;
   for (int base = 0; base < nf; base += 16) {
     const int i = base + wave * 4 + grp;
@@ -223,8 +234,8 @@
     qt += __popcll(eb_);                                                                    \
   } while (0)
 
-template <bool PROF>
-__device__ inline bool k4_flood(const K4& s, int qh0, int qt0, double lflood0, int lane, int* qt_out, long long* pc) {
+template <bool PROF, bool CP>
+__device__ inline bool k4_flood(const K4<CP>& s, int qh0, int qt0, double lflood0, int lane, int* qt_out, long long* pc) {
   const int n = s.n;
   int qh = qh0, qt = qt0;
   bool free_l = false;
@@ -313,8 +324,8 @@
   int sp, x, ystart, cp, cnext;
   double ck;
 };
-template <bool PROF>
-__device__ inline int k4_dfs(const K4& s, K4Dfs& D, const bool lazy, int lane, long long* q_iter, long long* q_act, long long* pd) {
+template <bool PROF, bool CP>
+__device__ inline int k4_dfs(const K4<CP>& s, K4Dfs& D, const bool lazy, int lane, long long* q_iter, long long* q_act, long long* pd) {
   const int n = s.n;
   const double bg = s.bg, eps = s.eps;
   int sp = D.sp, x = D.x, ystart = D.ystart;
@@ -449,19 +460,22 @@
       }
       sp--;
       if (sp < 0) return 0;
+      k4_gfence<CP>();
       x = s.stx[sp]; ystart = (int)s.sty[sp] + 1;
       if (PROF) { pd[4]++; pd[9] += (long long)__builtin_readcyclecounter() - t_it0; }
     }
     __builtin_amdgcn_wave_barrier();
   }
   __builtin_amdgcn_wave_barrier();
+  k4_gfence<CP>();
   const int ylast = s.sty[sp];
   for (int f = lane; f <= sp; f += 64) s.match[s.sty[f]] = s.stx[f];
   if (lane == 0) atomicAnd(&s.freey[ylast >> 5], ~(1u << (ylast & 31)));
   return 1;
 }
 
-__device__ inline bool k4_dfs_unwind(const K4& s, K4Dfs& D, int lane) {
+template <bool CP>
+__device__ inline bool k4_dfs_unwind(const K4<CP>& s, K4Dfs& D, int lane) {
   int keep = D.sp + 1;
   for (int base = 0; base <= D.sp; base += 64) {
     const int f = base + lane;
@@ -478,7 +492,8 @@
   return true;
 }
 
-__device__ inline int k4_literal(const K4& s, const Km2Problem& P) {
+template <bool CP>
+__device__ inline int k4_literal(const K4<CP>& s, const Km2Problem& P) {
   const int n = s.n;
   const double bg = s.bg, eps = s.eps;
   unsigned short* curs = s.tlc;
@@ -543,11 +558,21 @@
   return 0;
 }
 
-template <bool PROF>
-__device__ inline void k4_solve_block(const Km2Problem& P, int flags, char* smem, int lds_bytes, unsigned long long* __restrict__ lstat) {
+__host__ __device__ inline long long k4_lds_need(int n, bool compact) {
+  const long long nw = (n + 31) / 32, u16s = compact ? 5ll * n + 2 : 9ll * n + 4;
+  return 24ll * n + 16 * 8 + 32 * nw + SH_NUM * 4 + 2 * u16s + n;
+}
+__host__ __device__ inline long long k4_scratch_u16(int n) { return ((long long)n * (1 + 2 * K4_CAP) + 2 + 63) & ~63ll; }
+__device__ inline bool k4_takes_compact(int n, int flags, int lds_bytes) {
+  const int from = flags >> 8;
+  return (from > 0 && n >= from) || k4_lds_need(n, false) > (long long)lds_bytes;
+}
+
+template <bool PROF, bool CP>
+__device__ inline void k4_solve_block(const Km2Problem& P, int flags, char* smem, int lds_bytes, unsigned long long* __restrict__ lstat, k4_gu16 scr) {
   const unsigned long long t_wall0 = lstat ? __builtin_amdgcn_s_memrealtime() : 0ull;
   const int n = P.n, nw = (n + 31) / 32, tid = threadIdx.x, lane = tid & 63, wave = tid >> 6;
-  K4 s;
+  K4<CP> s;
   s.n = n; s.nw = nw; s.bg = P.bg; s.eps = P.eps;
   s.rptr = (k4_gu32)P.row_ptr; s.cols = (k4_gint)P.cols; s.vals = (k4_gf64)P.vals;
   s.lx = (double*)smem;
@@ -560,11 +585,20 @@
   s.sh = (int*)(s.ovf + nw);
   s.match = (unsigned short*)(s.sh + SH_NUM);
   s.stx = s.match + n;
-  s.sty = s.stx + n + 2;
-  s.tlc = s.sty + n + 2;
-  s.tlo = s.tlc + (size_t)n * K4_CAP;
-  s.tln = (unsigned char*)(s.tlo + (size_t)n * K4_CAP);
-  if ((long long)(reinterpret_cast<char*>(s.tln + n) - smem) > (long long)lds_bytes) {
+  if constexpr (CP) {
+    s.tlc = s.stx + n + 2;
+    s.tln = (unsigned char*)(s.tlc + (size_t)n * K4_CAP);
+    s.sty = scr;
+    s.tlo = scr + n + 2;
+    s.tlh = s.tlo + (size_t)n * K4_CAP;
+  } else {
+    s.sty = s.stx + n + 2;
+    s.tlc = s.sty + n + 2;
+    s.tlo = s.tlc + (size_t)n * K4_CAP;
+    s.tlh = s.tlo;
+    s.tln = (unsigned char*)(s.tlo + (size_t)n * K4_CAP);
+  }
+  if ((long long)(reinterpret_cast<char*>(s.tln + n) - smem) > (long long)lds_bytes || (CP && scr == nullptr)) {
     if (tid == 0 && P.status) *P.status = 6;
     for (int i = tid; i < n; i += K4_T) P.match_out[i] = -1;
     return;
@@ -578,7 +612,10 @@
   const long long t_begin = PROF ? (long long)__builtin_readcyclecounter() : 0;
 
   for (int i = tid; i < n; i += K4_T) { s.lx[i] = P.lx_init[i]; s.ly[i] = 0.0; s.match[i] = (unsigned short)K4_NONE; s.tln[i] = 0; }
-  for (int i = tid; i < n * K4_CAP; i += K4_T) { s.tlc[i] = 0; s.tlo[i] = 0; }
+  for (int i = tid; i < n * K4_CAP; i += K4_T) {
+    s.tlc[i] = 0;
+    if (!CP) s.tlo[i] = 0;
+  }
   for (int w = tid; w < nw; w += K4_T) {
     unsigned all = ~0u;
     if (w == nw - 1 && (n & 31)) all = (1u << (n & 31)) - 1u;
@@ -763,7 +800,11 @@
             const int xc = min(xx[k], n - 1);
             gdw[k] = s.good[xc >> 5]; lxv[k] = s.lx[xc]; tn[k] = s.tln[xc];
 #pragma unroll
-            for (int e = 0; e < K4_CAP; e++) { lc[k][e] = s.tlc[xc * K4_CAP + e]; lc[k][K4_CAP + e] = s.tlo[xc * K4_CAP + e]; }
+            for (int e = 0; e < K4_CAP; e++) {
+              lc[k][e] = s.tlc[xc * K4_CAP + e];
+              if (CP) lc[k][K4_CAP + e] = (tn[k] > K4_CAP + e && tn[k] <= K4_HINT) ? (int)s.tlh[xc * K4_CAP + e] : 0;
+              else lc[k][K4_CAP + e] = s.tlh[xc * K4_CAP + e];
+            }
           }
           unsigned gyw[2][K4_HINT];
 #pragma unroll
diff --git a/gh-icp_amd/csrc/km_prob.h b/gh-icp_amd/csrc/km_prob.h
--- a/gh-icp_amd/csrc/km_prob.h
+++ b/gh-icp_amd/csrc/km_prob.h
@@ -15,12 +15,17 @@
 int gh_km4_launch(ghicp_ctx* ctx, const Km2Problem* d_probs, int nprob, int n_max);
 bool gh_km4_fits(int n);
 size_t gh_km4_lds_bytes(int n);
+size_t gh_km4_lds_bytes_compact(int n);
+size_t gh_km4_slot_bytes(int n, bool compact_on);
+extern "C" int ghicp_km4_plan_probe(const int32_t* n, int32_t count, int32_t compact_on, int32_t* per_cu_of_problem, int64_t* lds_of_class, int32_t* nclass);
+extern "C" int64_t ghicp_km4_lds_bytes(int32_t n, int32_t compact);
 
 struct Km4Plan {
   int nclass = 0;
   int begin[8] = {0}, count[8] = {0};
   size_t lds[8] = {0};
   int per_cu[8] = {0};
+  int nmax[8] = {0};
   double weight[8] = {0};
   int* d_order = nullptr;
 };
diff --git a/gh-icp_amd/csrc/loop.hip b/gh-icp_amd/csrc/loop.hip
--- a/gh-icp_amd/csrc/loop.hip
+++ b/gh-icp_amd/csrc/loop.hip
@@ -541,7 +541,13 @@
 template <bool PROF>
 __device__ __noinline__ void pl_km(const Km2Problem* desc, int km_flags, char* smem, int lds_bytes) {
   const Km2Problem KP = *desc;
-  k4_solve_block<PROF>(KP, km_flags, smem, lds_bytes, nullptr);
+  k4_solve_block<PROF, false>(KP, km_flags, smem, lds_bytes, nullptr, (k4_gu16) nullptr);
+  __syncthreads();
+}
+template <bool PROF>
+__device__ __noinline__ void pl_km_compact(const Km2Problem* desc, int km_flags, char* smem, int lds_bytes, k4_gu16 scr) {
+  const Km2Problem KP = *desc;
+  k4_solve_block<PROF, true>(KP, km_flags, smem, lds_bytes, nullptr, scr);
   __syncthreads();
 }
 template <int FT>
@@ -553,7 +559,8 @@
 template <int FT, bool PROF>
 __global__ __launch_bounds__(K4_T, 4) void k_pair_loop(const LoopProb* __restrict__ probs, const int* __restrict__ order, const int npairs, int* qhead,
                                                   const int km_flags, const int lds_bytes, unsigned long long* lstat, int* progress,
-                                                  const int* __restrict__ order2, const int npairs2, int* qhead2) {
+                                                  const int* __restrict__ order2, const int npairs2, int* qhead2,
+                                                  unsigned short* __restrict__ scr, const long long scr_stride) {
   extern __shared__ __attribute__((aligned(16))) char smem[];
   double* sB = reinterpret_cast<double*>(smem);
   double* red = sB + CHUNK_MAX * 3;
@@ -582,7 +589,10 @@
       pl_sweep<FT>(P, sB, red);
       pl_graph<FT>(P, ired);
       const unsigned long long t0 = lstat ? __builtin_amdgcn_s_memrealtime() : 0ull;
-      pl_km<PROF>(P.km_desc, km_flags, smem, lds_bytes);
+      if (k4_takes_compact(P.C.n, km_flags, lds_bytes))
+        pl_km_compact<PROF>(P.km_desc, km_flags, smem, lds_bytes, scr ? (k4_gu16)(scr + (size_t)blockIdx.x * (size_t)scr_stride) : (k4_gu16) nullptr);
+      else
+        pl_km<PROF>(P.km_desc, km_flags, smem, lds_bytes);
       if (lstat) {
         const unsigned long long dt = __builtin_amdgcn_s_memrealtime() - t0;
         t_solve += dt; t_solve_max = dt > t_solve_max ? dt : t_solve_max; n_solve++;
@@ -669,7 +679,25 @@
   const bool prof = ctx->km_stats;
   const void* fn = prof ? reinterpret_cast<const void*>(&k_pair_loop<FT, true>) : reinterpret_cast<const void*>(&k_pair_loop<FT, false>);
   GH_HIP(hipFuncSetAttribute(fn, hipFuncAttributeMaxDynamicSharedMemorySize, 160 * 1024));
-  const int kflags = ctx->km_force_hazard ? 4 : 0;
+  const int kflags = ctx->km_kflags();
+  unsigned short* scr = nullptr;
+  long long scr_stride = 0;
+  size_t scr_next = 0;
+  {
+    int n_all = 1;
+    bool need = ctx->km_compact_from > 0;
+    for (int c = 0; c < nc; c++) {
+      n_all = std::max(n_all, plan.nmax[c]);
+      const size_t lds = std::max(std::max(plan.lds[c], (size_t)PL_SCRATCH + 64), (size_t)ctx->loop_min_lds);
+      need = need || k4_lds_need(plan.nmax[c], false) > (long long)lds;
+    }
+    if (need) {
+      scr_stride = k4_scratch_u16(n_all);
+      size_t slots = 0;
+      for (int c = 0; c < nc; c++) slots += 2 * (size_t)std::min(plan.count[c], 4 * ctx->num_cu);
+      GH_TRY(ctx->reserve(B_KM_SLACK, slots * (size_t)scr_stride, &scr));
+    }
+  }
   GH_HIP(hipMemsetAsync(dqheads, 0, 16 * sizeof(int), s));
   unsigned long long* lstat = nullptr;
   int batch_slots = 0, batch_grid = 0;
@@ -742,12 +770,14 @@
     const int* o2 = steal ? (const int*)(plan.d_order + plan.begin[1]) : (const int*)nullptr;
     const int n2 = steal ? plan.count[1] : 0;
     int* q2 = steal ? dqheads + 1 : (int*)nullptr;
+    unsigned short* scr_c = scr ? scr + scr_next * (size_t)scr_stride : nullptr;
+    scr_next += (size_t)grid;
     if (prof)
       hipLaunchKernelGGL((k_pair_loop<FT, true>), dim3(grid), dim3(K4_T), lds, sc, dprobs, (const int*)(plan.d_order + plan.begin[c]), plan.count[c],
-                         dqheads + c, kflags, (int)lds, lstat, ctx->progress_host, o2, n2, q2);
+                         dqheads + c, kflags, (int)lds, lstat, ctx->progress_host, o2, n2, q2, scr_c, scr_stride);
     else
       hipLaunchKernelGGL((k_pair_loop<FT, false>), dim3(grid), dim3(K4_T), lds, sc, dprobs, (const int*)(plan.d_order + plan.begin[c]), plan.count[c],
-                         dqheads + c, kflags, (int)lds, lstat, ctx->progress_host, o2, n2, q2);
+                         dqheads + c, kflags, (int)lds, lstat, ctx->progress_host, o2, n2, q2, scr_c, scr_stride);
     ctx->kt_end_on(KT_PAIR_LOOP_DISPATCH, kd, sc);
     GH_HIP_JOIN(hipGetLastError());
     if (c > 0 || confined) {
@@ -756,13 +786,15 @@
     }
     if (confined && c == 1 && !stole) {
       const int grid2 = std::min(plan.count[c], per_cu * confine_b);
+      unsigned short* scr_c2 = scr ? scr + scr_next * (size_t)scr_stride : nullptr;
+      scr_next += (size_t)grid2;
       hipEvent_t kd2 = ctx->kt_begin_on(KT_PAIR_LOOP_DISPATCH, ctx->confine_stream);
       if (prof)
         hipLaunchKernelGGL((k_pair_loop<FT, true>), dim3(grid2), dim3(K4_T), lds, ctx->confine_stream, dprobs, (const int*)(plan.d_order + plan.begin[c]),
-                           plan.count[c], dqheads + c, kflags, (int)lds, lstat, ctx->progress_host, (const int*)nullptr, 0, (int*)nullptr);
+                           plan.count[c], dqheads + c, kflags, (int)lds, lstat, ctx->progress_host, (const int*)nullptr, 0, (int*)nullptr, scr_c2, scr_stride);
       else
         hipLaunchKernelGGL((k_pair_loop<FT, false>), dim3(grid2), dim3(K4_T), lds, ctx->confine_stream, dprobs, (const int*)(plan.d_order + plan.begin[c]),
-                           plan.count[c], dqheads + c, kflags, (int)lds, lstat, ctx->progress_host, (const int*)nullptr, 0, (int*)nullptr);
+                           plan.count[c], dqheads + c, kflags, (int)lds, lstat, ctx->progress_host, (const int*)nullptr, 0, (int*)nullptr, scr_c2, scr_stride);
       ctx->kt_end_on(KT_PAIR_LOOP_DISPATCH, kd2, ctx->confine_stream);
       GH_HIP_JOIN(hipGetLastError());
       batch_grid += grid2;
```

Result: faster. 412.0, median of 6 (+6.3%).
